# luntergroup/smcsmc

Hardware: AMD Instinct MI355X
Metric: genome segments/sec per EM iteration (Np=10000, 2 diploids, 100 Mb) (higher is better)
Workload: dtype f64

## Files before the change

include/smcsmc_pf.h:

```cpp
#ifndef SMCSMC_PF_H
#define SMCSMC_PF_H
#include <stdint.h>

#ifdef __cplusplus
extern "C" {
#endif

typedef struct pf_model {
    int32_t n_epochs;
    int32_t n_pops;
    int32_t nsam;
    int32_t flags;
    double loci_length;
    double mutation_rate;
    double recombination_rate;
    const double* change_times;
    const double* pop_sizes;
    const double* mig_rates;
    const double* single_mig;
    const int32_t* sample_pops;
    const int32_t* record_flags;
    const double* lags;
    int32_t n_bias_heights;
    int32_t delay_type;
    const double* bias_heights;
    const double* bias_strengths;
    const double* application_delays;
    const double* vb_coal_counts;
    const double* vb_mig_counts;
    int32_t n_rate_segments;
    int32_t reserved2;
    const double* rate_positions;
    const double* rate_values;
    const double* leaf_rel_rates;
    const double* sample_times;
} pf_model;

typedef struct pf_params {
    int64_t np;
    double ess_fraction;
    uint64_t seed;
    int32_t max_trace_events;
    int32_t flags;
    int64_t log_cap;
    int64_t gen_cap;
    int64_t piece_cap;
    int32_t debug;
    int32_t mig_cap;
    int32_t count_wgs;
    int32_t delay_cap;
    int32_t count_workers;
    int32_t reserved4;
} pf_params;
#define PF_MODEL_WIDE_POPS 4
#define PF_MODEL_SAMPLE_TIMES 8
#define PF_FLAG_MP_LDS_ROWS 8
#define PF_DEBUG_FORCE_LDS 1
#define PF_DEBUG_NO_FUSE   2
#define PF_DEBUG_NO_COUNT  4
#define PF_DEBUG_TWO_LAUNCH 8
#define PF_DEBUG_NO_SPEC_STAGE 32
#define PF_DEBUG_K_PIPE   16

#define PF_DEBUG_NO_DRAW_TABLE 128

#define PF_DEBUG_NO_SEARCH_LUT 256

#define PF_DEBUG_ONE_LAUNCH (1 << 23)

#define PF_DEBUG_SIGNAL_ALL_COUNTS 16384
#define PF_DEBUG_NO_PAIR 4096
#define PF_DEBUG_FORCE_WIDE 2048

typedef struct pf_segments {
    int64_t n;
    const double* start;
    const double* length;
    const int8_t* state;
    const int8_t* alleles;
    const int32_t* max_record_epoch;
} pf_segments;

typedef struct pf_lookahead {
    int32_t level;
    int32_t max_doubletons;
    int32_t n_quantiles;
    int32_t flags;
    int64_t n;
    const double* first_singleton_distance;
    const double* relative_mutation_rate;
    const int8_t* is_singleton_unphased;
    const int32_t* n_doubletons;
    const int8_t* doubleton_idx;
    const double* doubleton_dist;
    const double* first_split_distance;
    const int8_t* split_alleles;
    const int32_t* split_count;
    const double* quantiles;
    const double* tbl_lengths;
    double mean_total_branch_length;
} pf_lookahead;
#define PF_LA_ROW_PIPELINE 1
#define PF_LA_ROW_PIPELINE_MP 2
#define PF_LA_ROW_PIPELINE_LDS 4

typedef struct pf_handle pf_handle;

#define PF_COUNTS_LEN(E) (6 * (E) + 4)
#define PF_COUNTS_LEN2(E, P) ((P) == 1 ? PF_COUNTS_LEN(E) : (3 * (E) * (P) + 3 * (E) + (E) * (P) * (P) + 2 * (E) * (P) + 4))

const char* pf_last_error(void);
int pf_device_count(void);
int pf_device_cus(int device);

pf_handle* pf_create(const pf_model* model, const pf_params* params, int device);
void pf_destroy(pf_handle* h);

int pf_init_prior(pf_handle* h, double initial_position);
int64_t pf_sample_tree_events(pf_handle* h, int32_t* kind, double* pos, double* height, uint32_t* desc, int64_t max_events,
                              int64_t* particle_out);
int64_t pf_sample_tree_events_pops(pf_handle* h, int32_t* kind, double* pos, double* height, uint32_t* desc, int32_t* from_pop,
                                   int32_t* to_pop, int64_t max_events, int64_t* particle_out);

int pf_load_lookahead(pf_handle* h, const pf_lookahead* la);
int pf_terminal_branch_quantiles(const pf_model* model, uint64_t seed, int64_t n_trees, const double* quantiles, int32_t nq,
                                 double* lengths_out, double* mean_total_out, int device);
int pf_load_segments(pf_handle* h, const pf_segments* segs);

int pf_update_segment(pf_handle* h, int64_t s);
int pf_count(pf_handle* h, int64_t s, int end_data);
int pf_resample(pf_handle* h, int64_t s);
int pf_run(pf_handle* h, int64_t s_begin, int64_t s_end);
int pf_run_many(pf_handle* const* handles, int32_t n_handles, int64_t s_begin, int64_t s_end);
int pf_can_run_many(pf_handle* const* handles, int32_t n_handles);
#define PF_PATH_GENERAL     0
#define PF_PATH_TWO_LAUNCH  1
#define PF_PATH_K_PIPE      2
#define PF_PATH_SWEEP       3
#define PF_PATH_SWEEP_SPLIT 4
#define PF_PATH_SWEEP_XMP   5
#define PF_PATH_SWEEP_XL    6
#define PF_PATH_SWEEP_XLMP  7
int pf_get_run_path(pf_handle* h, int many);
#define PF_ROW_FORM_NONE    0
#define PF_ROW_FORM_SINGLE  1
#define PF_ROW_FORM_PAIRED  2
int pf_get_row_form(pf_handle* h);
int pf_finish(pf_handle* h);
int pf_sync(pf_handle* h);

int64_t pf_num_segments_done(pf_handle* h);
double pf_logl(pf_handle* h);
int pf_get_counts(pf_handle* h, double* packed, int32_t n);
int pf_get_trace(pf_handle* h, double* T, double* ess, int32_t* resampled, double* logl, int64_t n);
int pf_get_resample_events(pf_handle* h, int32_t* seg_idx, int32_t* parents, int32_t max_events);
int pf_get_local_recomb(pf_handle* h, double* opp_diff, double* counts, int64_t nbins);
int pf_get_migrations(pf_handle* h, int32_t* n_events, double* times, int8_t* branch, int8_t* newpop, int8_t* node_pops,
                      int32_t cap);
int pf_get_particles(pf_handle* h, double* w_post, double* w_pilot, double* heights, int8_t* children,
                     double* next_base);
int pf_get_kernel_time(pf_handle* h, int k, double* ms, int64_t* launches);
int pf_set_timing(pf_handle* h, int enable);
int pf_debug_stamps(pf_handle* h, int64_t rows, uint64_t* out);
int pf_test_search_lut(const double* tab, int32_t n, uint8_t* lut, int32_t* kbase);
int pf_probe_handoff(int32_t mode, int32_t rows, int32_t nw, int64_t spin_ticks, double* us_per_row, double* checksum, int32_t device);
int pf_probe_tree_edit(int32_t ncases, const double* S, const int32_t* C, const double* h, const int32_t* lin, const int32_t* rp,
                        const int32_t* sb, const double* tc, const double* u_attach, int32_t* out_i, double* out_d, int32_t device);
int pf_probe_wave_prims(int32_t nwaves, const double* xd, const int32_t* xi, double* out_d, int32_t* out_i, int32_t device);
int pf_set_wg_trace(pf_handle* h, int64_t first_step, int32_t n_steps);
int64_t pf_get_wg_trace(pf_handle* h, uint64_t* out, int64_t cap_words, int32_t* info);
int pf_get_delay_stats(pf_handle* h, int64_t* n_forced, int32_t* peak_pending);
int pf_get_stats(pf_handle* h, int64_t* n_records, int64_t* state_bytes_per_particle, int64_t* n_resamples);

int pf_median_survival(const pf_model* model, uint64_t seed, int32_t min_events, int64_t max_trees, double* median_out,
                       int64_t* trees_used, int device);
int pf_median_survival_opts(const pf_model* model, uint64_t seed, int32_t min_events, int64_t max_trees, double* median_out,
                            int64_t* trees_used, int32_t debug, int device);

int pf_simulate_sites(const pf_model* model, uint64_t seed, int32_t nchunks, int64_t max_sites, double* pos, uint32_t* masks,
                      int64_t* n_sites, int device);
int pf_simulate_sites_wide(const pf_model* model, uint64_t seed, int32_t nchunks, int64_t max_sites, double* pos, uint64_t* masks,
                        int64_t* n_sites, int device);

int pf_test_math(const double* x, int64_t n, double* out_exp, double* out_log, double* out_fastexp, int device);
int pf_test_div(const double* a, const double* b, int64_t n, double* out, int device);
int pf_test_uniform(uint64_t seed, uint32_t slot, uint32_t stream, uint64_t first_draw, int64_t n, double* out,
                    int device);
int pf_test_reduce(const double* x, int64_t n, double* out_sum, double* out_incl_scan, int device);
int pf_test_systematic(const double* pilot, int64_t n, double u, int32_t* lo, int device);
int64_t pf_test_live_bytes(void);
int pf_test_plan(const pf_model* model, const pf_params* params, int32_t* out, int32_t n_out);

#ifdef __cplusplus
}
#endif
#endif
```

smcsmc_amd/csrc/pf_device.h:

```cpp
#pragma once
#include <hip/hip_runtime.h>
#include <stdint.h>

#ifndef PF_BS
#define PF_BS 256
#endif
#define PF_NMAX 16
#define PF_NMAX_WIDE 64
#define PF_INF (__longlong_as_double(0x7ff0000000000000LL))

namespace pf {

__device__ __forceinline__ double dexp(double x) {
    const double ln2HI = 6.93147180369123816490e-01;
    const double ln2LO = 1.90821492927058770002e-10;
    const double invln2 = 1.44269504088896338700e+00;
    const double P1 = 1.66666666666666019037e-01;
    const double P2 = -2.77777777770155933842e-03;
    const double P3 = 6.61375632143793436117e-05;
    const double P4 = -1.65339022054652515390e-06;
    const double P5 = 4.13813679705723846039e-08;
    if (x > 709.782712893383973096) return PF_INF;
    if (x < -745.13321910194110842) return 0.0;
    double ax = x < 0 ? -x : x;
// ... 134 lines not shown
        c0 = n0; c1 = lo1; c2 = n2; c3 = lo0;
        k0 += 0x9E3779B9u;
        k1 += 0xBB67AE85u;
    }
    unsigned long long b0 = (((unsigned long long)c0 << 32) | c1) >> 11;
    unsigned long long b1 = (((unsigned long long)c2 << 32) | c3) >> 11;
    u0 = ((double)b0 + 0.5) * 1.1102230246251565e-16;
    u1 = ((double)b1 + 0.5) * 1.1102230246251565e-16;
}

__device__ __forceinline__ int pf_bx() { return (int)blockIdx.x; }
__device__ __forceinline__ int pf_chunk() { return (int)blockIdx.y; }

constexpr int DPP_QUAD_XOR1 = 0xB1, DPP_QUAD_XOR2 = 0x4E, DPP_ROW_HALF_MIRROR = 0x141, DPP_ROW_MIRROR = 0x140, DPP_WAVE_SHR1 = 0x138;
constexpr int DPP_ROW_SHR = 0x110, DPP_ROW_ROR = 0x120, DPP_ROW_BCAST15 = 0x142, DPP_ROW_BCAST31 = 0x143;

template <int CTRL, int ROW_MASK = 0xf>
__device__ __forceinline__ int dpp_mov(int old, int src) { return __builtin_amdgcn_update_dpp(old, src, CTRL, ROW_MASK, 0xf, false); }
template <int CTRL, int ROW_MASK = 0xf>
__device__ __forceinline__ double dpp_mov(double old, double src) {
    const int lo = dpp_mov<CTRL, ROW_MASK>(__double2loint(old), __double2loint(src));
    const int hi = dpp_mov<CTRL, ROW_MASK>(__double2hiint(old), __double2hiint(src));
    return __hiloint2double(hi, lo);
}
struct WavePairI { int a, b; };
struct WavePairD { double a, b; };
__device__ __forceinline__ WavePairI wave_swap16(int v) {
    const auto r = __builtin_amdgcn_permlane16_swap((unsigned)v, (unsigned)v, false, false);
    return {(int)r[0], (int)r[1]};
}
__device__ __forceinline__ WavePairI wave_swap32(int v) {
    const auto r = __builtin_amdgcn_permlane32_swap((unsigned)v, (unsigned)v, false, false);
    return {(int)r[0], (int)r[1]};
}
__device__ __forceinline__ WavePairD wave_swap16(double v) {
    const WavePairI lo = wave_swap16(__double2loint(v)), hi = wave_swap16(__double2hiint(v));
    return {__hiloint2double(hi.a, lo.a), __hiloint2double(hi.b, lo.b)};
}
__device__ __forceinline__ WavePairD wave_swap32(double v) {
    const WavePairI lo = wave_swap32(__double2loint(v)), hi = wave_swap32(__double2hiint(v));
    return {__hiloint2double(hi.a, lo.a), __hiloint2double(hi.b, lo.b)};
}
template <class T>
__device__ __forceinline__ T wave_row_up(T v, int lane) {
    const auto r = wave_swap16(v);
    const auto h = wave_swap32(r.b);
    return (lane & 16) ? r.a : h.a;
}

__device__ __forceinline__ double wave_tree_sum_lds(double v) {
#pragma unroll
    for (int m = 1; m < 64; m <<= 1) v = v + __shfl_xor(v, m, 64);
    return v;
}
__device__ __forceinline__ double wave_tree_sum(double v) {
    v = v + dpp_mov<DPP_QUAD_XOR1>(v, v);
    v = v + dpp_mov<DPP_QUAD_XOR2>(v, v);
    v = v + dpp_mov<DPP_ROW_HALF_MIRROR>(v, v);
    v = v + dpp_mov<DPP_ROW_MIRROR>(v, v);
    const WavePairD r = wave_swap16(v);
    v = r.a + r.b;
    const WavePairD h = wave_swap32(v);
    return h.a + h.b;
}
__device__ __forceinline__ void wave_minmax_lds(int& cmin, int& cmax) {
#pragma unroll
    for (int m = 1; m < 64; m <<= 1) {
        int o1 = __shfl_xor(cmin, m, 64), o2 = __shfl_xor(cmax, m, 64);
        cmin = o1 < cmin ? o1 : cmin; cmax = o2 > cmax ? o2 : cmax;
    }
}
__device__ __forceinline__ void wave_minmax(int& cmin, int& cmax) {
    cmin = min(cmin, dpp_mov<DPP_QUAD_XOR1>(cmin, cmin));             cmax = max(cmax, dpp_mov<DPP_QUAD_XOR1>(cmax, cmax));
    cmin = min(cmin, dpp_mov<DPP_QUAD_XOR2>(cmin, cmin));             cmax = max(cmax, dpp_mov<DPP_QUAD_XOR2>(cmax, cmax));
    cmin = min(cmin, dpp_mov<DPP_ROW_HALF_MIRROR>(cmin, cmin));       cmax = max(cmax, dpp_mov<DPP_ROW_HALF_MIRROR>(cmax, cmax));
    cmin = min(cmin, dpp_mov<DPP_ROW_MIRROR>(cmin, cmin));            cmax = max(cmax, dpp_mov<DPP_ROW_MIRROR>(cmax, cmax));
    const WavePairI a = wave_swap16(cmin), b = wave_swap16(cmax);
    cmin = min(a.a, a.b); cmax = max(b.a, b.b);
    const WavePairI c = wave_swap32(cmin), e = wave_swap32(cmax);
    cmin = min(c.a, c.b); cmax = max(e.a, e.b);
}
template <int CTRL, int ROW_MASK>
__device__ __forceinline__ double wave_dpp_add(double v) {
    const int lo = __double2loint(v), hi = __double2hiint(v);
    const int slo = __builtin_amdgcn_update_dpp(0, lo, CTRL, ROW_MASK, 0xf, false);
    const int shi = __builtin_amdgcn_update_dpp(0, hi, CTRL, ROW_MASK, 0xf, false);
    return v + __hiloint2double(shi, slo);
}
__device__ __forceinline__ double wave_total_dpp(double v) {
    v = wave_dpp_add<0x111, 0xf>(v);
    v = wave_dpp_add<0x112, 0xf>(v);
    v = wave_dpp_add<0x114, 0xf>(v);
    v = wave_dpp_add<0x118, 0xf>(v);
    v = wave_dpp_add<0x142, 0xa>(v);
    v = wave_dpp_add<0x143, 0xc>(v);
    const int lo = __builtin_amdgcn_readlane(__double2loint(v), 63), hi = __builtin_amdgcn_readlane(__double2hiint(v), 63);
    return __hiloint2double(hi, lo);
}
template <class T>
__device__ __forceinline__ T wave_prev_lane(T v, T first) { return dpp_mov<DPP_WAVE_SHR1>(first, v); }
__device__ __forceinline__ double wave_hs_scan_lds(double v, int lane) {
#pragma unroll
    for (int d = 1; d < 64; d <<= 1) {
        double o = __shfl_up(v, d, 64);
        if (lane >= d) v = o + v;
    }
    return v;
}
__device__ __forceinline__ double wave_hs_scan(double v, int lane) {
    double o = dpp_mov<DPP_WAVE_SHR1>(v, v);
    v = lane >= 1 ? o + v : v;
    o = dpp_mov<DPP_WAVE_SHR1>(v, v); o = dpp_mov<DPP_WAVE_SHR1>(o, o);
    v = lane >= 2 ? o + v : v;
    o = dpp_mov<DPP_ROW_SHR + 4>(dpp_mov<DPP_ROW_ROR + 4>(v, wave_row_up(v, lane)), v);
    v = lane >= 4 ? o + v : v;
    o = dpp_mov<DPP_ROW_SHR + 8>(dpp_mov<DPP_ROW_ROR + 8>(v, wave_row_up(v, lane)), v);
    v = lane >= 8 ? o + v : v;
    o = wave_row_up(v, lane);
    v = lane >= 16 ? o + v : v;
    o = wave_swap32(v).a;
    v = lane >= 32 ? o + v : v;
    return v;
}
__device__ __forceinline__ double wave_max_scan_d_lds(double v, int lane) {
#pragma unroll
    for (int d = 1; d < 64; d <<= 1) {
        double o = __shfl_up(v, d, 64);
        if (lane >= d) v = o > v ? o : v;
    }
    return v;
}
__device__ __forceinline__ int wave_max_scan_i_lds(int v, int lane) {
#pragma unroll
    for (int d = 1; d < 64; d <<= 1) {
        int o = __shfl_up(v, d, 64);
        if (lane >= d) v = max(v, o);
    }
    return v;
}
template <int CTRL, int ROW_MASK = 0xf>
__device__ __forceinline__ double wave_dpp_max(double v) { const double o = dpp_mov<CTRL, ROW_MASK>(v, v); return o > v ? o : v; }
template <int CTRL, int ROW_MASK = 0xf>
__device__ __forceinline__ int wave_dpp_max(int v) { return max(v, dpp_mov<CTRL, ROW_MASK>(v, v)); }
template <class T>
__device__ __forceinline__ T wave_max_scan(T v) {
    v = wave_dpp_max<DPP_ROW_SHR + 1>(v);
    v = wave_dpp_max<DPP_ROW_SHR + 2>(v);
    v = wave_dpp_max<DPP_ROW_SHR + 4>(v);
    v = wave_dpp_max<DPP_ROW_SHR + 8>(v);
    v = wave_dpp_max<DPP_ROW_BCAST15, 0xa>(v);
    v = wave_dpp_max<DPP_ROW_BCAST31, 0xc>(v);
    return v;
}
__device__ __forceinline__ double wave_max_scan_d(double v, int) { return wave_max_scan(v); }
__device__ __forceinline__ int wave_max_scan_i(int v, int) { return wave_max_scan(v); }

struct Lane {
    double* S;
    int8_t* C;
    const double* T;
    const double* I;
    const double* H;
    double uq0, uq1, uq2, uq3;
    int uqn = 0;
    const int* RF;
    int E, n;
    double L, mu, rho;
    unsigned long long seed;
    unsigned slot;
    unsigned stream;
    unsigned long long ctr;
    double ebuf;
    double Ltree;
    const double* vbc;
    double upd_fac;
    const double* ST = nullptr;
    double STsum = 0.0;
};

#define LS(ln, r) ((ln).S[(r) * PF_BS])
#define LC(ln, r, s) ((ln).C[((r) * 2 + (s)) * PF_BS])

__device__ __forceinline__ void prefetch_update_uniforms(Lane& ln) {
    philox_pair(ln.seed, ln.slot, ln.stream, ln.ctr, ln.uq0, ln.uq1);
    philox_pair(ln.seed, ln.slot, ln.stream, ln.ctr + 1, ln.uq2, ln.uq3);
    ln.ctr += 2;
    ln.uqn = 4;
}
__device__ __forceinline__ double uni(Lane& ln) {
    if (ln.uqn > 0) {
        const double u = ln.uqn == 4 ? ln.uq0 : (ln.uqn == 3 ? ln.uq1 : (ln.uqn == 2 ? ln.uq2 : ln.uq3));
        --ln.uqn;
        return u;
    }
    return philox_uniform(ln.seed, ln.slot, ln.stream, ln.ctr++);
}

__device__ __forceinline__ int epoch_of(const Lane& ln, double t) {
    int e = 0;
    while (e + 1 < ln.E && ln.T[e + 1] <= t) ++e;
    return e;
}
__device__ __forceinline__ double epoch_end(const Lane& ln, int e) { return e + 1 < ln.E ? ln.T[e + 1] : PF_INF; }
__device__ __forceinline__ double node_h(const Lane& ln, int id) { return id < ln.n ? (ln.ST ? ln.ST[id] : 0.0) : LS(ln, id - ln.n); }
__device__ __forceinline__ bool leaf_absent(const Lane& ln, int id, double time) { return ln.ST && id < ln.n && ln.ST[id] > time; }

__device__ __forceinline__ double tree_length(const Lane& ln, int nleaves) {
    double acc = 0.0, prev = 0.0;
    for (int r = 0; r < nleaves - 1; ++r) {
        double s = LS(ln, r);
        acc += (double)(nleaves - r) * (s - prev);
        prev = s;
    }
    if (ln.ST) acc -= ln.STsum;
    return acc;
}

__device__ __forceinline__ int lineages_at(const Lane& ln, int ni, double time, int want, int* pr, int* ps) {
    int R = 0;
    while (R < ni && LS(ln, R) <= time) ++R;
    int cnt = 0;
    for (int r = R; r < ni; ++r)
        for (int s = 0; s < 2; ++s) {
            int id = LC(ln, r, s);
            if ((id < ln.n || id - ln.n < R) && !leaf_absent(ln, id, time)) {
                if (cnt == want) { *pr = r; *ps = s; }
                ++cnt;
            }
        }
    return cnt;
}

__device__ __forceinline__ void remove_rank(Lane& ln, int ni, int rp, int sib, int* a, int* b) {
    const int pid = ln.n + rp;
    for (int r = rp + 1; r < ni; ++r)
        for (int s = 0; s < 2; ++s)
            if (LC(ln, r, s) == pid) LC(ln, r, s) = (int8_t)sib;
    for (int r = rp; r + 1 < ni; ++r) {
        LS(ln, r) = LS(ln, r + 1);
        LC(ln, r, 0) = LC(ln, r + 1, 0);
        LC(ln, r, 1) = LC(ln, r + 1, 1);
    }
    for (int r = 0; r < ni - 1; ++r)
        for (int s = 0; s < 2; ++s)
            if (LC(ln, r, s) > pid) LC(ln, r, s) -= 1;
    if (*a > pid) *a -= 1;
    if (*b > pid) *b -= 1;
}

__device__ __forceinline__ void insert_node(Lane& ln, int ni, double h, int fl, int pr, int ps, int root_id) {
    int rn = 0;
    while (rn < ni && LS(ln, rn) <= h) ++rn;
    const int nid = ln.n + rn;
    for (int r = 0; r < ni; ++r)
        for (int s = 0; s < 2; ++s)
            if (LC(ln, r, s) >= nid) LC(ln, r, s) += 1;
    if (fl >= nid) fl += 1;
    if (root_id >= nid) root_id += 1;
    for (int r = ni; r > rn; --r) {
        LS(ln, r) = LS(ln, r - 1);
        LC(ln, r, 0) = LC(ln, r - 1, 0);
        LC(ln, r, 1) = LC(ln, r - 1, 1);
    }
    int target;
    if (pr >= 0) {
        if (pr >= rn) pr += 1;
        target = LC(ln, pr, ps);
        LC(ln, pr, ps) = (int8_t)nid;
    } else {
        target = root_id;
    }
    LS(ln, rn) = h;
    LC(ln, rn, 0) = (int8_t)fl;
    LC(ln, rn, 1) = (int8_t)target;
}

template <class HeightAt>
__device__ __forceinline__ double coalesce_up(Lane& ln, HeightAt Sh, int ns, int nl, double h) {
    int e = epoch_of(ln, h);
    double Hc = ln.H[e] + (h - ln.T[e]) * ln.I[e];
    int i = 0;
    while (i < ns && Sh(i) <= h) ++i;
    double lower = h, kd;
    for (;;) {
        if (i >= ns) { kd = 1.0; break; }
        kd = (double)(nl - i);
        const double sn = Sh(i);
        const int en = epoch_of(ln, sn);
        const double Hn = ln.H[en] + (sn - ln.T[en]) * ln.I[en];
        const double need = (Hn - Hc) * kd;
        if (!(ln.ebuf > need)) break;
        ln.ebuf -= need;
        Hc = Hn; lower = sn; ++i;
    }
    const double C = Hc + ln.ebuf / kd;
    int es = 0;
    while (es + 1 < ln.E && ln.H[es + 1] <= C) ++es;
    double t1 = ln.T[es] + (C - ln.H[es]) / ln.I[es];
    if (t1 < lower) t1 = lower;
    if (i < ns) { const double sn = Sh(i); if (t1 > sn) t1 = sn; }
    ln.ebuf = -dlog(uni(ln));
    if (ln.vbc) ln.upd_fac *= ln.vbc[es];
    return t1;
}

__device__ __forceinline__ double sample_next_base(Lane& ln, double x) {
// ... 61 lines not shown
```

smcsmc_amd/csrc/pf_get.h:

```cpp
#pragma once

int pf_sync(pf_handle* h) {
    HIPCHK(hipSetDevice(h->device));
    HIPCHK(hipStreamSynchronize(h->cstream));
    if (h->fin_pending) {
        hipLaunchKernelGGL(k_count_fin, dim3(1), dim3(256), 0, h->stream, h->A);
        h->fin_pending = false;
    }
    HIPCHK(hipStreamSynchronize(h->stream));
    if (harvest_spans(h)) return -1;
    Ctrl c;
    if (read_ctrl(h, c)) return -1;
    if (c.err) {
        const char* msg = "unknown device error";
        if (c.err == ERR_LOG_OVERFLOW) msg = "event log ring overflow (raise pf_params.log_cap)";
        if (c.err == ERR_GEN_OVERFLOW) msg = "generation ledger overflow (raise pf_params.gen_cap)";
        if (c.err == ERR_ZERO_PROB) msg = "Zero or negative probabilities";
        if (c.err == ERR_MIG_OVERFLOW) msg = "too many migration events on one local tree";
        if (c.err == ERR_MP_INTERNAL) msg = "structured-model genealogy update: coalescence partners inconsistent";
        if (c.err == ERR_NO_COALESCENCE) msg = "No final coalescence event was sampled!";
        if (c.err == ERR_DELAY_OVERFLOW) msg = "delayed-factor store overflow (raise pf_params.delay_cap)";
        if (c.err == ERR_PAIR_STALL) msg = "row kernel, paired form: a wavefront waited 0.1 s for its partner (PF_DEBUG_NO_PAIR runs the other form)";
        g_err = msg;
        return -2;
// ... 181 lines not shown
                                 double* out) {
    const int g = (int)(blockIdx.x * blockDim.x + threadIdx.x);
    if (g >= ngen) return;
    double* o = out + (size_t)off[g] * A.RS;
    for (unsigned k = k0[g]; k < k1[g]; ++k) {
        const double* rec = rec_ptr(A, slot[g], k);
        for (int j = 0; j < A.RS; ++j) *o++ = rec[j];
    }
}

__global__ void k_gather_pieces(KArgs A, int nrec, const int* slot, const unsigned* pstart, const unsigned* np, const long long* off,
                                double* out) {
    const int i = (int)(blockIdx.x * blockDim.x + threadIdx.x);
    if (i >= nrec) return;
    double* o = out + (size_t)off[i] * 3;
    for (unsigned j = 0; j < np[i]; ++j) {
        const double* q = A.plog + ((size_t)slot[i] * A.pcap + ((pstart[i] + j) % A.pcap)) * 3;
        *o++ = q[0]; *o++ = q[1]; *o++ = q[2];
    }
}

int64_t pf_sample_tree_events(pf_handle* h, int32_t* kind, double* pos, double* height, uint32_t* desc, int64_t max_events,
                              int64_t* particle_out) {
    return pf_sample_tree_events_pops(h, kind, pos, height, desc, nullptr, nullptr, max_events, particle_out);
}

int64_t pf_sample_tree_events_pops(pf_handle* h, int32_t* kind, double* pos, double* height, uint32_t* desc, int32_t* from_pop,
                                   int32_t* to_pop, int64_t max_events, int64_t* particle_out) {
    if (!h->A.rec_trees) { g_err = "pf_sample_tree_events: the handle was not created with tree recording (pf_params.flags bit 1)"; return -1; }
    if (pf_sync(h)) return -1;
    Ctrl c;
    if (read_ctrl(h, c)) return -1;
    const long long Np = h->Np;
    std::vector<double> w;
    if (download(w, state_slot(h->A, c.cur).w_pilot, (size_t)Np)) return -1;
    double total = 0.0;
    for (double v : w) total += v;
    const double u = philox_uniform_host((unsigned long long)h->A.seed, 0xFFFFFFFFu, 1, (unsigned long long)c.n_resample);
    long long j = 0;
    double acc = 0.0;
    for (; j < Np - 1; ++j) { acc += w[j]; if (acc > u * total) break; }
    if (particle_out) *particle_out = j;
    const int G = c.gen;
    std::vector<unsigned> k0, k1, rstart, rnp;
    std::vector<long long> off(G + 1);
    std::vector<long long> poff;
    std::vector<int> rslot;
    DevMem tmp;
    int* dslot; unsigned *dk0, *dk1; const long long* doff;
    if (tmp.reserve(&dslot, (size_t)G + 1) || tmp.reserve(&dk0, (size_t)G + 1) || tmp.reserve(&dk1, (size_t)G + 1)) return -1;
    hipLaunchKernelGGL(k_trace_ancestry, dim3(1), dim3(1), 0, h->stream, h->A, G, (int)j, dslot, dk0, dk1);
    HIPCHK(hipStreamSynchronize(h->stream));
    if (download(k0, dk0, (size_t)G + 1) || download(k1, dk1, (size_t)G + 1)) return -1;
    long long nrec = 0;
    for (int g = 0; g <= G; ++g) { off[g] = nrec; nrec += (long long)(k1[g] - k0[g]); }
    const int RS = h->A.RS;
    double* drec;
    if (tmp.upload(&doff, off.data(), (size_t)G + 1, h->stream) || tmp.reserve(&drec, (size_t)nrec * RS)) return -1;
    hipLaunchKernelGGL(k_gather_records, dim3((unsigned)((G + 1 + 255) / 256)), dim3(256), 0, h->stream, h->A, G + 1, dslot, dk0, dk1, doff, drec);
    HIPCHK(hipStreamSynchronize(h->stream));
    std::vector<double> rec;
    if (download(rec, drec, (size_t)nrec * RS)) return -1;
    std::vector<double> pieces;
    poff.assign((size_t)nrec + 1, 0);
    if (h->P > 1 && nrec) {
        std::vector<int> gslot;
        if (download(gslot, dslot, (size_t)G + 1)) return -1;
        rslot.resize((size_t)nrec); rstart.resize((size_t)nrec); rnp.resize((size_t)nrec);
        for (int g = 0; g <= G; ++g)
            for (long long r = off[g]; r < off[g] + (long long)(k1[g] - k0[g]); ++r) rslot[(size_t)r] = gslot[g];
        for (long long r = 0; r < nrec; ++r) {
            const double* q = &rec[(size_t)r * RS];
            unsigned long long meta, ref;
            memcpy(&meta, &q[4], 8);
            memcpy(&ref, &q[3], 8);
            const int type = (int)(meta & 0xff);
            const bool has = type == 0 || type == 2;
            rstart[(size_t)r] = has ? (unsigned)(ref & 0xffffffffu) : 0u;
            rnp[(size_t)r] = has ? (unsigned)(ref >> 32) : 0u;
            poff[(size_t)r + 1] = poff[(size_t)r] + rnp[(size_t)r];
        }
        const long long npieces = poff[(size_t)nrec];
        const int* d_s; const unsigned *d_p0, *d_np; const long long* d_off; double* d_out;
        if (tmp.upload(&d_s, rslot.data(), (size_t)nrec, h->stream) || tmp.upload(&d_p0, rstart.data(), (size_t)nrec, h->stream) ||
            tmp.upload(&d_np, rnp.data(), (size_t)nrec, h->stream) || tmp.upload(&d_off, poff.data(), (size_t)nrec, h->stream) ||
            tmp.reserve(&d_out, (size_t)npieces * 3)) return -1;
        hipLaunchKernelGGL(k_gather_pieces, dim3((unsigned)((nrec + 255) / 256)), dim3(256), 0, h->stream, h->A, (int)nrec, d_s, d_p0, d_np, d_off, d_out);
        HIPCHK(hipStreamSynchronize(h->stream));
        if (download(pieces, d_out, (size_t)npieces * 3)) return -1;
    }
    tmp.clear();
    int64_t nout = 0;
    auto emit = [&](int kd, double x, double t, unsigned d, int from, int to) {
        if (nout < max_events) {
            if (kind) kind[nout] = kd;
            if (pos) pos[nout] = x;
            if (height) height[nout] = t;
            if (desc) desc[nout] = d;
            if (from_pop) from_pop[nout] = from;
            if (to_pop) to_pop[nout] = to;
        }
        ++nout;
    };
    const unsigned full = (1u << h->n) - 1u;
    for (long long r = nrec - 1; r >= 0; --r) {
        const double* q = &rec[(size_t)r * RS];
        unsigned long long meta;
        memcpy(&meta, &q[4], 8);
        const int type = (int)(meta & 0xff);
        if (type != 0 && type != 2) continue;
        const unsigned cut = (unsigned)((meta >> 32) & 0xffff), below = (unsigned)((meta >> 48) & 0xffff);
        if (type == 0) emit(0, q[1], q[2], cut, -1, -1);
        if (h->P == 1) { emit(1, q[1], q[3], below, 0, -1); continue; }
        const int leaf = (int)((meta >> 24) & 0xff);
        const unsigned fl = type == 0 ? cut : (1u << leaf);
        const unsigned rt = type == 0 ? (full & ~cut) : ((1u << leaf) - 1u);
        for (long long j = poff[(size_t)r + 1] - 1; j >= poff[(size_t)r]; --j) {
            long long tag;
            memcpy(&tag, &pieces[(size_t)j * 3], 8);
            const int pop = (int)(tag & 0xff), kd = (int)((tag >> 8) & 0xff), to = (int)((tag >> 16) & 0xff);
            const double t1 = pieces[(size_t)j * 3 + 2];
            if (kd & 1) emit(1, q[1], t1, below, pop, -1);
            if (kd & 2) emit(2, q[1], t1, (kd & 4) ? rt : fl, pop, to);
        }
    }
    return nout;
}

int pf_set_timing(pf_handle* h, int period) {
    h->timing_period = period;
    if (period > 0 && h->span_overhead_ms == 0) {
        HIPCHK(hipSetDevice(h->device));
        HIPCHK(hipStreamSynchronize(h->stream));
        std::vector<float> empty;
        for (int i = 0; i < 64; ++i) {
            hipEvent_t a = get_event(h), b = get_event(h);
            hipEventRecord(a, h->stream); hipEventRecord(b, h->stream);
            HIPCHK(hipEventSynchronize(b));
            float ms = 0;
            HIPCHK(hipEventElapsedTime(&ms, a, b));
            empty.push_back(ms);
            h->ev_pool.push_back(a); h->ev_pool.push_back(b);
        }
        std::sort(empty.begin(), empty.end());
        h->span_overhead_ms = empty[empty.size() / 2];
    }
    return 0;
}

int pf_debug_stamps(pf_handle* h, int64_t rows, uint64_t* out) {
    HIPCHK(hipSetDevice(h->device));
    if (rows > 0 && !out) {
        unsigned long long* buf = nullptr;
        if (h->alloc(&buf, (size_t)rows * h->A.nc * PF_STAMP_W)) return -1;
        HIPCHK(hipMemset(buf, 0, (size_t)rows * h->A.nc * PF_STAMP_W * 8));
        HIPCHK(hipStreamSynchronize(h->stream));
        h->A.stamps = buf; h->A.stamp_rows = rows;
        return 0;
    }
    if (!h->A.stamps) { g_err = "pf_debug_stamps: not enabled"; return -1; }
    if (pf_sync(h)) return -1;
    HIPCHK(hipMemcpy(out, h->A.stamps, (size_t)std::min<long long>(rows, h->A.stamp_rows) * h->A.nc * PF_STAMP_W * 8, hipMemcpyDeviceToHost));
    return 0;
}

int pf_get_kernel_time(pf_handle* h, int k, double* ms, int64_t* launches) {
    if (k < 0 || k > 3) return -1;
    if (pf_sync(h)) return -1;
    double mean = h->k_timed[k] ? h->k_ms[k] / (double)h->k_timed[k] : 0.0;
    if (ms) *ms = mean * (double)h->k_launches[k];
    if (launches) *launches = h->k_launches[k];
    return 0;
}

int pf_set_wg_trace(pf_handle* h, int64_t first_step, int32_t n_steps) {
    HIPCHK(hipSetDevice(h->device));
    if (pf_sync(h)) return -1;
    h->trace_mem.clear(); h->d_trace = nullptr;
    h->trace_t0 = (int)std::max<int64_t>(0, first_step);
    h->trace_n = std::max(0, n_steps);
    h->trace_stride = 0; h->trace_words = 0;
    return 0;
}

int64_t pf_get_wg_trace(pf_handle* h, uint64_t* out, int64_t cap_words, int32_t* info) {
    if (hipSetDevice(h->device) != hipSuccess || pf_sync(h)) return -1;
    if (info) { info[0] = h->d_trace ? h->trace_n : 0; info[1] = h->trace_stride; }
    if (!h->d_trace) return 0;
    const size_t nw = std::min<size_t>(h->trace_words, (size_t)std::max<int64_t>(0, cap_words));
    if (out && nw && hipMemcpy(out, h->d_trace, nw * 8, hipMemcpyDeviceToHost) != hipSuccess) { g_err = "copy of the workgroup trace failed"; return -1; }
    return (int64_t)h->trace_words;
}

int pf_get_delay_stats(pf_handle* h, int64_t* n_forced, int32_t* peak_pending) {
    if (pf_sync(h)) return -1;
    Ctrl c;
    if (read_ctrl(h, c)) return -1;
    if (n_forced) *n_forced = (int64_t)c.n_delay_evict;
    if (peak_pending) *peak_pending = c.delay_peak;
    return 0;
}

int pf_get_stats(pf_handle* h, int64_t* n_records, int64_t* state_bytes, int64_t* n_resamples) {
    if (pf_sync(h)) return -1;
    if (n_records) {
        std::vector<unsigned> w;
        if (download(w, h->A.widx, (size_t)h->Np)) return -1;
        long long t = 0;
        for (unsigned v : w) t += v;
        *n_records = t;
    }
    if (state_bytes) *state_bytes = (int64_t)(h->n - 1) * 8 + 2 * (h->n - 1) + 5 * 8 + 4 + 8 + 8 + 4;
    if (n_resamples) {
        Ctrl c;
        if (read_ctrl(h, c)) return -1;
        *n_resamples = c.n_resample;
    }
    return 0;
}
```

smcsmc_amd/csrc/pf_hip.hip:

```cpp
#include <hip/hip_runtime.h>
#include <type_traits>
#include <hip/hip_ext.h>

#include <algorithm>
#include <atomic>
#include <cmath>
#include <cstdio>
#include <cstdlib>
#include <cstring>
#include <mutex>
#include <string>
#include <vector>

#include "../../include/smcsmc_pf.h"
#include "pf_device.h"
#include "pf_types.h"
#include "pf_lane.h"
#include "pf_tree_reg.h"
#include "pf_look_reg.h"
#include "pf_lds_body.h"
#include "pf_mp_host.h"
#include "pf_wide_host.h"
#include "pf_pipe.h"
#include "pf_lds_pipe.h"

using namespace pf;

__global__ __launch_bounds__(PF_BS) void k_init(KArgs A, double initial_position) {
    extern __shared__ double smem[];
    init_lds_body(A, initial_position, smem);
}

__global__ __launch_bounds__(PF_BS) void k_extend(KArgs A, long long s) {
    extern __shared__ double smem[];
    extend_lds_body(A, s, smem);
}

__device__ __forceinline__ double in_vgpr(double x) { double y; asm("v_mov_b64 %0, %1" : "=v"(y) : "s"(x)); return y; }
__device__ __forceinline__ unsigned long long in_vgpr(unsigned long long x) { unsigned long long y; asm("v_mov_b64 %0, %1" : "=v"(y) : "s"(x)); return y; }

#ifdef PF_STAMPS
__device__ __forceinline__ void pf_acc_trip(unsigned long long* a) { a[5] += 1; }
#else
#define pf_acc_trip(a) do {} while (0)
#endif
#ifdef PF_STAMPS
#define PF_STAMP(k) do { if (A.stamps && (threadIdx.x & 63) == 0 && s < A.stamp_rows)                                   \
        A.stamps[((size_t)s * A.nc + (size_t)(((long long)pf_bx() * PF_BS + threadIdx.x) >> 6)) * PF_STAMP_W + (k)] = wall_clock64(); } while (0)
#define PF_TICK(var) unsigned long long var = wall_clock64()
#define PF_ACC(slot, t0, t1) pf_acc[slot] += (t1) - (t0)
#define PF_ACC_DECL unsigned long long pf_acc[6] = {0, 0, 0, 0, 0, 0}, pf_acc2[8] = {0, 0, 0, 0, 0, 0, 0, 0}
#define PF_ACC_PARAMS , unsigned long long* pf_acc, unsigned long long* pf_acc2, unsigned long long tk1
#define PF_ACC_ARGS , pf_acc, pf_acc2, tk1
#define PF_ACC2(slot, t0, t1) pf_acc2[slot] += (t1) - (t0)
#define PF_ACC_STORE do { if (A.stamps && (threadIdx.x & 63) == 0 && s < A.stamp_rows) {                                \
        for (int k_ = 0; k_ < 6; ++k_)                                                                                  \
            A.stamps[((size_t)s * A.nc + (size_t)(((long long)pf_bx() * PF_BS + threadIdx.x) >> 6)) * PF_STAMP_W + 9 + k_] = pf_acc[k_]; \
        for (int k_ = 0; k_ < 8; ++k_)                                                                                  \
            A.stamps[((size_t)s * A.nc + (size_t)(((long long)pf_bx() * PF_BS + threadIdx.x) >> 6)) * PF_STAMP_W + 21 + k_] = pf_acc2[k_]; } } while (0)
#else
#define PF_STAMP(k) do {} while (0)
#define PF_TICK(var) do {} while (0)
#define PF_ACC(slot, t0, t1) do {} while (0)
#define PF_ACC2(slot, t0, t1) do {} while (0)
#define PF_ACC_DECL do {} while (0)
#define PF_ACC_PARAMS
#define PF_ACC_ARGS
#define PF_ACC_STORE do {} while (0)
#endif

template <class KA>
__device__ __forceinline__ int gridDim_particles(const KA& A) { return (int)((A.Np + PF_BS - 1) / PF_BS); }

__device__ __forceinline__ int pf_arrive(int v) { asm volatile("" : "+v"(v)); return __builtin_amdgcn_readfirstlane(v); }
__device__ __forceinline__ long long pf_arrive(long long v) {
    asm volatile("" : "+v"(v));
    const unsigned lo = (unsigned)__builtin_amdgcn_readfirstlane((int)(unsigned)((unsigned long long)v & 0xffffffffu));
    const unsigned hi = (unsigned)__builtin_amdgcn_readfirstlane((int)(unsigned)((unsigned long long)v >> 32));
    return (long long)(((unsigned long long)hi << 32) | lo);
}
__device__ __forceinline__ double pf_arrive(double v) { return __longlong_as_double(pf_arrive(__double_as_longlong(v))); }

__device__ __forceinline__ int row_spec_lo(int first, int own, int nc, int flags) {
    int spec_lo = first - (PF_PIPE_STAGE - own) / 2;
    if (spec_lo > nc - PF_PIPE_STAGE) spec_lo = nc - PF_PIPE_STAGE;
    if (spec_lo < 0) spec_lo = 0;
    if (flags & 256) spec_lo = -0x40000000;
    return spec_lo;
}
__device__ __forceinline__ int row_parent_chunk(const PipeLds& q, int nc, double lhs, double dn) {
    int lo_c = 0, hi_c = nc - 1;
    while (lo_c < hi_c) {
        int mid = (lo_c + hi_c) >> 1;
        if (lhs < dn * q.pmx[mid + 1]) hi_c = mid; else lo_c = mid + 1;
    }
    return lo_c;
}
template <class KA, class MARK>
__device__ __forceinline__ void row_parent_in_chunk(const KA& A, const PipeLds& q, const double* sm, int pch, int stage_lo, int nst, double lhs, double dn,
                                                    long long p, const RowDecision& d, long long& a, bool& first_copy, MARK&& found) {
    const double coff_p = pipe_chunk_offset(q, pch);
    const double pm_p = q.pmx[pch];
    const bool staged = pch >= stage_lo && pch - stage_lo < nst;
    auto val_at = [&](int l) -> double {
        long long idx = (long long)pch * 64 + l;
        double smv = staged ? q.stage[(pch - stage_lo) * 64 + l] : (idx < A.Np ? sm[idx] : PF_INF);
        double w = coff_p + smv;
        return pm_p > w ? pm_p : w;
    };
    int lo_l = 0, hi_l = 63;
    while (lo_l < hi_l) {
        int mid = (lo_l + hi_l) >> 1;
        if (lhs < dn * val_at(mid)) hi_l = mid; else lo_l = mid + 1;
    }
    a = (long long)pch * 64 + lo_l;
    found();
    if (a > A.Np - 1) a = A.Np - 1;
    const int la = (int)(a & 63);
    if (p == 0 || a == 0) first_copy = (p == 0);
    else {
        double vprev = la > 0 ? val_at(la - 1) : pm_p;
        if (a != (long long)pch * 64 + lo_l) {
            long long am = a - 1;
            int chm = (int)(am >> 6);
            double w = pipe_chunk_offset(q, chm) + sm[am];
            vprev = q.pmx[chm] > w ? q.pmx[chm] : w;
        }
        first_copy = ((((double)(p - 1)) + d.u) * d.S1 < dn * vprev);
    }
}
__device__ __forceinline__ void row_close_record(double* rec, double x_mark, double pos, int mark_limit, int n) {
    rec[0] = x_mark;
    rec[1] = pos;
    rec[2] = 0.0; rec[3] = 0.0;
    rec[4] = __longlong_as_double((long long)make_meta(1, mark_limit, -1, n));
}
struct RowMasks { unsigned one = 0, zero = 0, present = 0, two = 0; int missing = 0; };
template <int NM, class F>
__device__ __forceinline__ RowMasks row_masks(int n, F&& allele) {
    RowMasks m;
#pragma unroll
    for (int i = 0; i < NM; ++i) if (i < n) {
        int d = allele(i);
        m.missing += d == -1;
        if (d == 1) m.one |= 1u << i;
        if (d == 0) m.zero |= 1u << i;
        if (d == 2) m.two |= 1u << i;
        if (d >= 0) m.present |= 1u << i;
    }
    return m;
}
template <int NM>
__device__ __forceinline__ double row_site_lik(const RTree<NM>& t, int n, double v_mu, unsigned one_mask, unsigned zero_mask, unsigned two_mask, bool dephase, bool anc) {
    unsigned het_pairs = 0;
    int ncfg = 1;
    for (int i = 0; i + 1 < n; i += 2) {
        bool d0_two = (two_mask >> i) & 1u;
        bool one0 = (one_mask >> i) & 1u, one1 = (one_mask >> (i + 1)) & 1u;
        bool zero0 = (zero_mask >> i) & 1u, zero1 = (zero_mask >> (i + 1)) & 1u;
        bool het = d0_two || (dephase && ((one0 && zero1) || (zero0 && one1)));
        if (het) {
            ncfg *= 2;
            het_pairs |= 1u << i;
            one_mask &= ~(3u << i); zero_mask &= ~(3u << i);
            zero_mask |= 1u << i;
            one_mask |= 1u << (i + 1);
        }
    }
    double norm = 1.0 / (double)ncfg;
    RBranchP<NM> bprob;
    r_site_branch_probs(t, n, v_mu, bprob);
    double lik = 0;
    for (;;) {
        lik += r_site_lik_from(t, n, bprob, one_mask, zero_mask, anc);
        if (ncfg == 1) break;
        bool more = false;
        for (int i = 0; i + 1 < n; i += 2) {
            if (!((het_pairs >> i) & 1)) continue;
            if ((zero_mask >> i) & 1) {
                zero_mask &= ~(1u << i); one_mask |= 1u << i;
                one_mask &= ~(1u << (i + 1)); zero_mask |= 1u << (i + 1);
                more = true;
                break;
            }
            one_mask &= ~(1u << i); zero_mask |= 1u << i;
            zero_mask &= ~(1u << (i + 1)); one_mask |= 1u << (i + 1);
        }
        if (!more) break;
    }
    lik *= norm;
    return lik;
}
struct RowScans { double sc, sp, sq, scp, scm; };
__device__ __forceinline__ RowScans row_scans(double w_post, double w_pilot, int lane) {
    RowScans r;
    r.sc = wave_hs_scan(w_pilot, lane);
    r.sp = wave_tree_sum(w_post);
    r.sq = wave_tree_sum(w_pilot * w_pilot);
    r.scp = wave_hs_scan(w_post, lane);
    r.scm = wave_max_scan_d(r.sc, lane);
    return r;
}
template <class KA>
__device__ __forceinline__ void row_scans_store(const KA& A2, int cur, long long p, bool active, int lane, const RowScans& r) {
    const long long chunk = p >> 6;
    const size_t ro = (size_t)cur * A2.Np, co = (size_t)cur * A2.nc;
    if (active) { A2.rg_scan1[ro + p] = r.sc; A2.rg_scanp[ro + p] = r.scp; A2.rg_scan1m[ro + p] = r.scm; }
    if (p == A2.Np - 1) A2.ctrl->last1[cur] = r.sc;
    if (lane == 63 && chunk < A2.nc) {
        A2.rg_cpost[co + chunk] = r.sp;
        A2.rg_csq[co + chunk] = r.sq;
        A2.rg_cpil[co + chunk] = r.sc;
        A2.rg_cpp[co + chunk] = r.scp;
// ... 999 lines not shown
    lmap_add(L, last, -(li * dens));
}
__device__ __forceinline__ void lmap_opportunity(const LMap& L, double x_lo, double x_hi, double weight, double opp) {
    const double iv = 100.0;
    long long first = (long long)(x_lo / iv);
    long long last = (long long)(1 + x_hi / iv);
    double dens = weight * opp / (x_hi - x_lo);
    if (first == last - 1) {
        double top = (double)(first + 1) * iv;
        double first_interval = (top < x_hi ? top : x_hi) - x_lo;
        lmap_add(L, first, first_interval * dens);
        lmap_add(L, first + 1, -(first_interval * dens));
    } else {
        lmap_left(L, x_lo, dens);
        lmap_right(L, x_hi, dens);
    }
}
template <class M>
__device__ __forceinline__ void lmap_event(const LMap& L, int n, double event_base, double h, M desc, double weight) {
    long long idx = (long long)(event_base / 100.0);
    if (idx < 0 || idx >= L.nbins) return;
    const int nd = sizeof(M) == 8 ? __popcll((unsigned long long)desc) : __popc((unsigned)desc);
    const long long k = idx - L.b0;
    if (k >= 0 && k < L.ncnt) {
        typedef __attribute__((address_space(3))) double lds_double;
        lds_double* base = (lds_double*)L.lds + L.nlds + k;
        for (int i = 0; i < n; ++i)
            if ((desc >> i) & (M)1) __hip_atomic_fetch_add(base + (size_t)i * L.ncnt, weight / nd, __ATOMIC_RELAXED, __HIP_MEMORY_SCOPE_WORKGROUP);
        __hip_atomic_fetch_add(base + (size_t)n * L.ncnt, weight * h, __ATOMIC_RELAXED, __HIP_MEMORY_SCOPE_WORKGROUP);
        __hip_atomic_fetch_add(base + (size_t)(n + 1) * L.ncnt, weight * dlog(h + 1.0), __ATOMIC_RELAXED, __HIP_MEMORY_SCOPE_WORKGROUP);
        return;
    }
    for (int i = 0; i < n; ++i)
        if ((desc >> i) & (M)1) atomicAdd(&L.gcnt[(size_t)i * L.nbins + idx], weight / nd);
    atomicAdd(&L.gcnt[(size_t)n * L.nbins + idx], weight * h);
    atomicAdd(&L.gcnt[(size_t)(n + 1) * L.nbins + idx], weight * dlog(h + 1.0));
}

template <int NI, int P, class KA>
__device__ __forceinline__ void stretch_contrib(AccT<P>& acc, const KA& A, const Win& W, const LMap& L, double w, double x0,
                                                double x1, const double (&S)[NI], int lim_start) {
    if (!(W.rf & REC_RECOMB) || W.e > lim_start) return;
    double xs = ovl(x0, x1, W.a_e, W.b_e);
    if (!(xs > 0.0)) return;
    double len = slice_len<NI>(S, A.n - 1, A.n, W.T0, W.T1, 0.0, PF_INF, false) - W.dead;
    if (!(len > 0.0)) return;
    double opp = len * xs;
    acc.v[AccT<P>::RO] += w * opp;
    acc.v[AccT<P>::RW] += w * w * opp;
    if (L.gopp) lmap_opportunity(L, x0 > W.a_e ? x0 : W.a_e, x1 < W.b_e ? x1 : W.b_e, w, opp);
}

template <int NI, int P, class KA>
__device__ __forceinline__ void record_contrib_one(AccT<P>& acc, const KA& A, const Win& W, const LMap& L, double w, long long a,
                                                   double f0, double f1, double f2, double f3, double f4, const double (&S)[NI],
                                                   unsigned long long desc_wide = 0) {
    using AC = AccT<P>;
    const int n = A.n;
    double x0 = f0, x1 = f1;
    if (x1 < W.a_e) return;
    unsigned long long meta = (unsigned long long)__double_as_longlong(f4);
    int type = (int)(meta & 0xff);
    int lim_start = (int)((meta >> 8) & 0xff) - 1;
    int lim_event = (int)((meta >> 16) & 0xff) - 1;
    int n_eff = (int)((meta >> 24) & 0xff);
    if (type <= 1) stretch_contrib<NI, P>(acc, A, W, L, w, x0, x1, S, lim_start);
    if (type == 0 || type == 2) {
        double h = f2;
        bool inwin = (W.a_e <= x1) && (x1 < W.b_e);
        if constexpr (P == 1) {
            double tc = f3;
            if (inwin && (W.rf & REC_COALMIGR) && W.e <= lim_event && tc >= W.T0 && h < W.T1) {
                double opp = slice_len<NI>(S, n_eff - 1, n_eff, W.T0, W.T1, h, tc, true);
                acc.v[AC::CO] += w * opp;
                acc.v[AC::CW] += w * w * opp;
                if (W.T0 <= tc && tc < W.T1) acc.v[AC::CC] += w;
            }
        } else {
            (void)n_eff;
            const unsigned span = (unsigned)((meta >> 48) & 0xffff);
            const bool elsewhere = !A.rec_trees && (span & 0x1000u) && (W.e < (int)(span & 63u) || W.e > (int)((span >> 6) & 63u));
            if (inwin && (W.rf & REC_COALMIGR) && W.e <= lim_event && !elsewhere) {
                unsigned long long ref = (unsigned long long)__double_as_longlong(f3);
                unsigned pstart = (unsigned)(ref & 0xffffffffu), np_ = (unsigned)(ref >> 32);
                if (A.pidx[a] - pstart > A.pcap || np_ > A.pcap) { if (!A.ctrl->err) A.ctrl->err = ERR_LOG_OVERFLOW; np_ = 0; }
                for (unsigned j = 0; j < np_; ++j) {
                    const double* q = A.plog + ((size_t)a * A.pcap + ((pstart + j) % A.pcap)) * 3;
                    long long tag = __double_as_longlong(q[0]);
                    const double t0 = q[1], t1 = q[2];
                    const int pop = (int)(tag & 0xff), kind = (int)((tag >> 8) & 0xff), to = (int)((tag >> 16) & 0xff);
                    const double lo = t0 > W.T0 ? t0 : W.T0, hi = t1 < W.T1 ? t1 : W.T1;
                    const double mo = hi > lo ? hi - lo : 0.0;
                    const bool ev = (kind & 3) != 0 && W.T0 <= t1 && t1 < W.T1;
                    if (!(mo > 0.0) && !ev) continue;
                    const double co = (double)((tag >> 24) & 0xff) * mo;
#pragma unroll
                    for (int pp = 0; pp < P; ++pp)
                        if (pp == pop) {
                            acc.v[AC::CO + pp] += w * co;
                            acc.v[AC::CW + pp] += w * w * co;
                            acc.v[AC::MO + pp] += w * mo;
                            acc.v[AC::MW + pp] += w * w * mo;
                            if (ev && (kind & 1)) acc.v[AC::CC + pp] += w;
                            if (ev && (kind & 2)) {
                                if constexpr (AC::MIG_LDS) {
                                    if (to < P) __hip_atomic_fetch_add((pf_lds_double*)count_mig() + pp * P + to, w, __ATOMIC_RELAXED, __HIP_MEMORY_SCOPE_WORKGROUP);
                                } else {
#pragma unroll
                                for (int qq = 0; qq < P; ++qq)
                                    if (qq == to) acc.v[AC::MC + pp * P + qq] += w;
                                }
                            }
                        }
                }
            }
        }
        if (type == 0) {
            bool inwin_r = (W.a_e <= x1) && ((x1 < W.b_e) || W.end_seq);
            if (inwin_r && (W.rf & REC_RECOMB) && W.e <= lim_event && W.T0 <= h && h < W.T1) {
                acc.v[AC::RC] += w;
                if constexpr (NI >= PF_NMAX) { if (L.gopp) lmap_event(L, n, x1, h, desc_wide, w); }
                else { if (L.gopp) lmap_event(L, n, x1, h, (unsigned)((meta >> 32) & 0xffff), w); }
            }
        }
    }
}

template <int NI, int P, class KA>
__device__ __forceinline__ void records_contrib(AccT<P>& acc, const KA& A, const Win& W, const LMap& L, double w, long long a,
                                                unsigned k0, unsigned k1) {
    const int n = A.n;
    unsigned lo = k0, len = k1 - k0;
    while (len > 4) {
        const unsigned q = len >> 2;
        const double xa = rec_ptr(A, a, lo + q)[1], xb = rec_ptr(A, a, lo + 2 * q)[1], xc = rec_ptr(A, a, lo + 3 * q)[1];
        if (xc < W.a_e) { lo += 3 * q + 1; len -= 3 * q + 1; }
        else if (xb < W.a_e) { lo += 2 * q + 1; len = q; }
        else if (xa < W.a_e) { lo += q + 1; len = q; }
        else len = q;
    }
    for (unsigned k = lo; k != k1; ++k) {
        const double* rec = rec_ptr(A, a, k);
        double f0 = rec[0], f1 = rec[1], f2 = rec[2], f3 = rec[3], f4 = rec[4];
        double S[NI];
#pragma unroll
        for (int r = 0; r < NI; ++r) S[r] = r < n - 1 ? rec[5 + r] : 0.0;
        if (f0 >= W.b_e && !W.end_seq) break;
        unsigned long long dw = 0;
        if constexpr (NI >= PF_NMAX) if (L.gopp) dw = (unsigned long long)__double_as_longlong(rec[4 + n]);
        record_contrib_one<NI, P>(acc, A, W, L, w, a, f0, f1, f2, f3, f4, S, dw);
    }
}

struct RunLists { int* st; int* anc; int* nruns; };
struct CountSrc {
    const double* w; const double* S; const double* xm; const int* ml; const unsigned* widx;
    const unsigned* widx_live;
    const double* scanp; const double* offp;
    RunLists lists;
    double inv; int G, g_lo, g_hi;
};
template <class KA>
__device__ __forceinline__ RunLists run_lists(const KA& A, int ver) {
    RunLists r;
    r.st = ver ? A.run_st2 : A.run_st; r.anc = ver ? A.run_anc2 : A.run_anc; r.nruns = ver ? A.nruns2 : A.nruns;
    return r;
}
template <class KA>
__device__ __forceinline__ CountSrc count_src_parity(const KA& A, int sp, int e) {
    const Ctrl* c = A.ctrl;
    CountSrc q;
    q.w = A.snap_w[sp]; q.S = A.snap_S[sp]; q.xm = A.snap_xm[sp]; q.ml = A.snap_ml[sp]; q.widx = A.snap_widx[sp];
    q.widx_live = A.widx;
    q.scanp = A.scanp2[sp]; q.offp = A.chunk_offp2[sp];
    q.lists = run_lists(A, c->lver);
    q.inv = c->step[sp].inv_T; q.G = c->step[sp].G;
    q.g_lo = e < A.E ? c->g_lo[e] : 0; q.g_hi = e < A.E ? c->g_hi[e] : 0;
    return q;
}

__device__ __forceinline__ double* count_bins() {
    __shared__ double bins[PF_LBINS];
    return bins;
}

#define PF_COUNT_LDS_BYTES 14336
template <int BYTES>
__device__ __forceinline__ char* count_lds() {
    __shared__ __attribute__((aligned(16))) char buf[BYTES];
    return buf;
}

#define PF_CNT_TILE 2048
#define PF_CNT_WIDE 128
#define PF_CNT_BATCH 2

template <int NI, int P, class KA>
__device__ __forceinline__ void count_run(AccT<P>& acc, const KA& A, const CountSrc& Q, const Win& W, const LMap& L, int g, long long i,
                                          int nr, const int* rst, const int* ran, double inv) {
    const long long Np = A.Np;
    int q0 = rst[i];
    int q1 = i + 1 < nr ? rst[i + 1] : (int)Np;
    long long a = ran[i];
    if (q1 <= q0 || q1 > (int)Np || q0 < 0 || a < 0 || a >= Np) return;
    const double* offp = Q.offp;
    const double* scp_ = Q.scanp;
    double hi = offp[(q1 - 1) >> 6] + scp_[q1 - 1];
    double lo = q0 > 0 ? offp[(q0 - 1) >> 6] + scp_[q0 - 1] : 0.0;
    double w = (hi - lo) * inv;
    if (!(w > 0.0)) return;
    unsigned k0 = A.gstart[(size_t)(g % A.Gcap) * Np + a];
    unsigned k1 = A.gstart[(size_t)((g + 1) % A.Gcap) * Np + a];
    if (Q.widx_live[a] - k0 > A.cap || k1 - k0 > A.cap) { if (!A.ctrl->err) A.ctrl->err = ERR_LOG_OVERFLOW; return; }
    records_contrib<NI, P>(acc, A, W, L, w, a, k0, k1);
}

struct FlatTask { double w; int a; unsigned k0; };
__device__ __forceinline__ FlatTask* count_flat_tasks() {
    __shared__ FlatTask ft[PF_BS];
    return ft;
}
__device__ __forceinline__ int* count_flat_prefix() {
    __shared__ int pre[PF_BS + 1];
    return pre;
}

template <int NM, int P, bool EXACT = false, bool ACC_AT_ENTRY = false, bool ANC = false, class KA>
__device__ __forceinline__ void count_body(const KA& A, const CountSrc& Q, int e, double win_a, double win_b, int bx, int nbxg) {
    constexpr int NI = NM - 1;
    using AC = AccT<P>;
    double acc_before = 0.0;
    if constexpr (ACC_AT_ENTRY) { if (threadIdx.x < AC::NC) acc_before = A.partial[((size_t)e * A.nbx + bx) * AC::NC + threadIdx.x]; }
    constexpr int LDS_BYTES = (int)(((sizeof(AC) * (PF_BS / 64) + 15) & ~(size_t)15) + sizeof(int) * (PF_CNT_TILE + 1 + PF_BS / 64) + 16);
    char* const cl = count_lds<LDS_BYTES>();
    AC* const red = (AC*)cl;
    int* const s_off = (int*)(cl + ((sizeof(AC) * (PF_BS / 64) + 15) & ~(size_t)15));
    int* const s_wsum = s_off + PF_CNT_TILE + 1;
    const long long Np = A.Np;
    const int n = EXACT ? NM : A.n;
    const int G = Q.G;
    const double inv = Q.inv;
    Win W;
    W.e = e; W.rf = A.recflags[e];
    W.T0 = A.T[e]; W.T1 = e + 1 < A.E ? A.T[e + 1] : PF_INF;
    W.a_e = win_a; W.b_e = win_b;
    W.end_seq = (A.L == W.b_e);
    if constexpr (ANC) W.dead = A.anc[A.n + e]; else W.dead = 0.0;
    double* const s_lbins = count_bins();
    LMap L;
    L.lds = s_lbins; L.b0 = (long long)(W.a_e / 100.0); L.gopp = A.lmap_opp; L.gcnt = A.lmap_cnt; L.nbins = A.lmap_bins;
    {
        const long long span = (long long)(W.b_e / 100.0) - L.b0 + 4;
        L.nlds = span < 1 ? 1 : (span > PF_LBINS ? PF_LBINS : (int)span);
        L.ncnt = (A.n + 3) * L.nlds <= PF_LBINS ? L.nlds : 0;
    }
    bool bins_ready = false;
    const int g_lo = Q.g_lo, g_hi = Q.g_hi;
    if (g_hi < g_lo) return;
    const int lane = threadIdx.x & 63;
    const long long gtid = (long long)bx * PF_BS + threadIdx.x;
    const long long nthreads = (long long)nbxg * PF_BS;
    AC acc;
#pragma unroll
    for (int k = 0; k < AC::NR; ++k) acc.v[k] = 0.0;
    if constexpr (AC::MIG_LDS) { if (threadIdx.x < P * P) count_mig()[threadIdx.x] = 0.0; }
    for (int tile_hi = g_hi; tile_hi >= g_lo; tile_hi -= PF_CNT_TILE) {
        const int tile_lo = tile_hi - PF_CNT_TILE + 1 > g_lo ? tile_hi - PF_CNT_TILE + 1 : g_lo;
        const int ntile = tile_hi - tile_lo + 1;
        __syncthreads();
        constexpr int PER = PF_CNT_TILE / PF_BS;
        int loc[PER];
        int lsum = 0;
#pragma unroll
        for (int k = 0; k < PER; ++k) {
            int idx = threadIdx.x * PER + k;
            int v = 0;
            if (idx < ntile) {
                int g = tile_hi - idx;
                v = g == G ? (int)Np : Q.lists.nruns[g % A.Gcap];
            }
            loc[k] = v;
            lsum += v;
        }
        int incl = lsum;
#pragma unroll
        for (int d = 1; d < 64; d <<= 1) {
            int o = __shfl_up(incl, d, 64);
            if (lane >= d) incl += o;
        }
        if (lane == 63) s_wsum[threadIdx.x >> 6] = incl;
        __syncthreads();
        int base = 0;
        for (int w = 0; w < (int)(threadIdx.x >> 6); ++w) base += s_wsum[w];
        int run = base + incl - lsum;
#pragma unroll
        for (int k = 0; k < PER; ++k) {
            int idx = threadIdx.x * PER + k;
            if (idx <= ntile) s_off[idx] = run;
            run += loc[k];
        }
        if (threadIdx.x == PF_BS - 1) s_off[ntile] = run;
        __syncthreads();
        const long long T = s_off[ntile];
        if (tile_hi == g_hi && tile_lo == g_lo && (long long)bx * PF_BS >= T) return;
        if (A.flags & (1 << 20)) return;
        if (L.gopp && !bins_ready) {
            for (int k = threadIdx.x; k < L.nlds + (A.n + 2) * L.ncnt; k += PF_BS) s_lbins[k] = 0.0;
            __syncthreads();
            bins_ready = true;
        }
        FlatTask* const s_ft = count_flat_tasks();
        int* const s_fpre = count_flat_prefix();
        for (long long base = (long long)bx * PF_BS; base < T; base += nthreads) {
            const long long t = base + threadIdx.x;
            const bool tval = t < T;
            int lo_i = 0, hi_i = ntile;
            while (tval && hi_i - lo_i > 1) {
                int mid = (lo_i + hi_i) >> 1;
                if ((long long)s_off[mid] <= t) lo_i = mid; else hi_i = mid;
            }
            const int tg = tile_hi - lo_i;
            const long long ti = t - s_off[lo_i];
            const int tnr = s_off[lo_i + 1] - s_off[lo_i];
            const bool tlive = tval && tg == G;
            int q0 = 0, q1 = 0;
            long long aa = -1;
            if (tval && !tlive) {
                const int* rst = Q.lists.st + (size_t)(tg % A.Gcap) * Np;
                const int* ran = Q.lists.anc + (size_t)(tg % A.Gcap) * Np;
                q0 = rst[ti];
                q1 = ti + 1 < tnr ? rst[ti + 1] : (int)Np;
                aa = ran[ti];
            }
            double w = 0.0;
            long long a_t = 0;
            unsigned k0 = 0, nrec = 0;
            if (tlive) {
                const long long a = ti;
                w = Q.w[a] * inv;
                double S[NI];
#pragma unroll
                for (int r = 0; r < NI; ++r) S[r] = r < n - 1 ? Q.S[(size_t)r * Np + a] : 0.0;
                const double xm = Q.xm[a];
                const int ml = Q.ml[a];
                const unsigned g0 = A.gstart[(size_t)(tg % A.Gcap) * Np + a];
                const unsigned g1 = Q.widx[a];
                if (!(A.flags & (1 << 21)) && w != 0.0) {
                    stretch_contrib<NI, P>(acc, A, W, L, w, xm, PF_INF, S, ml);
                    if (g1 - g0 > A.cap) { if (!A.ctrl->err) A.ctrl->err = ERR_LOG_OVERFLOW; }
                    else { a_t = a; k0 = g0; nrec = g1 - g0; }
                }
            } else if (tval && !(q1 <= q0 || q1 > (int)Np || q0 < 0 || aa < 0 || aa >= Np)) {
                const double mhi = Q.offp[(q1 - 1) >> 6] + Q.scanp[q1 - 1];
                const double mlo = q0 > 0 ? Q.offp[(q0 - 1) >> 6] + Q.scanp[q0 - 1] : 0.0;
                const unsigned rk0 = A.gstart[(size_t)(tg % A.Gcap) * Np + aa];
                const unsigned rk1 = A.gstart[(size_t)((tg + 1) % A.Gcap) * Np + aa];
                const unsigned rwl = Q.widx_live[aa];
                w = (mhi - mlo) * inv;
                if (!(A.flags & (1 << 21)) && w > 0.0) {
                    if (rwl - rk0 > A.cap || rk1 - rk0 > A.cap) { if (!A.ctrl->err) A.ctrl->err = ERR_LOG_OVERFLOW; }
                    else { a_t = aa; k0 = rk0; nrec = rk1 - rk0; }
                }
            }
            int incl_r = (int)nrec;
#pragma unroll
            for (int d = 1; d < 64; d <<= 1) {
                const int o = __shfl_up(incl_r, d, 64);
                if (lane >= d) incl_r += o;
            }
            if (lane == 63) s_wsum[threadIdx.x >> 6] = incl_r;
            __syncthreads();
            int base_r = 0;
            for (int wv = 0; wv < (int)(threadIdx.x >> 6); ++wv) base_r += s_wsum[wv];
            s_fpre[threadIdx.x] = base_r + incl_r - (int)nrec;
            if (threadIdx.x == PF_BS - 1) s_fpre[PF_BS] = base_r + incl_r;
            s_ft[threadIdx.x].w = w; s_ft[threadIdx.x].a = (int)a_t; s_ft[threadIdx.x].k0 = k0;
            __syncthreads();
            const int nrec_all = s_fpre[PF_BS];
            for (int r = (int)threadIdx.x; r < nrec_all; r += PF_BS) {
                int lo_j = 0, hi_j = PF_BS;
                while (hi_j - lo_j > 1) { const int mid = (lo_j + hi_j) >> 1; if (s_fpre[mid] <= r) lo_j = mid; else hi_j = mid; }
                const double w_r = s_ft[lo_j].w;
                const long long a_r = s_ft[lo_j].a;
                const double* rec = rec_ptr(A, a_r, s_ft[lo_j].k0 + (unsigned)(r - s_fpre[lo_j]));
                double f0 = rec[0], f1 = rec[1], f2 = rec[2], f3 = rec[3], f4 = rec[4];
                double S[NI];
#pragma unroll
                for (int q = 0; q < NI; ++q) S[q] = q < n - 1 ? rec[5 + q] : 0.0;
                unsigned long long dw = 0;
                if constexpr (NI >= PF_NMAX) if (L.gopp) dw = (unsigned long long)__double_as_longlong(rec[4 + n]);
                record_contrib_one<NI, P>(acc, A, W, L, w_r, a_r, f0, f1, f2, f3, f4, S, dw);
            }
            __syncthreads();
        }
    }
    if (L.gopp && bins_ready) {
        __syncthreads();
        for (int k = threadIdx.x; k < L.nlds; k += PF_BS) {
            double v = s_lbins[k];
            long long idx = L.b0 + k;
            if (v != 0.0 && idx < L.nbins) atomicAdd(&L.gopp[idx], v);
        }
        for (int k = threadIdx.x; k < (A.n + 2) * L.ncnt; k += PF_BS) {
            const double v = s_lbins[L.nlds + k];
            const long long idx = L.b0 + k % L.ncnt;
            if (v != 0.0 && idx < L.nbins) atomicAdd(&L.gcnt[(size_t)(k / L.ncnt) * L.nbins + idx], v);
        }
    }
#pragma unroll
    for (int k = 0; k < AC::NR; ++k) acc.v[k] = wave_tree_sum(acc.v[k]);
    if ((threadIdx.x & 63) == 0) red[threadIdx.x >> 6] = acc;
    __syncthreads();
    if (threadIdx.x < AC::NC) {
        const int k = threadIdx.x;
        double t;
        if constexpr (AC::MIG_LDS) {
            if (k >= AC::MC && k < AC::MC + P * P) t = count_mig()[k - AC::MC];
            else {
                const int kr = k < AC::MC ? k : k - P * P;
                t = red[0].v[kr];
                for (int w = 1; w < PF_BS / 64; ++w) t += red[w].v[kr];
            }
        } else {
        t = red[0].v[k];
        for (int w = 1; w < PF_BS / 64; ++w) t += red[w].v[k];
        }
        if constexpr (ACC_AT_ENTRY) A.partial[((size_t)e * A.nbx + bx) * AC::NC + k] = acc_before + t;
        else A.partial[((size_t)e * A.nbx + bx) * AC::NC + k] += t;
    }
}


template <int NM, int P>
__global__ __launch_bounds__(PF_BS) void k_count(KArgs A, int e0, Windows Wn) {
    const int e = e0 + (int)blockIdx.y;
    if (e < Wn.first || e >= A.E) return;
    count_body<NM, P>(A, count_src_parity(A, A.sp, e), e, Wn.a[e], Wn.b[e], (int)blockIdx.x, (int)gridDim.x);
}

template <int NM, int P>
__global__ __launch_bounds__(PF_BS) void k_count_anc(KArgs A, int e0, Windows Wn) {
    const int e = e0 + (int)blockIdx.y;
    if (e < Wn.first || e >= A.E) return;
    count_body<NM, P, false, false, true>(A, count_src_parity(A, A.sp, e), e, Wn.a[e], Wn.b[e], (int)blockIdx.x, (int)gridDim.x);
}

template <int NM, int P>
__global__ __launch_bounds__(PF_BS) void k_count_cw(KArgs A, int e0, Windows Wn) {
    const int e = e0 + (int)blockIdx.y;
    if (e < Wn.first || e >= A.E) return;
    const int j = A.E - 1 - e;
    const int cnb = A.cw_off[j + 1] - A.cw_off[j];
    if ((int)blockIdx.x >= cnb) return;
    count_body<NM, P>(A, count_src_parity(A, A.sp, e), e, Wn.a[e], Wn.b[e], (int)blockIdx.x, cnb);
}

template <int NM, bool BIASED, bool EXACT, bool TREES = false>
__global__ __launch_bounds__(PF_BS) void k_row(KArgs A, long long s, int fuse, int nb, int count_first, Windows Wprev) {
    if ((int)blockIdx.x < nb) {
        extend_reg_body<NM, BIASED, EXACT, TREES>(A, s, fuse);
    } else {
        const int idx = (int)blockIdx.x - nb;
        const int e = count_first + idx / nb;
        if (e < Wprev.first || e >= A.E) return;
        count_body<NM, 1, EXACT>(A, count_src_parity(A, A.sp ^ 1, e), e, Wprev.a[e], Wprev.b[e], idx % nb, nb);
    }
}

__global__ void k_count_fin(KArgs A) {
    __shared__ double stage[PF_FIN_PAIRS * PF_FIN_TILE_B];
    Ctrl* c = A.ctrl;
    if (c->pending_fin) finalize_counts(A, c, threadIdx.x, blockDim.x, stage);
}

#define PF_LEDGER_PER 8
#define PF_LEDGER_MAXT 1024
#define PF_LEDGER_NEW 64

template <class KA>
__device__ __forceinline__ void ledger_update(const KA& A, int lb, int nlb, int G, int g_ret, RunLists src, RunLists dst) {
    __shared__ int scnt[PF_LEDGER_PER * (PF_LEDGER_MAXT / 64)], sexc[PF_LEDGER_PER * (PF_LEDGER_MAXT / 64)];
    __shared__ int stot;
    const long long Np = A.Np;
    const int* lo = A.lo + (size_t)(G % A.Gcap) * (Np + 1);
    const int tid = threadIdx.x, lane = tid & 63, wave = tid >> 6;
    const int NT = (int)blockDim.x, NW = NT >> 6;
    const int NCNT = PF_LEDGER_PER * NW;
    for (int k = 1 + lb; k < PF_LEDGER_NEW; k += nlb) {
        const int g = G - k;
        if (g < g_ret) break;
        const int* rst = src.st + (size_t)(g % A.Gcap) * Np;
        const int* ran = src.anc + (size_t)(g % A.Gcap) * Np;
        int* wst = dst.st + (size_t)(g % A.Gcap) * Np;
        int* wan = dst.anc + (size_t)(g % A.Gcap) * Np;
        const int nr = src.nruns[g % A.Gcap];
        int out_base = 0;
        for (int tile0 = 0; tile0 < nr; tile0 += PF_LEDGER_PER * NT) {
            int ns[PF_LEDGER_PER], an[PF_LEDGER_PER], nx[PF_LEDGER_PER];
#pragma unroll
            for (int j = 0; j < PF_LEDGER_PER; ++j) {
                const int i = tile0 + j * NT + tid;
                ns[j] = i < nr ? rst[i] : 0;
                an[j] = i < nr ? ran[i] : 0;
                nx[j] = (lane == 63 && i < nr) ? (i + 1 < nr ? rst[i + 1] : (int)Np) : 0;
            }
#pragma unroll
            for (int j = 0; j < PF_LEDGER_PER; ++j) {
                const int i = tile0 + j * NT + tid;
                ns[j] = i < nr ? lo[ns[j]] : 0;
                nx[j] = (lane == 63 && i < nr) ? lo[nx[j]] : 0;
            }
            unsigned keep = 0;
#pragma unroll
            for (int j = 0; j < PF_LEDGER_PER; ++j) {
                const int i = tile0 + j * NT + tid;
                int ne = __shfl_down(ns[j], 1, 64);
                if (lane == 63) ne = nx[j];
                else if (i + 1 >= nr) ne = (int)Np;
                const bool kp = i < nr && ne > ns[j];
                const unsigned long long bal = __ballot(kp);
                if (kp) keep |= 1u << j;
                if (lane == 0) scnt[j * NW + wave] = __popcll(bal);
            }
            asm volatile("s_waitcnt vmcnt(0)" ::: "memory");
            __syncthreads();
            if (tid < 64) {
                const int c0 = 2 * lane < NCNT ? scnt[2 * lane] : 0;
                const int c1 = 2 * lane + 1 < NCNT ? scnt[2 * lane + 1] : 0;
                int incl = c0 + c1;
#pragma unroll
                for (int d = 1; d < 64; d <<= 1) {
                    int o = __shfl_up(incl, d, 64);
                    if (lane >= d) incl += o;
                }
                const int excl = incl - (c0 + c1);
                if (2 * lane < NCNT) sexc[2 * lane] = excl;
                if (2 * lane + 1 < NCNT) sexc[2 * lane + 1] = excl + c0;
                if (lane == 63) stot = incl;
            }
            __syncthreads();
#pragma unroll
            for (int j = 0; j < PF_LEDGER_PER; ++j) {
                const bool kp = (keep >> j) & 1u;
                const unsigned long long bal = __ballot(kp);
                if (kp) {
                    const int pos = out_base + sexc[j * NW + wave] + __popcll(bal & ((1ULL << lane) - 1ULL));
                    wst[pos] = ns[j];
                    wan[pos] = an[j];
                }
            }
            out_base += stot;
            __syncthreads();
        }
        if (tid == 0) dst.nruns[g % A.Gcap] = out_base;
    }
    const int wl = lb * NW + wave;
    const int nwl = nlb * NW;
    for (int g = G - PF_LEDGER_NEW - wl; g >= g_ret; g -= nwl) {
        const int* rst = src.st + (size_t)(g % A.Gcap) * Np;
        const int* ran = src.anc + (size_t)(g % A.Gcap) * Np;
        int* wst = dst.st + (size_t)(g % A.Gcap) * Np;
        int* wan = dst.anc + (size_t)(g % A.Gcap) * Np;
        const int nr = src.nruns[g % A.Gcap];
        int base = 0;
        for (int off = 0; off < nr; off += 64) {
            int i = off + lane;
            bool valid = i < nr;
            int stv = 0, nxt = 0, anc = 0;
            if (valid) {
                stv = rst[i];
                nxt = (i + 1 < nr) ? rst[i + 1] : (int)Np;
                anc = ran[i];
            }
            int ns = valid ? lo[stv] : 0;
            int ne = valid ? lo[nxt] : 0;
            bool keep = valid && ne > ns;
            unsigned long long bal = __ballot(keep);
            int pos = __popcll(bal & ((1ULL << lane) - 1ULL));
            if (keep) { wst[base + pos] = ns; wan[base + pos] = anc; }
            base += __popcll(bal);
        }
        if (lane == 0) dst.nruns[g % A.Gcap] = base;
    }
}

template <class KA>
__device__ __forceinline__ void ledger_new_list(const KA& A, RunLists dst, const int* blkcnt, int nblocks, int bx, int Gx, int gran = 1) {
    const long long Np = A.Np;
    const long long i = (long long)bx * PF_BS + threadIdx.x;
    __shared__ int wsum[PF_BS / 64];
    const int* lox = A.lo + (size_t)(Gx % A.Gcap) * (Np + 1);
    const int lane = threadIdx.x & 63, wave = threadIdx.x >> 6;
    int l0 = 0, l1 = 0;
    if (i < Np) { l0 = lox[i]; l1 = lox[i + 1]; }
    const bool surv = l1 > l0;
    unsigned long long bal = __ballot(surv);
    if (lane == 0) wsum[wave] = __popcll(bal);
    __shared__ int sblk[1024];
    for (int b = threadIdx.x; b < nblocks; b += PF_BS) {
        int v = 0;
        for (int j = 0; j < gran; ++j) v += blkcnt[b * gran + j];
        sblk[b] = v;
    }
    __syncthreads();
    int base = 0;
    for (int b = 0; b < bx; ++b) base += sblk[b];
    for (int w = 0; w < wave; ++w) base += wsum[w];
    if (surv) {
        int pos = base + __popcll(bal & ((1ULL << lane) - 1ULL));
        dst.st[(size_t)(Gx % A.Gcap) * Np + pos] = l0;
        dst.anc[(size_t)(Gx % A.Gcap) * Np + pos] = (int)i;
    }
    if (bx == nblocks - 1 && threadIdx.x == PF_BS - 1) {
        int tot = base + __popcll(bal);
        dst.nruns[Gx % A.Gcap] = tot;
    }
}

template <class KA>
__device__ __forceinline__ void ledger_body(const KA& A, int sp, int nblocks, int bx, int nbt) {
    const Ctrl* c = A.ctrl;
    if (!c->step[sp].flag) return;
    const int Gx = c->step[sp].G;
    const RunLists lists = run_lists(A, c->lver);
    if (bx >= nblocks) {
        ledger_update(A, bx - nblocks, nbt - nblocks, Gx, c->g_retain, lists, lists);
        return;
    }
    ledger_new_list(A, lists, A.blkcnt2[sp], nblocks, bx, Gx);
}

__global__ void k_pipe_seed(KArgs A, int slot) {
    Ctrl* c = A.ctrl;
    Ctrl::RowInfo& r = c->ri[slot];
    r.n_res = c->n_resample; r.gen = c->gen; r.flag = 0; r.lver = c->lver; r.g_retain = c->g_retain; r.first = A.E;
    r.inv_T = 1.0; r.T = 1.0; r.S1 = 0.0; r.u = 0.0; r.pos = c->cur_pos;
    c->xr[slot].n_res = c->n_resample; c->xr[slot].gen = c->gen; c->xr[slot].flag = 0;
}

template <bool BIASED, class KA>
__device__ __forceinline__ void pipe_bookkeeping(const KA& A, const PipeLds& q, const PipeLaunch& PL, const Windows& W) {
    Ctrl* c = A.ctrl;
    const int tid = threadIdx.x, lane = tid & 63, wave = tid >> 6, nwaves = PF_BS / 64;
    const int E = A.E, nc = A.nc, ng = (nc + 63) / 64;
    const int slot = PL.b_slot;
    const long long n_res = c->n_resample;
    const int G = c->gen;
    RowDecision d = decide_row<false>(A, q, slot, n_res);
    __syncthreads();
    const double* cpp = A.rg_cpp + (size_t)slot * nc;
    for (int g = wave; g < ng; g += nwaves) {
        int ch = g * 64 + lane;
        double vq = ch < nc ? cpp[ch] : 0.0;
        double scq = wave_hs_scan(vq, lane);
        if (ch < nc) q.pmx[ch] = scq;
        if (lane == 63) q.l2_post[g] = scq;
    }
    __syncthreads();
    for (int ch = tid; ch < nc; ch += PF_BS) {
        double runp = 0.0;
        for (int g = 0; g < ch / 64; ++g) runp = runp + q.l2_post[g];
        double offp = (ch % 64 == 0) ? 0.0 : q.pmx[ch - 1];
        A.rg_coffp[(size_t)slot * nc + ch] = runp + offp;
    }
    Ctrl::RowInfo& r = c->ri[slot];
    constexpr bool W_IN_LDS = !std::is_same<KA, KArgs>::value;
    for (int e = W_IN_LDS ? (tid < E ? tid : E) : 0; e < E; e = W_IN_LDS ? E : e + 1) {
        const double wa = W.a[e], wb = W.b[e];
        if (tid != e) continue;
        int g = c->g_lo[e];
        while (g < G && A.gen_x0[(g + 1) % A.Gcap] <= wa) ++g;
        c->g_lo[e] = g;
        int h = c->g_hi[e];
        if (e >= W.first) {
            if (h < g) h = g;
            while (h < G && A.gen_x0[(h + 1) % A.Gcap] < wb) ++h;
            c->g_hi[e] = h;
        }
        r.g_lo[e] = g; r.g_hi[e] = h; r.wa[e] = wa; r.wb[e] = wb;
    }
    __syncthreads();
    if (tid == 0) {
        int gr = c->g_lo[0];
        for (int e = 1; e < E; ++e) gr = c->g_lo[e] < gr ? c->g_lo[e] : gr;
        c->g_retain = gr;
        c->g_safe = c->ri[(slot + PF_RING - (PL.nL == -3 ? PF_RING - 1 : 2)) & (PF_RING - 1)].g_retain;
        c->delayed_opp += W.b[E - 1] - W.a[E - 1];
        if (BIASED) {
            long long npend = 0;
            for (int k = 0; k < nc; ++k) npend += A.rg_dpend[(size_t)slot * nc + k];
            c->delayed_count += (double)npend * (W.b[E - 1] - W.a[E - 1]);
        }
        c->first_epoch = W.first;
        c->count_active = W.first < E;
        if (W.first < E) c->pending_fin = 1;
        c->nbx_used = A.nbx;
        c->wq[PL.b_slot] = 0;
        if (!(d.T > 0.0) && !c->err) c->err = ERR_ZERO_PROB;
        double logl = c->logl + dlog(d.T);
        c->logl = logl;
        const long long row = PL.b_row;
        A.tr_T[row] = d.T; A.tr_ess[row] = d.ess; A.tr_flag[row] = d.flag; A.tr_logl[row] = logl;
        c->cur_pos = PL.b_pos;
        c->T = d.T; c->inv_T = d.inv; c->S1 = d.S1; c->S2 = d.S2; c->ess = d.ess; c->u = d.u; c->flag = 0;
        r.T = d.T; r.inv_T = d.inv; r.S1 = d.S1; r.u = d.u; r.pos = PL.b_pos;
        r.n_res = n_res; r.gen = G; r.flag = d.flag; r.g_retain = gr; r.first = W.first; r.lver = c->lver;
        if (d.flag) {
            int ev = (int)n_res;
            if (ev < A.max_trace_events) A.ev_seg[ev] = (int)row;
            c->gen = G + 1;
            A.gen_x0[(G + 1) % A.Gcap] = PL.b_pos;
            c->n_resample = n_res + 1;
            c->lver ^= 1;
            if (G + 1 - gr >= A.Gcap - 1 - (PL.ahead ? PF_RING : 0)) c->err = ERR_GEN_OVERFLOW;
            if (A.rec_trees && G + 2 >= A.Gcap) c->err = ERR_GEN_OVERFLOW;
        }
        c->gen_prev = c->gen; c->nres_prev = c->n_resample;
        if (PL.b_set_cur >= 0) c->cur = PL.b_set_cur;
    }
}

template <class KA>
__device__ __forceinline__ void draw_role(const KA& A, int tb, int nT, int par) {
    const long long Np = A.Np;
    const unsigned long long* c_in = A.dt_ctr + (size_t)(par ^ 1) * Np;
    const unsigned long long* f_in = A.dt_filled + (size_t)(par ^ 1) * Np;
    unsigned long long* f_out = A.dt_filled + (size_t)par * Np;
    const unsigned long long seed = A.seed;
    for (long long p = (long long)tb * PF_BS + threadIdx.x; p < Np; p += (long long)nT * PF_BS) {
        const unsigned long long c0 = c_in[p], f_old = f_in[p];
        const unsigned long long to = c0 + PF_DRAW_RING;
        double2* tab = (double2*)A.dt_tab + (size_t)p * PF_DRAW_RING;
        for (unsigned long long cc = f_old > c0 ? f_old : c0; cc < to; ++cc) {
            double u0, u1;
            philox_pair(seed, (unsigned)p, 0u, cc, u0, u1);
            tab[(unsigned)cc & (PF_DRAW_RING - 1)] = make_double2(u0, -dlog(u1));
        }
        f_out[p] = to;
    }
}

template <class KA>
__device__ __forceinline__ void pipe_ledger_item(const KA& A, const PipeLaunch& PL, const Ctrl::RowInfo& r, int lb) {
    const RunLists src = run_lists(A, r.lver), dst = run_lists(A, r.lver ^ 1);
    const int nblk = PL.nblk;
    if (lb < nblk) ledger_new_list(A, dst, A.rg_blkcnt + (size_t)PL.lc_slot * nblk * A.blk_gran, nblk, lb, r.gen, A.blk_gran);
    else ledger_update(A, lb - nblk, PL.nL - nblk, r.gen, r.g_retain, src, dst);
}

template <int NM, bool EXACT, int P, bool ACC_AT_ENTRY = false, class KA>
__device__ __forceinline__ void pipe_count_item(const KA& A, const PipeLaunch& PL, const Ctrl::RowInfo& r, int idx) {
    int e, cbx, cnb;
    if (A.cw_off && !(A.flags & 512)) {
        int j = 0, hi = A.E;
        while (hi - j > 1) { const int mid = (j + hi) >> 1; if (A.cw_off[mid] <= idx) j = mid; else hi = mid; }
        e = A.E - 1 - j; cbx = idx - A.cw_off[j]; cnb = A.cw_off[j + 1] - A.cw_off[j];
    } else {
        e = (A.flags & 512) ? r.first + idx / PL.ncw : A.E - 1 - idx / PL.ncw;
        cbx = idx % PL.ncw; cnb = PL.ncw;
    }
    if (e >= A.E || e < r.first) return;
    if (A.flags & (1 << 22)) return;
    const DState st = state_slot(A, PL.lc_slot);
    CountSrc Q;
    Q.w = st.w_post; Q.S = st.S; Q.xm = st.x_mark; Q.ml = st.mark_limit;
    Q.widx = A.rg_widx + (size_t)PL.lc_slot * A.Np;
    Q.widx_live = A.rg_widx + (size_t)PL.live_slot * A.Np;
    Q.scanp = A.rg_scanp + (size_t)PL.lc_slot * A.Np;
    Q.offp = A.rg_coffp + (size_t)PL.lc_slot * A.nc;
    Q.lists = run_lists(A, r.lver);
    Q.inv = r.inv_T; Q.G = r.gen; Q.g_lo = r.g_lo[e]; Q.g_hi = r.g_hi[e];
    count_body<NM, P, EXACT, ACC_AT_ENTRY>(A, Q, e, r.wa[e], r.wb[e], cbx, cnb);
}

template <int NM, bool BIASED, bool EXACT, bool TREES, int P = 1, bool BLC = false, bool QUEUE = false, bool LEAN = false, bool NO_EXTEND = false, bool LOOK = false,
          bool ACC_AT_ENTRY = false, class KA>
__device__ __forceinline__ void pipe_roles(const KA& A, long long s, const PipeLaunch& PL, const Windows& Wb) {
    const int bx = pf_bx();
    const int nb = PL.nb;
    if constexpr (!LEAN) {
        if (bx < nb) {
            if constexpr (P == 1 && !BLC && !NO_EXTEND) { if (PL.row.extend || PL.row.complete) extend_reg_body<NM, BIASED, EXACT, TREES, true, false, LOOK>(A, s, 0, PL.row); }
            return;
        }
        if (bx == nb) {
            if (PL.b_slot < 0) return;
            extern __shared__ double smem[];
            PipeLds q = pipe_carve(smem + (2 * PF_EPAD + A.E + 2 * PF_BIAS_MAX + 3), A.nc);
            pipe_bookkeeping<BIASED>(A, q, PL, Wb);
            return;
        }
        if (bx - (nb + 1) < PL.nT) {
            if constexpr (P == 1 && !BLC) draw_role(A, bx - (nb + 1), PL.nT, PL.row.draws - 1);
            return;
        }
    } else {
        if (bx <= nb) return;
    }
    if (PL.lc_slot < 0 || PL.nL < -1) return;
    const Ctrl* c = A.ctrl;
    const Ctrl::RowInfo& r = c->ri[PL.lc_slot];
    const int lb = bx - (nb + 1) - PL.nT;
    if constexpr (!QUEUE) {
        if (lb < PL.nL) { if (r.flag) pipe_ledger_item(A, PL, r, lb); }
        else pipe_count_item<NM, EXACT, P, ACC_AT_ENTRY>(A, PL, r, lb - PL.nL);
    } else {
        __shared__ int s_wk[8];
        if (lb >= PL.workers) return;
        if (threadIdx.x == 0) { s_wk[0] = PL.lc_slot; s_wk[1] = PL.live_slot; s_wk[2] = PL.nL; s_wk[3] = PL.nblk; s_wk[4] = PL.ncw; }
        const KA* Ap = &A;
        for (;;) {
            asm volatile("" : "+s"(Ap));
            const KA& A2 = *Ap;
            __syncthreads();
            if (threadIdx.x == 0) s_wk[6] = (int)__hip_atomic_fetch_add(&A2.ctrl->wq[s_wk[0]], 1u, __ATOMIC_RELAXED, __HIP_MEMORY_SCOPE_AGENT);
            __syncthreads();
            PipeLaunch Q2;
            Q2.lc_slot = s_wk[0]; Q2.live_slot = s_wk[1]; Q2.nL = s_wk[2]; Q2.nblk = s_wk[3]; Q2.ncw = s_wk[4];
            const int it = s_wk[6];
            const Ctrl::RowInfo& r2 = A2.ctrl->ri[Q2.lc_slot];
            const int ncnt = r2.first < A2.E ? (A2.cw_off ? A2.cw_off[A2.E - r2.first] : (A2.E - r2.first) * Q2.ncw) : 0;
            if (it >= ncnt + (r2.flag ? Q2.nL : 0)) return;
            if (it < ncnt) pipe_count_item<NM, EXACT, P>(A2, Q2, r2, it);
            else pipe_ledger_item(A2, Q2, r2, it - ncnt);
        }
    }
}

template <int NM, bool BIASED, bool EXACT, bool TREES>
__global__ __launch_bounds__(PF_BS) void k_pipe(KArgs A, long long s, PipeLaunch PL, Windows Wb) {
    pipe_roles<NM, BIASED, EXACT, TREES>(A, s, PL, Wb);
}

template <class KA>
__device__ __forceinline__ void sweep_windows(const KA& A, Ctrl* c, double pos, Windows& W) {
    const int e = threadIdx.x, E = A.E;
    if (e < 64) {
        const bool in = e < E;
        const double lagging = in ? A.lags[e] : 0.0;
        const double x_end = pos - lagging;
        const double ct = in ? c->counted_to[e] : 0.0;
        const bool small = (x_end - ct) < lagging * 0.1;
        const unsigned long long moved = __ballot(in && !small);
        const int first = moved ? (int)__builtin_ctzll(moved) : E;
        if (in) {
            const double b = (small && first > e) ? ct : x_end;
            W.a[e] = ct; W.b[e] = b;
            c->counted_to[e] = b;
        }
        if (e == 0) { W.first = first; W.end_data = 0; }
    }
    __syncthreads();
}

__device__ __forceinline__ unsigned long long* wg_trace_slot(SweepChunkC& ch, long long t) {
    if (!ch.trace || t < ch.trace_t0 || t >= ch.trace_t0 + ch.trace_n) return nullptr;
    const size_t lin = blockIdx.x + (size_t)gridDim.x * (blockIdx.y + (size_t)gridDim.y * blockIdx.z);
    return ch.trace + ((size_t)(t - ch.trace_t0) * (size_t)ch.trace_stride + lin) * 4;
}

template <int NM, bool BIASED, bool EXACT, bool TREES, bool TRACE = false, bool QUEUE = false, bool HEAD = false, bool LOOK = false, bool PAIR = false>
__device__ __forceinline__ void sweep_kernel_body(const SweepChunk* tab_g, long long t, int nb) {
    SweepChunkC* tab = (SweepChunkC*)tab_g;
    SweepChunkC& ch = tab[pf_chunk()];
    KArgsC& A = ch.A;
    __shared__ Windows W;
    if constexpr (TRACE) {
        if (threadIdx.x == 0) {
            if (unsigned long long* w = wg_trace_slot(ch, t)) {
                w[0] = wall_clock64();
                w[2] = (unsigned long long)__builtin_amdgcn_s_getreg((31 << 11) | 4) | ((unsigned long long)__builtin_amdgcn_s_getreg((3 << 11) | 20) << 32);
                w[3] = (unsigned long long)(unsigned)pf_bx() | ((unsigned long long)(unsigned)pf_chunk() << 32);
            }
        }
    }
    if (HEAD && pf_bx() < nb) {
        if constexpr (HEAD) {
            __builtin_amdgcn_s_waitcnt(0x0F70);
            const SweepHeadR H(sweep_head_of((SweepHeadC*)tab_g, pf_chunk(), t));
            const long long s_begin = PF_HL(H, s_begin), s_last = PF_HL(H, s_last), sx = s_begin + t;
            if (s_last >= s_begin && sx <= s_last + 1) {
                PipeRow PR;
                PR.extend = sx <= s_last ? 1 : 0;
                PR.complete = sx > s_begin ? 1 : 0;
                PR.slot_prev = PR.complete ? (int)((sx - 1) & (PF_RING - 1)) : -1;
                PR.slot_out = (int)(sx & (PF_RING - 1));
                PR.pos_prev = 0.0;
                PR.draws = PF_HI(H, nT) > 0 ? 1 + (int)(sx & 1) : 0;
                PR.ahead = (PF_HI(H, split) || PF_HI(H, P) > 1) ? 1 : 0;
                if constexpr (PAIR) extend_pair_body<EXACT>(A, sx, nb, PR, H);
                else extend_reg_body<NM, BIASED, EXACT, TREES, true, true>(A, sx, 0, PR, H);
            }
        }
    } else {
        const long long s = ch.s_begin + t;
        PipeLaunch PL;
        if (sweep_plan(ch, s, nb, PL)) {
            if (ch.split == 2) PL.nL = -3;
            if (pf_bx() == nb && PL.b_slot >= 0) sweep_windows(A, A.ctrl, PL.b_pos, W);
            pipe_roles<NM, BIASED, EXACT, TREES, 1, false, QUEUE, false, HEAD, LOOK>(A, s, PL, W);
        }
    }
    if constexpr (TRACE) {
        __syncthreads();
        if (threadIdx.x == 0) if (unsigned long long* w = wg_trace_slot(ch, t)) w[1] = wall_clock64();
    }
}
template <int NM, bool BIASED, bool EXACT, bool TREES, bool LOOK = false>
__global__ __launch_bounds__(PF_BS) void k_sweep(const SweepChunk* tab_g, long long t, int nb) {
    sweep_kernel_body<NM, BIASED, EXACT, TREES, false, false, false, LOOK>(tab_g, t, nb);
}
template <bool EXACT, bool TREES>
__global__ __launch_bounds__(PF_BS) __attribute__((amdgpu_waves_per_eu(3, 3))) void k_sweep4(const SweepChunk* tab_g, long long t, int nb) {
    sweep_kernel_body<4, false, EXACT, TREES, false, false, true>(tab_g, t, nb);
}
template <bool EXACT>
__global__ __launch_bounds__(PF_BS) void k_sweep4p(const SweepChunk* tab_g, long long t, int nb) {
    sweep_kernel_body<4, false, EXACT, false, false, false, true, false, true>(tab_g, t, nb);
}
template <bool EXACT, bool TRACE>
__global__ __launch_bounds__(PF_BS) __attribute__((amdgpu_waves_per_eu(3, 3))) void k_sweep4q(const SweepChunk* tab_g, long long t, int nb) {
    sweep_kernel_body<4, false, EXACT, false, TRACE, true, true>(tab_g, t, nb);
}
template <bool EXACT>
__global__ __launch_bounds__(PF_BS) __attribute__((amdgpu_waves_per_eu(3, 3))) void k_sweep4t(const SweepChunk* tab_g, long long t, int nb) {
    sweep_kernel_body<4, false, EXACT, false, true, false, true>(tab_g, t, nb);
}

template <int NM, int P, bool BIASED, bool EXACT = false, bool LEAN = false, bool QUEUE = false, bool COUNTS_ONLY = false>
__device__ __forceinline__ void sweep_blc_body(const SweepChunk* tab_g, long long t) {
    SweepChunkC* tab = (SweepChunkC*)tab_g;
    SweepChunkC& ch = tab[pf_chunk()];
    KArgsC& A = ch.A;
    const long long s = ch.s_begin + t;
    __shared__ Windows W;
    Ctrl* c = A.ctrl;
    PipeLaunch PL;
    if constexpr (COUNTS_ONLY) {
        static_assert(LEAN && !QUEUE, "the second launch of a split step in its static form");
        if (sweep_plan<false>(ch, s, 0, PL)) {
            PL.nT = 0; PL.b_slot = -1;
            pipe_roles<NM, BIASED, EXACT, false, P, true, false, true, false, false, true>(A, s, PL, W);
        }
    } else if (sweep_plan(ch, s, 0, PL)) {
        PL.nT = 0;
        if (ch.split == 2) PL.b_slot = -1;
        if (pf_bx() == 0 && PL.b_slot >= 0) sweep_windows(A, c, PL.b_pos, W);
        pipe_roles<NM, BIASED, EXACT, false, P, true, QUEUE, LEAN>(A, s, PL, W);
    }
}

template <int NM, int P, bool BIASED>
__global__ __launch_bounds__(PF_BS) void k_sweep_blc(const SweepChunk* tab_g, long long t) {
    sweep_blc_body<NM, P, BIASED>(tab_g, t);
}
template <bool EXACT>
__global__ __launch_bounds__(PF_BS) __attribute__((amdgpu_waves_per_eu(4, 4))) void k_sweep_blc4(const SweepChunk* tab_g, long long t) {
    sweep_blc_body<4, 1, false, EXACT, true, false, true>(tab_g, t);
}
template <bool EXACT>
__global__ __launch_bounds__(PF_BS) __attribute__((amdgpu_waves_per_eu(4, 4))) void k_sweep_blc4q(const SweepChunk* tab_g, long long t) {
    sweep_blc_body<4, 1, false, EXACT, true, true>(tab_g, t);
}

template <bool BIASED, bool LOOK = false>
__global__ __launch_bounds__(PF_BS) void k_sweep_xl(const SweepChunk* tab_g, long long t) {
    SweepChunkC* tab = (SweepChunkC*)tab_g;
    SweepChunkC& ch = tab[pf_chunk()];
    KArgsC& A = ch.A;
    const long long s = ch.s_begin + t;
    PipeLaunch PL;
    if (!sweep_plan(ch, s, 0, PL)) return;
    if (!(PL.row.extend || PL.row.complete)) return;
    extern __shared__ double smem[];
    extend_lds_pipe_body<BIASED, LOOK>(A, s, PL.row, smem);
}

__global__ void k_sweep_seed(const SweepChunk* tab_g) {
    SweepChunkC* tab = (SweepChunkC*)tab_g;
    SweepChunkC& ch = tab[blockIdx.x];
    KArgsC& A = ch.A;
    if (ch.s_last < ch.s_begin) return;
    Ctrl* c = A.ctrl;
    const int slot = (int)((ch.s_begin + PF_RING - 1) & (PF_RING - 1));
    if (threadIdx.x == 0) {
        Ctrl::RowInfo& r = c->ri[slot];
        r.n_res = c->n_resample; r.gen = c->gen; r.flag = 0; r.lver = c->lver; r.g_retain = c->g_retain; r.first = A.E;
        r.inv_T = 1.0; r.T = 1.0; r.S1 = 0.0; r.u = 0.0; r.pos = c->cur_pos;
        c->xr[slot].n_res = c->n_resample; c->xr[slot].gen = c->gen; c->xr[slot].flag = 0;
    }
    if ((int)threadIdx.x < A.E) c->counted_to[threadIdx.x] = ch.counted_to[threadIdx.x];
    if ((int)threadIdx.x < PF_RING) c->wq[threadIdx.x] = 0;
    if (ch.nT > 0) {
        const size_t par = (size_t)((ch.s_begin + 1) & 1);
        for (long long p = threadIdx.x; p < A.Np; p += blockDim.x) {
            A.dt_ctr[par * A.Np + p] = A.rng_ctr[p];
            A.dt_filled[par * A.Np + p] = 0;
        }
    }
}

__global__ __launch_bounds__(PF_BS) void k_ledger(KArgs A, int nblocks) {
    ledger_body(A, A.sp, nblocks, (int)blockIdx.x, (int)gridDim.x);
}

__global__ __launch_bounds__(PF_BS) void k_decide(KArgs A, long long s, int mode, Windows W, int nblocks) {
    decide_body(A, s, mode, W, nblocks);
}

__global__ __launch_bounds__(PF_LEDGER_MAXT) void k_decide_ledger(KArgs A, long long s, int mode, Windows W, int nblocks, int ledger_nbt) {
    if ((int)blockIdx.x <= nblocks) {
        if (threadIdx.x < PF_BS) decide_body(A, s, mode, W, nblocks);
    } else {
        const int bx = (int)blockIdx.x - (nblocks + 1);
        if (bx >= nblocks || threadIdx.x < PF_BS) ledger_body(A, A.sp ^ 1, nblocks, bx, ledger_nbt);
    }
}

__global__ __launch_bounds__(PF_BS) void k_resample(KArgs A, long long s, int nblocks) {
    Ctrl* c = A.ctrl;
    if (blockIdx.x == 0 && threadIdx.x == 0) { c->gen_prev = c->gen; c->nres_prev = c->n_resample; }
    const long long Np = A.Np;
    const long long i = (long long)blockIdx.x * PF_BS + threadIdx.x;
    const double inv = c->inv_T;
    if (!c->flag) {
        if (i >= Np) return;
        const DState st = state_slot(A, __builtin_amdgcn_readfirstlane(c->cur));
        st.w_post[i] *= inv;
        st.w_pilot[i] *= inv;
        return;
    }
    if (i >= Np) return;
    const int n = A.n;
    const int G = c->gen - 1;
    const DState src = state_slot(A, __builtin_amdgcn_readfirstlane(c->cur ^ 1));
    const DState dst = state_slot(A, __builtin_amdgcn_readfirstlane(c->cur));
    const int* lo = A.lo + (size_t)(G % A.Gcap) * (Np + 1);
    const double pos = c->cur_pos;
    unsigned widx = A.widx[i];
    if (lo[i + 1] > lo[i]) {
        double* rec = rec_ptr(A, i, widx);
        rec[0] = src.x_mark[i];
        rec[1] = pos;
        rec[2] = 0.0; rec[3] = 0.0;
        rec[4] = __longlong_as_double((long long)make_meta(1, src.mark_limit[i], -1, n));
        for (int r = 0; r < n - 1; ++r) rec[5 + r] = src.S[(size_t)r * Np + i];
        ++widx;
        A.widx[i] = widx;
    }
    A.gstart[(size_t)((G + 1) % A.Gcap) * Np + i] = widx;
    const int q = (int)i;
    const long long a = A.parent[q];
    int ev = (int)c->n_resample - 1;
    if (ev < A.max_trace_events) A.ev_parents[(size_t)ev * Np + q] = (int)a;
    for (int r = 0; r < n - 1; ++r) {
        dst.S[(size_t)r * Np + q] = src.S[(size_t)r * Np + a];
        dst.C[(size_t)(2 * r) * Np + q] = src.C[(size_t)(2 * r) * Np + a];
        dst.C[(size_t)(2 * r + 1) * Np + q] = src.C[(size_t)(2 * r + 1) * Np + a];
    }
    if (A.P > 1) {
        for (int r = 0; r < n - 1; ++r) dst.Pn[(size_t)r * Np + q] = src.Pn[(size_t)r * Np + a];
        const int nmv = src.nm[a];
        dst.nm[q] = nmv;
        for (int k = 0; k < nmv; ++k) {
            dst.Mt[(size_t)k * Np + q] = src.Mt[(size_t)k * Np + a];
            dst.Mb[(size_t)k * Np + q] = src.Mb[(size_t)k * Np + a];
            dst.Mq[(size_t)k * Np + q] = src.Mq[(size_t)k * Np + a];
        }
    }
    double wp = src.w_post[a] * inv;
    double wq = src.w_pilot[a] * inv;
    double sumn = c->S1 * inv;
    double adj = sumn / ((double)Np * wq);
    dst.w_post[q] = wp * adj;
    dst.w_pilot[q] = wq * adj;
    double Lt = src.Ltree[a];
    dst.Ltree[q] = Lt;
    dst.x_mark[q] = pos;
    dst.mark_limit[q] = src.mark_limit[a];
    if (A.apf > 0) dst.lookahead[q] = src.lookahead[a];
    if (A.g_K > 0) dst.ridx[q] = src.ridx[a];
    if (A.n_bias > 0 || A.g_K > 0) {
        int dc = src.dcount[a];
        dst.dcount[q] = dc;
        dst.total_delayed[q] = src.total_delayed[a];
        for (int k = 0; k < dc; ++k) {
            dst.dpos[(size_t)k * Np + q] = src.dpos[(size_t)k * Np + a];
            dst.dfac[(size_t)k * Np + q] = src.dfac[(size_t)k * Np + a];
            dst.ddelta[(size_t)k * Np + q] = src.ddelta[(size_t)k * Np + a];
            dst.dk[(size_t)k * Np + q] = src.dk[(size_t)k * Np + a];
        }
    }
    double nb = src.next_base[a];
    if (q != lo[a] && pos < A.L) {
        Lane ln;
// ... 330 lines not shown
```

smcsmc_amd/csrc/pf_probe.hip:

```cpp
#include <hip/hip_runtime.h>

#include <cstdint>
#include <vector>

#include "pf_tree_reg.h"

namespace {

constexpr int NPART = 5;

__device__ __forceinline__ void spin_100mhz(long long ticks) {
    if (ticks <= 0) return;
    const long long t0 = wall_clock64();
    while (wall_clock64() - t0 < ticks) __builtin_amdgcn_s_sleep(1);
}

__device__ __forceinline__ double reduce_partials(const double* part, int nw, bool coherent) {
    const int lane = threadIdx.x & 63;
    double acc = 0.0;
    for (int k = lane; k < nw * NPART; k += 64) {
        const double v = coherent ? __hip_atomic_load(&part[k], __ATOMIC_RELAXED, __HIP_MEMORY_SCOPE_AGENT) : part[k];
        acc += v;
    }
#pragma unroll
    for (int m = 1; m < 64; m <<= 1) acc += __shfl_xor(acc, m, 64);
    return acc;
}

__global__ __launch_bounds__(256) void k_handoff_launch(const double* prev, double* next, int nw, long long spin, double* out, int row) {
    const int gw = blockIdx.x * 4 + (threadIdx.x >> 6), lane = threadIdx.x & 63;
    double acc = reduce_partials(prev, nw, false);
    spin_100mhz(spin);
    if (gw < nw && lane < NPART) next[gw * NPART + lane] = acc * 1e-3 + (double)(gw + lane + row);
    if (gw < nw && lane == 0) out[gw] = acc;
}

__global__ __launch_bounds__(256) void k_handoff_resident(double* part , unsigned* arrive , int nw, int rows,
                                                          long long spin, double* out, int* err) {
    const int gw = blockIdx.x * 4 + (threadIdx.x >> 6), lane = threadIdx.x & 63;
    double acc = 0.0;
    for (int r = 0; r < rows; ++r) {
        double* mine = part + (size_t)(r & 1) * nw * NPART;
        spin_100mhz(spin);
        if (gw < nw && lane < NPART) __hip_atomic_store(&mine[gw * NPART + lane], acc * 1e-3 + (double)(gw + lane + r), __ATOMIC_RELAXED, __HIP_MEMORY_SCOPE_AGENT);
        if (gw < nw) {
            if (lane == 0) {
                __hip_atomic_fetch_add(&arrive[r], 1u, __ATOMIC_RELEASE, __HIP_MEMORY_SCOPE_AGENT);
                int guard = 0;
                while (__hip_atomic_load(&arrive[r], __ATOMIC_ACQUIRE, __HIP_MEMORY_SCOPE_AGENT) < (unsigned)nw) {
                    if (++guard > 4000000) { *err = 1; break; }
                    __builtin_amdgcn_s_sleep(1);
                }
            }
            __builtin_amdgcn_wave_barrier();
        }
        if (__hip_atomic_load(err, __ATOMIC_RELAXED, __HIP_MEMORY_SCOPE_AGENT)) break;
        acc = reduce_partials(mine, nw, true);
    }
    if (gw < nw && lane == 0) out[gw] = acc;
}

__global__ __launch_bounds__(256) void k_handoff_resident_wg(double* part, unsigned* arrive, int nw, int rows, long long spin, double* out, int* err) {
    __shared__ double s_part[4096];
    __shared__ int s_bad;
    const int gw = blockIdx.x * 4 + (threadIdx.x >> 6), lane = threadIdx.x & 63;
    const int nwg = (int)gridDim.x, np = nw * NPART;
    double acc = 0.0;
    if (threadIdx.x == 0) s_bad = 0;
    for (int r = 0; r < rows; ++r) {
        double* mine = part + (size_t)(r & 1) * np;
        spin_100mhz(spin);
        if (gw < nw && lane < NPART) __hip_atomic_store(&mine[gw * NPART + lane], acc * 1e-3 + (double)(gw + lane + r), __ATOMIC_RELAXED, __HIP_MEMORY_SCOPE_AGENT);
        __syncthreads();
        if (threadIdx.x == 0) {
            __hip_atomic_fetch_add(&arrive[r], 1u, __ATOMIC_RELEASE, __HIP_MEMORY_SCOPE_AGENT);
            int guard = 0;
            while (__hip_atomic_load(&arrive[r], __ATOMIC_ACQUIRE, __HIP_MEMORY_SCOPE_AGENT) < (unsigned)nwg) {
                if (++guard > 4000000) { *err = 1; break; }
                __builtin_amdgcn_s_sleep(1);
            }
            if (__hip_atomic_load(err, __ATOMIC_RELAXED, __HIP_MEMORY_SCOPE_AGENT)) s_bad = 1;
        }
        __syncthreads();
        if (s_bad) break;
        for (int k = threadIdx.x; k < np && k < 4096; k += 256) s_part[k] = __hip_atomic_load(&mine[k], __ATOMIC_RELAXED, __HIP_MEMORY_SCOPE_AGENT);
        __syncthreads();
        double a2 = 0.0;
        for (int k = lane; k < np && k < 4096; k += 64) a2 += s_part[k];
#pragma unroll
        for (int m = 1; m < 64; m <<= 1) a2 += __shfl_xor(a2, m, 64);
        acc = a2;
        __syncthreads();
    }
    if (gw < nw && lane == 0) out[gw] = acc;
}

__global__ __launch_bounds__(256) void k_tree_edit4(int ncases, const double* S, const int32_t* Cin, const double* h, const int32_t* lin,
                                                    const int32_t* rp, const int32_t* sb, const double* tc, const double* u_attach,
                                                    int32_t* oi, double* od) {
    const int i = blockIdx.x * 256 + threadIdx.x;
    if (i >= ncases) return;
#pragma unroll
    for (int form = 0; form < 2; ++form) {
        pf::RTree<4> t;
#pragma unroll
        for (int r = 0; r < 3; ++r) { t.S[r] = S[(size_t)3 * i + r]; t.C0[r] = Cin[(size_t)6 * i + 2 * r]; t.C1[r] = Cin[(size_t)6 * i + 2 * r + 1]; }
        int s_rp = 0, s_sb = 0;
        unsigned desc = 0;
        double Sp = 0.0;
        bool changed = false;
        if (form == 0) {
            pf::RCtx cx = {};
            cx.n = 4; cx.want_desc = true;
            unsigned tmask[7];
            pf::r_update_select<4>(cx, t, 4, h[i], lin[i], false, true, &s_rp, &s_sb, tmask);
            desc = cx.last_desc;
            pf::r_update_edit<4>(cx, t, 4, rp[i], sb[i], tc[i], u_attach[i], tmask, &Sp, &changed);
        } else {
            pf::r4_select(t, h[i], lin[i], &s_rp, &s_sb, &desc);
            pf::r4_edit(t, rp[i], sb[i], tc[i], u_attach[i], &Sp, &changed);
        }
        int32_t* o = oi + ((size_t)form * ncases + i) * 10;
        o[0] = s_rp; o[1] = s_sb; o[2] = (int32_t)desc;
#pragma unroll
        for (int r = 0; r < 3; ++r) { o[3 + 2 * r] = t.C0[r]; o[4 + 2 * r] = t.C1[r]; }
        o[9] = changed ? 1 : 0;
        double* d = od + ((size_t)form * ncases + i) * 4;
#pragma unroll
        for (int r = 0; r < 3; ++r) d[r] = t.S[r];
        d[3] = Sp;
    }
}

__global__ __launch_bounds__(256) void k_wave_prims(int nwaves, const double* xd, const int32_t* xi, double* od, int32_t* oi) {
    const size_t i = (size_t)blockIdx.x * 256 + threadIdx.x, n = (size_t)nwaves * 64;
    const int lane = threadIdx.x & 63;
    if (i >= n) return;
    const double v = xd[i];
    const int k = xi[i];
    od[(0 * 4 + 0) * n + i] = pf::wave_tree_sum_lds(v);
    od[(0 * 4 + 1) * n + i] = pf::wave_hs_scan_lds(v, lane);
    od[(0 * 4 + 2) * n + i] = pf::wave_max_scan_d_lds(v, lane);
    od[(0 * 4 + 3) * n + i] = __shfl_up(v, 1, 64);
    od[(1 * 4 + 0) * n + i] = pf::wave_tree_sum(v);
    od[(1 * 4 + 1) * n + i] = pf::wave_hs_scan(v, lane);
    od[(1 * 4 + 2) * n + i] = pf::wave_max_scan_d(v, lane);
    od[(1 * 4 + 3) * n + i] = pf::wave_prev_lane(v, v);
    int mn = k, mx = k;
    pf::wave_minmax_lds(mn, mx);
    oi[(0 * 4 + 0) * n + i] = pf::wave_max_scan_i_lds(k, lane);
    oi[(0 * 4 + 1) * n + i] = mn;
    oi[(0 * 4 + 2) * n + i] = mx;
    oi[(0 * 4 + 3) * n + i] = __shfl_up(k, 1, 64);
    mn = k; mx = k;
    pf::wave_minmax(mn, mx);
    oi[(1 * 4 + 0) * n + i] = pf::wave_max_scan_i(k, lane);
    oi[(1 * 4 + 1) * n + i] = mn;
    oi[(1 * 4 + 2) * n + i] = mx;
    oi[(1 * 4 + 3) * n + i] = pf::wave_prev_lane(k, k);
}

}

extern "C" int pf_probe_handoff(int32_t mode, int32_t rows, int32_t nw, int64_t spin_ticks, double* us_per_row, double* checksum, int32_t device) {
    if (rows < 1 || nw < 1 || nw > 4096 || (mode == 2 && nw * NPART > 4096)) return -1;
    if (hipSetDevice(device) != hipSuccess) return -1;
    const int nwg = (nw + 3) / 4;
    double *part = nullptr, *out = nullptr;
    unsigned* arrive = nullptr;
    int* err = nullptr;
    hipStream_t st;
    hipEvent_t e0, e1;
    if (hipMalloc(&part, (size_t)2 * nw * NPART * 8) != hipSuccess || hipMalloc(&out, (size_t)nw * 8) != hipSuccess ||
        hipMalloc(&arrive, (size_t)rows * 4) != hipSuccess || hipMalloc(&err, 4) != hipSuccess) return -1;
    hipMemset(part, 0, (size_t)2 * nw * NPART * 8); hipMemset(arrive, 0, (size_t)rows * 4); hipMemset(err, 0, 4); hipMemset(out, 0, (size_t)nw * 8);
    hipStreamCreateWithFlags(&st, hipStreamNonBlocking);
    hipEventCreate(&e0); hipEventCreate(&e1);
    hipDeviceSynchronize();
    if (mode == 0) hipLaunchKernelGGL(k_handoff_launch, dim3(nwg), dim3(256), 0, st, part, part + (size_t)nw * NPART, nw, 0LL, out, -1);
    hipStreamSynchronize(st);
    hipMemset(part, 0, (size_t)2 * nw * NPART * 8);
    hipEventRecord(e0, st);
    if (mode == 0) {
        for (int r = 0; r < rows; ++r) {
            double* prev = part + (size_t)((r + 1) & 1) * nw * NPART;
            double* next = part + (size_t)(r & 1) * nw * NPART;
            hipLaunchKernelGGL(k_handoff_launch, dim3(nwg), dim3(256), 0, st, prev, next, nw, (long long)spin_ticks, out, r);
        }
    } else if (mode == 1) {
        hipLaunchKernelGGL(k_handoff_resident, dim3(nwg), dim3(256), 0, st, part, arrive, nw, rows, (long long)spin_ticks, out, err);
    } else {
        hipLaunchKernelGGL(k_handoff_resident_wg, dim3(nwg), dim3(256), 0, st, part, arrive, nw, rows, (long long)spin_ticks, out, err);
    }
    hipEventRecord(e1, st);
    if (mode == 0)
        hipLaunchKernelGGL(k_handoff_launch, dim3(nwg), dim3(256), 0, st, part + (size_t)((rows + 1) & 1) * nw * NPART, part + (size_t)(rows & 1) * nw * NPART, nw, 0LL, out, rows);
    const hipError_t rc = hipStreamSynchronize(st);
    float ms = 0.f;
    hipEventElapsedTime(&ms, e0, e1);
    std::vector<double> h(nw);
    int herr = 0;
    hipMemcpy(h.data(), out, (size_t)nw * 8, hipMemcpyDeviceToHost);
    hipMemcpy(&herr, err, 4, hipMemcpyDeviceToHost);
    double cs = 0.0;
    for (double v : h) cs += v;
    if (us_per_row) *us_per_row = 1e3 * (double)ms / rows;
    if (checksum) *checksum = cs;
    hipFree(part); hipFree(out); hipFree(arrive); hipFree(err);
    hipEventDestroy(e0); hipEventDestroy(e1); hipStreamDestroy(st);
    return (rc == hipSuccess && herr == 0) ? 0 : -2;
}

extern "C" int pf_probe_tree_edit(int32_t ncases, const double* S, const int32_t* C, const double* h, const int32_t* lin, const int32_t* rp,
                                   const int32_t* sb, const double* tc, const double* u_attach, int32_t* out_i, double* out_d, int32_t device) {
    if (ncases < 1 || ncases > (1 << 24)) return -1;
    if (hipSetDevice(device) != hipSuccess) return -1;
    const size_t nc = (size_t)ncases;
    const void* src[8] = {S, C, h, lin, rp, sb, tc, u_attach};
    const size_t bytes[8] = {nc * 3 * 8, nc * 6 * 4, nc * 8, nc * 4, nc * 4, nc * 4, nc * 8, nc * 8};
    void* d[8] = {};
    int32_t* d_oi = nullptr;
    double* d_od = nullptr;
    bool ok = true;
    for (int k = 0; k < 8 && ok; ++k)
        ok = hipMalloc(&d[k], bytes[k]) == hipSuccess && hipMemcpy(d[k], src[k], bytes[k], hipMemcpyHostToDevice) == hipSuccess;
    ok = ok && hipMalloc(&d_oi, nc * 2 * 10 * 4) == hipSuccess && hipMalloc(&d_od, nc * 2 * 4 * 8) == hipSuccess;
    if (ok) {
        hipLaunchKernelGGL(k_tree_edit4, dim3((unsigned)((nc + 255) / 256)), dim3(256), 0, 0, ncases, (const double*)d[0], (const int32_t*)d[1],
                           (const double*)d[2], (const int32_t*)d[3], (const int32_t*)d[4], (const int32_t*)d[5], (const double*)d[6],
                           (const double*)d[7], d_oi, d_od);
        ok = hipGetLastError() == hipSuccess && hipDeviceSynchronize() == hipSuccess &&
             hipMemcpy(out_i, d_oi, nc * 2 * 10 * 4, hipMemcpyDeviceToHost) == hipSuccess &&
             hipMemcpy(out_d, d_od, nc * 2 * 4 * 8, hipMemcpyDeviceToHost) == hipSuccess;
    }
    for (int k = 0; k < 8; ++k) if (d[k]) hipFree(d[k]);
    if (d_oi) hipFree(d_oi);
    if (d_od) hipFree(d_od);
    return ok ? 0 : -2;
}

extern "C" int pf_probe_wave_prims(int32_t nwaves, const double* xd, const int32_t* xi, double* out_d, int32_t* out_i, int32_t device) {
    if (nwaves < 1 || nwaves > (1 << 18)) return -1;
    if (hipSetDevice(device) != hipSuccess) return -1;
    const size_t n = (size_t)nwaves * 64;
    double *d_xd = nullptr, *d_od = nullptr;
    int32_t *d_xi = nullptr, *d_oi = nullptr;
    bool ok = hipMalloc(&d_xd, n * 8) == hipSuccess && hipMalloc(&d_xi, n * 4) == hipSuccess && hipMalloc(&d_od, n * 8 * 8) == hipSuccess &&
              hipMalloc(&d_oi, n * 8 * 4) == hipSuccess && hipMemcpy(d_xd, xd, n * 8, hipMemcpyHostToDevice) == hipSuccess &&
              hipMemcpy(d_xi, xi, n * 4, hipMemcpyHostToDevice) == hipSuccess;
    if (ok) {
        hipLaunchKernelGGL(k_wave_prims, dim3((unsigned)((n + 255) / 256)), dim3(256), 0, 0, nwaves, (const double*)d_xd, (const int32_t*)d_xi, d_od, d_oi);
        ok = hipGetLastError() == hipSuccess && hipDeviceSynchronize() == hipSuccess &&
             hipMemcpy(out_d, d_od, n * 8 * 8, hipMemcpyDeviceToHost) == hipSuccess &&
             hipMemcpy(out_i, d_oi, n * 8 * 4, hipMemcpyDeviceToHost) == hipSuccess;
    }
    if (d_xd) hipFree(d_xd);
    if (d_xi) hipFree(d_xi);
    if (d_od) hipFree(d_od);
    if (d_oi) hipFree(d_oi);
    return ok ? 0 : -2;
}
```

smcsmc_amd/pf.py:

```python
import ctypes as C
import os

import numpy as np

_HERE = os.path.dirname(os.path.abspath(__file__))
LIB_PATH = os.path.join(_HERE, "csrc", "libsmcsmc_pf.so")
_LIB = None


class PfError(RuntimeError):
    pass


class _Model(C.Structure):
    _fields_ = [
        ("n_epochs", C.c_int32), ("n_pops", C.c_int32), ("nsam", C.c_int32), ("flags", C.c_int32),
        ("loci_length", C.c_double), ("mutation_rate", C.c_double), ("recombination_rate", C.c_double),
        ("change_times", C.POINTER(C.c_double)), ("pop_sizes", C.POINTER(C.c_double)),
        ("mig_rates", C.POINTER(C.c_double)), ("single_mig", C.POINTER(C.c_double)),
        ("sample_pops", C.POINTER(C.c_int32)), ("record_flags", C.POINTER(C.c_int32)),
        ("lags", C.POINTER(C.c_double)),
        ("n_bias_heights", C.c_int32), ("delay_type", C.c_int32),
        ("bias_heights", C.POINTER(C.c_double)), ("bias_strengths", C.POINTER(C.c_double)),
        ("application_delays", C.POINTER(C.c_double)),
        ("vb_coal_counts", C.POINTER(C.c_double)), ("vb_mig_counts", C.POINTER(C.c_double)),
        ("n_rate_segments", C.c_int32), ("reserved2", C.c_int32),
        ("rate_positions", C.POINTER(C.c_double)), ("rate_values", C.POINTER(C.c_double)),
        ("leaf_rel_rates", C.POINTER(C.c_double)),
        ("sample_times", C.POINTER(C.c_double)),
    ]


class _Params(C.Structure):
    _fields_ = [("np", C.c_int64), ("ess_fraction", C.c_double), ("seed", C.c_uint64),
                ("max_trace_events", C.c_int32), ("flags", C.c_int32),
                ("log_cap", C.c_int64), ("gen_cap", C.c_int64), ("piece_cap", C.c_int64),
                ("debug", C.c_int32), ("mig_cap", C.c_int32), ("count_wgs", C.c_int32), ("delay_cap", C.c_int32),
                ("count_workers", C.c_int32), ("reserved4", C.c_int32)]


DEBUG_FORCE_LDS, DEBUG_NO_FUSE, DEBUG_NO_COUNT, DEBUG_TWO_LAUNCH = 1, 2, 4, 8
DEBUG_FORCE_WIDE = 2048
NSAM_MAX, NSAM_MAX_WIDE = 16, 64


class _Segments(C.Structure):
    _fields_ = [("n", C.c_int64), ("start", C.POINTER(C.c_double)), ("length", C.POINTER(C.c_double)),
                ("state", C.POINTER(C.c_int8)), ("alleles", C.POINTER(C.c_int8)),
                ("max_record_epoch", C.POINTER(C.c_int32))]


class _Lookahead(C.Structure):
    _fields_ = [("level", C.c_int32), ("max_doubletons", C.c_int32), ("n_quantiles", C.c_int32), ("flags", C.c_int32),
                ("n", C.c_int64),
                ("first_singleton_distance", C.POINTER(C.c_double)), ("relative_mutation_rate", C.POINTER(C.c_double)),
                ("is_singleton_unphased", C.POINTER(C.c_int8)), ("n_doubletons", C.POINTER(C.c_int32)),
                ("doubleton_idx", C.POINTER(C.c_int8)), ("doubleton_dist", C.POINTER(C.c_double)),
                ("first_split_distance", C.POINTER(C.c_double)), ("split_alleles", C.POINTER(C.c_int8)),
                ("split_count", C.POINTER(C.c_int32)), ("quantiles", C.POINTER(C.c_double)),
                ("tbl_lengths", C.POINTER(C.c_double)), ("mean_total_branch_length", C.c_double)]


LA_ROW_PIPELINE = 1
LA_ROW_PIPELINE_MP = 2
LA_ROW_PIPELINE_LDS = 4


class PackedLookahead:

    def __init__(self, la, level, tbl, quantiles, struct_cls=_Lookahead, pipeline=False, structured=False, lds=False):
        f = lambda a, t: np.ascontiguousarray(a, dtype=t)
        self.a = [f(la["first_singleton_distance"], np.float64), f(la["relative_mutation_rate"], np.float64),
                  f(la["is_singleton_unphased"], np.int8), f(la["n_doubletons"], np.int32), f(la["doubleton_idx"], np.int8),
                  f(la["doubleton_dist"], np.float64), f(la["first_split_distance"], np.float64),
                  f(la["split_alleles"], np.int8), f(la["split_count"], np.int32), f(quantiles, np.float64),
                  f(tbl[0], np.float64)]
        ptr = lambda a: a.ctypes.data_as(C.POINTER({np.dtype(np.float64): C.c_double, np.dtype(np.int8): C.c_int8,
                                                    np.dtype(np.int32): C.c_int32}[a.dtype]))
        self.struct = struct_cls(int(level), int(la["max_doubletons"]), len(quantiles),
                                 (LA_ROW_PIPELINE if pipeline else 0) | (LA_ROW_PIPELINE_MP if structured else 0) |
                                 (LA_ROW_PIPELINE_LDS if lds else 0),
                                 len(la["n_doubletons"]),
                                 *[ptr(a) for a in self.a], float(tbl[1]))


EXPORTS = [
    "pf_last_error", "pf_device_count", "pf_device_cus", "pf_create", "pf_destroy", "pf_init_prior", "pf_load_segments", "pf_load_lookahead",
    "pf_terminal_branch_quantiles",
    "pf_update_segment", "pf_count", "pf_resample", "pf_run", "pf_run_many", "pf_can_run_many", "pf_get_run_path", "pf_get_row_form", "pf_finish", "pf_sync",
    "pf_num_segments_done", "pf_logl", "pf_get_counts", "pf_get_trace", "pf_get_resample_events",
    "pf_get_particles", "pf_get_migrations", "pf_get_local_recomb", "pf_sample_tree_events", "pf_sample_tree_events_pops", "pf_get_kernel_time", "pf_set_timing", "pf_get_stats", "pf_get_delay_stats", "pf_probe_handoff", "pf_probe_tree_edit", "pf_probe_wave_prims", "pf_set_wg_trace", "pf_get_wg_trace", "pf_debug_stamps", "pf_test_search_lut", "pf_simulate_sites",
    "pf_simulate_sites_wide", "pf_median_survival", "pf_median_survival_opts", "pf_test_math", "pf_test_div", "pf_test_uniform", "pf_test_reduce", "pf_test_systematic",
    "pf_test_live_bytes", "pf_test_plan",
]


def load_library(path=None):
    global _LIB
    if _LIB is not None and path is None:
        return _LIB
    path = path or LIB_PATH
    if not os.path.exists(path):
        raise PfError("HIP extension %s is missing: run `python -c 'import __graft_entry__ as g; g.build()'` "
                      "(there is no CPU fallback)" % path)
    L = C.CDLL(path)
    vp = C.c_void_p
    L.pf_last_error.restype = C.c_char_p
    L.pf_device_count.restype = C.c_int
    L.pf_device_cus.argtypes = [C.c_int]
    L.pf_create.restype = vp
    L.pf_create.argtypes = [C.POINTER(_Model), C.POINTER(_Params), C.c_int]
    L.pf_destroy.argtypes = [vp]
    L.pf_init_prior.argtypes = [vp, C.c_double]
    L.pf_load_segments.argtypes = [vp, C.POINTER(_Segments)]
    L.pf_load_lookahead.argtypes = [vp, C.POINTER(_Lookahead)]
    L.pf_terminal_branch_quantiles.argtypes = [C.POINTER(_Model), C.c_uint64, C.c_int64, vp, C.c_int32, vp, vp, C.c_int]
    L.pf_update_segment.argtypes = [vp, C.c_int64]
    L.pf_count.argtypes = [vp, C.c_int64, C.c_int]
    L.pf_resample.argtypes = [vp, C.c_int64]
    L.pf_run.argtypes = [vp, C.c_int64, C.c_int64]
    L.pf_run_many.argtypes = [vp, C.c_int32, C.c_int64, C.c_int64]
    L.pf_can_run_many.argtypes = [vp, C.c_int32]
    L.pf_get_run_path.argtypes = [vp, C.c_int]
    L.pf_get_row_form.argtypes = [vp]
    L.pf_finish.argtypes = [vp]
    L.pf_sync.argtypes = [vp]
    L.pf_sample_tree_events.restype = C.c_int64
    L.pf_sample_tree_events.argtypes = [vp, vp, vp, vp, vp, C.c_int64, C.POINTER(C.c_int64)]
    L.pf_sample_tree_events_pops.restype = C.c_int64
    L.pf_sample_tree_events_pops.argtypes = [vp, vp, vp, vp, vp, vp, vp, C.c_int64, C.POINTER(C.c_int64)]
    L.pf_num_segments_done.restype = C.c_int64
    L.pf_num_segments_done.argtypes = [vp]
    L.pf_logl.restype = C.c_double
    L.pf_logl.argtypes = [vp]
    L.pf_get_counts.argtypes = [vp, vp, C.c_int32]
    L.pf_get_trace.argtypes = [vp, vp, vp, vp, vp, C.c_int64]
    L.pf_get_resample_events.argtypes = [vp, vp, vp, C.c_int32]
    L.pf_get_particles.argtypes = [vp, vp, vp, vp, vp, vp]
    L.pf_get_migrations.argtypes = [vp, vp, vp, vp, vp, vp, C.c_int32]
    L.pf_get_local_recomb.argtypes = [vp, vp, vp, C.c_int64]
    L.pf_get_kernel_time.argtypes = [vp, C.c_int, vp, vp]
    L.pf_set_timing.argtypes = [vp, C.c_int]
    L.pf_get_stats.argtypes = [vp, vp, vp, vp]
    L.pf_get_delay_stats.argtypes = [vp, vp, vp]
    L.pf_probe_handoff.argtypes = [C.c_int32, C.c_int32, C.c_int32, C.c_int64, vp, vp, C.c_int32]
    L.pf_probe_tree_edit.argtypes = [C.c_int32] + [vp] * 10 + [C.c_int32]
    L.pf_probe_wave_prims.argtypes = [C.c_int32] + [vp] * 4 + [C.c_int32]
    L.pf_set_wg_trace.argtypes = [vp, C.c_int64, C.c_int32]
    L.pf_get_wg_trace.argtypes = [vp, vp, C.c_int64, vp]
    L.pf_get_wg_trace.restype = C.c_int64
    L.pf_median_survival.argtypes = [C.POINTER(_Model), C.c_uint64, C.c_int32, C.c_int64, vp, vp, C.c_int]
    L.pf_median_survival_opts.argtypes = [C.POINTER(_Model), C.c_uint64, C.c_int32, C.c_int64, vp, vp, C.c_int32, C.c_int]
    L.pf_simulate_sites_wide.argtypes = [C.c_void_p, C.c_uint64, C.c_int32, C.c_int64, C.c_void_p, C.c_void_p, C.c_void_p, C.c_int]
    L.pf_simulate_sites_wide.restype = C.c_int
    L.pf_test_math.argtypes = [vp, C.c_int64, vp, vp, vp, C.c_int]
    L.pf_test_div.argtypes = [vp, vp, C.c_int64, vp, C.c_int]
    L.pf_test_uniform.argtypes = [C.c_uint64, C.c_uint32, C.c_uint32, C.c_uint64, C.c_int64, vp, C.c_int]
    L.pf_test_reduce.argtypes = [vp, C.c_int64, vp, vp, C.c_int]
    L.pf_test_systematic.argtypes = [vp, C.c_int64, C.c_double, vp, C.c_int]
    L.pf_test_live_bytes.restype = C.c_int64
    L.pf_test_live_bytes.argtypes = []
    L.pf_test_plan.argtypes = [C.POINTER(_Model), C.POINTER(_Params), vp, C.c_int32]
    if path == LIB_PATH:
        _LIB = L
    return L


def _dp(a):
    return a.ctypes.data_as(C.POINTER(C.c_double))


def _err(L):
    return (L.pf_last_error() or b"").decode()


def _attach_bias(owner, cmodel, m):
    bh = m.get("bias_heights")
    if bh is None or len(bh) == 0:
        cmodel.n_bias_heights = 0
        return
    owner._bh = np.ascontiguousarray(bh, dtype=np.float64)
    owner._bs = np.ascontiguousarray(m["bias_strengths"], dtype=np.float64)
    owner._ad = np.ascontiguousarray(m["application_delays"], dtype=np.float64)
    if len(owner._bs) != len(owner._bh) + 1 or len(owner._ad) != cmodel.n_epochs:
        raise PfError("bias_strengths needs one more entry than bias_heights; application_delays one per epoch")
    cmodel.n_bias_heights = len(owner._bh)
    cmodel.delay_type = int(m.get("delay_type", 0))
    cmodel.bias_heights = _dp(owner._bh)
    cmodel.bias_strengths = _dp(owner._bs)
    cmodel.application_delays = _dp(owner._ad)


def _attach_structure(owner, cmodel, m, E, P):
    if P > 4:
        cmodel.flags |= MODEL_WIDE_POPS
    if m.get("sample_times") is not None:
        owner._stimes = np.ascontiguousarray(m["sample_times"], dtype=np.float64)
        if len(owner._stimes) != cmodel.nsam:
            raise PfError("sample_times needs one entry per sample")
        cmodel.sample_times = _dp(owner._stimes)
        cmodel.flags |= MODEL_SAMPLE_TIMES
    if m.get("mig_rates") is not None:
        owner._mig = np.ascontiguousarray(m["mig_rates"], dtype=np.float64).reshape(E * P * P)
        cmodel.mig_rates = _dp(owner._mig)
    if m.get("single_mig") is not None:
        owner._smig = np.ascontiguousarray(m["single_mig"], dtype=np.float64).reshape(E * P * P)
        cmodel.single_mig = _dp(owner._smig)
    if m.get("guide") is not None:
        gd = m["guide"]
        owner._gpos = np.ascontiguousarray(gd["positions"], dtype=np.float64)
        owner._grate = np.ascontiguousarray(gd["rates"], dtype=np.float64)
        owner._gleaf = np.ascontiguousarray(gd["leaf_rates"], dtype=np.float64).reshape(len(owner._gpos) * cmodel.nsam)
        cmodel.n_rate_segments = len(owner._gpos)
        cmodel.rate_positions = _dp(owner._gpos)
        cmodel.rate_values = _dp(owner._grate)
        cmodel.leaf_rel_rates = _dp(owner._gleaf)
        if not cmodel.application_delays:
            owner._gad = np.ascontiguousarray(m["application_delays"], dtype=np.float64)
            cmodel.application_delays = _dp(owner._gad)
            cmodel.delay_type = int(m.get("delay_type", 0))
    if m.get("vb_coal_counts") is not None:
        owner._vbc = np.ascontiguousarray(m["vb_coal_counts"], dtype=np.float64).reshape(E * P)
        cmodel.vb_coal_counts = _dp(owner._vbc)
        if m.get("vb_mig_counts") is not None:
            owner._vbm = np.ascontiguousarray(m["vb_mig_counts"], dtype=np.float64).reshape(E * P * P)
            cmodel.vb_mig_counts = _dp(owner._vbm)
    if m.get("sample_pops") is not None:
        owner._spop = np.ascontiguousarray(m["sample_pops"], dtype=np.int32)
        if len(owner._spop) != cmodel.nsam:
            raise PfError("sample_pops needs one entry per sample")
        cmodel.sample_pops = owner._spop.ctypes.data_as(C.POINTER(C.c_int32))


def counts_len(E, P=1):
    return 6 * E + 4 if P == 1 else 3 * E * P + 3 * E + E * P * P + 2 * E * P + 4


def unpack_counts(out, E, P=1):
    if P == 1:
        return {
            "coal_count": out[0:E].copy(), "coal_opp": out[E:2 * E].copy(), "coal_weight": out[2 * E:3 * E].copy(),
            "rec_count": out[3 * E:4 * E].copy(), "rec_opp": out[4 * E:5 * E].copy(),
            "rec_weight": out[5 * E:6 * E].copy(), "delayed_opp": out[6 * E], "delayed_count": out[6 * E + 1],
            "resample_count": out[6 * E + 2], "logl": out[6 * E + 3],
        }
    o = 0
    d = {}
    for k in ("coal_count", "coal_opp", "coal_weight"):
        d[k] = out[o:o + E * P].reshape(E, P).copy(); o += E * P
    for k in ("rec_count", "rec_opp", "rec_weight"):
        d[k] = out[o:o + E].copy(); o += E
    d["mig_count"] = out[o:o + E * P * P].reshape(E, P, P).copy(); o += E * P * P
    for k in ("mig_opp", "mig_weight"):
        d[k] = out[o:o + E * P].reshape(E, P).copy(); o += E * P
    d["delayed_opp"], d["delayed_count"], d["resample_count"], d["logl"] = (float(v) for v in out[o:o + 4])
    return d


KERNEL_CLASSES = ("extend", "decide", "count", "resample")


def probe_handoff(mode, rows=2000, nw=157, spin_us=0.0, device=0):
    L = load_library()
    us = C.c_double(); cs = C.c_double()
    rc = L.pf_probe_handoff(int(mode), int(rows), int(nw), int(round(spin_us * 100.0)), C.byref(us), C.byref(cs), int(device))
    if rc != 0:
        raise PfError("pf_probe_handoff failed (%d)" % rc)
    return us.value, cs.value


def probe_tree_edit(S, Cc, h, lin, rp, sb, tc, u_attach, device=0):
    L = load_library()
    f8 = lambda a, shape: np.ascontiguousarray(a, dtype=np.float64).reshape(shape)
    i4 = lambda a, shape: np.ascontiguousarray(a, dtype=np.int32).reshape(shape)
    n = len(h)
    a = [f8(S, (n, 3)), i4(Cc, (n, 6)), f8(h, n), i4(lin, n), i4(rp, n), i4(sb, n), f8(tc, n), f8(u_attach, n)]
    oi = np.zeros((2, n, 10), np.int32); od = np.zeros((2, n, 4), np.float64)
    rc = L.pf_probe_tree_edit(n, *[x.ctypes.data for x in a], oi.ctypes.data, od.ctypes.data, int(device))
    if rc != 0:
        raise PfError("pf_probe_tree_edit failed (%d)" % rc)
    return oi, od


WAVE_PRIMS_D = ("wave_tree_sum", "wave_hs_scan", "wave_max_scan_d", "wave_prev_lane")
WAVE_PRIMS_I = ("wave_max_scan_i", "wave_minmax.min", "wave_minmax.max", "wave_prev_lane")


def probe_wave_prims(xd, xi, device=0):
    L = load_library()
    xd = np.ascontiguousarray(xd, dtype=np.float64); xi = np.ascontiguousarray(xi, dtype=np.int32)
    if xd.ndim != 2 or xd.shape[1] != 64 or xi.shape != xd.shape:
        raise PfError("probe_wave_prims: xd and xi must both be [K][64]")
    k = xd.shape[0]
    od = np.zeros((2, 4, k, 64), np.float64); oi = np.zeros((2, 4, k, 64), np.int32)
    rc = L.pf_probe_wave_prims(k, xd.ctypes.data, xi.ctypes.data, od.ctypes.data, oi.ctypes.data, int(device))
    if rc != 0:
        raise PfError("pf_probe_wave_prims failed (%d)" % rc)
    return od, oi


RUN_PATHS = ("General", "TwoLaunch", "KPipe", "Sweep", "SweepSplit", "SweepXmp", "SweepXl", "SweepXlmp")
ROW_FORMS = (None, "single", "paired")
DEBUG_NO_PAIR = 4096
MODEL_SAMPLE_TIMES = 8
MODEL_WIDE_POPS = 4
FLAG_MP_LDS_ROWS = 8
DEBUG_SIGNAL_ALL_COUNTS = 16384


class ParticleFilter:
    def __init__(self, model, np_particles, ess_fraction=0.5, seed=1, max_trace_events=64, device=0, local_recomb=False,
                 record_trees=False, log_cap=0, gen_cap=0, piece_cap=0, debug=0, mig_cap=0, count_wgs=0, delay_cap=0,
                 delay_evict=False, count_workers=0, mp_rows=False):
        self.L = load_library()
        self._pack(model, np_particles, ess_fraction, seed, max_trace_events, local_recomb, record_trees, log_cap, gen_cap, piece_cap, debug,
                   mig_cap, count_wgs, delay_cap, delay_evict, count_workers, mp_rows)
        self.h = self.L.pf_create(C.byref(self._model), C.byref(self._params), int(device))
        if not self.h:
            raise PfError(_err(self.L))
        self.n_segs = 0

    def _pack(self, model, np_particles, ess_fraction=0.5, seed=1, max_trace_events=64, local_recomb=False, record_trees=False, log_cap=0,
              gen_cap=0, piece_cap=0, debug=0, mig_cap=0, count_wgs=0, delay_cap=0, delay_evict=False, count_workers=0, mp_rows=False):
        m = model
        self._ct = np.ascontiguousarray(m["change_times"], dtype=np.float64)
        E = len(self._ct)
        P = int(m.get("n_pops", 1))
        self._ps = np.ascontiguousarray(m["pop_sizes"], dtype=np.float64).reshape(E * P)
        self._rf = np.ascontiguousarray(m.get("record_flags", [3] * E), dtype=np.int32)
        self._lags = np.ascontiguousarray(m["lags"], dtype=np.float64)
        flags = (1 if m.get("ancestral_aware") else 0) | (2 if m.get("dephase") else 0)
        self.E, self.P, self.nsam, self.Np = E, P, int(m["nsam"]), int(np_particles)
        self.max_trace_events = int(max_trace_events)
        self._model = _Model(E, P, self.nsam, flags, float(m["loci_length"]), float(m["mutation_rate"]),
                             float(m["recombination_rate"]), _dp(self._ct), _dp(self._ps), None, None, None,
                             self._rf.ctypes.data_as(C.POINTER(C.c_int32)), _dp(self._lags))
        _attach_bias(self, self._model, m)
        _attach_structure(self, self._model, m, E, P)
        self.loci_length = float(m["loci_length"])
        self._params = _Params(self.Np, float(ess_fraction), int(seed), self.max_trace_events,
                               (1 if local_recomb else 0) | (2 if record_trees else 0) | (4 if delay_evict else 0) | (FLAG_MP_LDS_ROWS if mp_rows else 0),
                               int(log_cap), int(gen_cap), int(piece_cap), int(debug), int(mig_cap), int(count_wgs), int(delay_cap), int(count_workers), 0)
        self.mig_cap = int(mig_cap) if mig_cap else 96

    def _chk(self, rc):
        if rc < 0:
            raise PfError(_err(self.L))
        return rc

    def close(self):
        if getattr(self, "h", None):
            self.L.pf_destroy(self.h)
            self.h = None

    def __del__(self):
        try:
            self.close()
        except Exception:
            pass

    def init_prior(self, initial_position=0.0):
        self._chk(self.L.pf_init_prior(self.h, float(initial_position)))

    def load_segments(self, segs):
        self._s0 = np.ascontiguousarray(segs["start"], dtype=np.float64)
        self._s1 = np.ascontiguousarray(segs["length"], dtype=np.float64)
        self._s2 = np.ascontiguousarray(segs["state"], dtype=np.int8)
        self._s3 = np.ascontiguousarray(segs["alleles"], dtype=np.int8).reshape(-1)
        self._s4 = np.ascontiguousarray(segs["max_record_epoch"], dtype=np.int32)
        n = len(self._s0)
        assert len(self._s3) == n * self.nsam
        sg = _Segments(n, _dp(self._s0), _dp(self._s1), self._s2.ctypes.data_as(C.POINTER(C.c_int8)),
                       self._s3.ctypes.data_as(C.POINTER(C.c_int8)), self._s4.ctypes.data_as(C.POINTER(C.c_int32)))
        self._chk(self.L.pf_load_segments(self.h, C.byref(sg)))
        self.n_segs = n

    def load_lookahead(self, la, level, tbl, quantiles=None, pipeline=False, structured=False, lds=False):
        from . import segments as segmod
        self._la = PackedLookahead(la, level, tbl, segmod.TBL_QUANTILES if quantiles is None else quantiles, pipeline=pipeline,
                                   structured=structured, lds=lds)
        self._chk(self.L.pf_load_lookahead(self.h, C.byref(self._la.struct)))

    def run(self, s_begin=0, s_end=None):
        self._chk(self.L.pf_run(self.h, int(s_begin), int(self.n_segs if s_end is None else s_end)))

    @staticmethod
    def run_many(filters, s_begin=0, s_end=None):
        if s_end is None:
            s_end = max(f.n_segs for f in filters)
        hs = (C.c_void_p * len(filters))(*[f.h for f in filters])
        filters[0]._chk(filters[0].L.pf_run_many(hs, len(filters), int(s_begin), int(s_end)))

    @staticmethod
    def can_run_many(filters):
        if not filters:
            return False
        hs = (C.c_void_p * len(filters))(*[f.h for f in filters])
        return bool(filters[0].L.pf_can_run_many(hs, len(filters)))

    def run_path(self, many=False):
        k = int(self.L.pf_get_run_path(self.h, int(bool(many))))
        return None if k < 0 else RUN_PATHS[k]

    def row_form(self):
        return ROW_FORMS[int(self.L.pf_get_row_form(self.h))]

    def update_segment(self, s):
        self._chk(self.L.pf_update_segment(self.h, int(s)))

    def count(self, s, end_data=False):
        self._chk(self.L.pf_count(self.h, int(s), int(end_data)))

    def resample(self, s):
        self._chk(self.L.pf_resample(self.h, int(s)))

    def finish(self):
        self._chk(self.L.pf_finish(self.h))

    def sync(self):
        self._chk(self.L.pf_sync(self.h))

    def segments_done(self):
        return int(self.L.pf_num_segments_done(self.h))

    def logl(self):
        return float(self.L.pf_logl(self.h))

    def trace(self):
        self.sync()
        n = self.segments_done()
        T = np.zeros(n); ess = np.zeros(n); flag = np.zeros(n, np.int32); logl = np.zeros(n)
        self._chk(self.L.pf_get_trace(self.h, T.ctypes.data, ess.ctypes.data, flag.ctypes.data, logl.ctypes.data, n))
        return {"T": T, "ess": ess, "resampled": flag, "logl": logl}

    def resample_events(self):
        seg = np.zeros(max(1, self.max_trace_events), np.int32)
        par = np.zeros((max(1, self.max_trace_events), self.Np), np.int32)
        n = self._chk(self.L.pf_get_resample_events(self.h, seg.ctypes.data, par.ctypes.data, self.max_trace_events))
        return seg[:n], par[:n]

    def particles(self):
        n = self.nsam
        wp = np.zeros(self.Np); wq = np.zeros(self.Np); H = np.zeros((self.Np, n - 1))
        Ch = np.zeros((self.Np, n - 1, 2), np.int8); nb = np.zeros(self.Np)
        self._chk(self.L.pf_get_particles(self.h, wp.ctypes.data, wq.ctypes.data, H.ctypes.data, Ch.ctypes.data,
                                          nb.ctypes.data))
        return {"w_post": wp, "w_pilot": wq, "heights": H, "children": Ch, "next_base": nb}

    def counts(self):
        out = np.zeros(counts_len(self.E, self.P))
        self._chk(self.L.pf_get_counts(self.h, out.ctypes.data, len(out)))
        return unpack_counts(out, self.E, self.P)

# ... 207 lines not shown
```

Baseline: 48290.

## Add short-window count path with register offsets and DPP integer scans

Adds a SHORT_WIN variant of the count body. When a workgroup's generation window spans fewer than four generations, it reads the run counts directly into registers and picks each task's generation with comparisons. This skips the LDS prefix-sum tile, its barriers and the binary search. The shuffle-based integer scans are replaced with DPP row-shift scans, and the ledger update moves into its own header. New probes and per-workgroup stamps are added for validation and profiling, at the cost of another template instantiation and extra code paths to keep correct.

```diff
diff --git a/include/smcsmc_pf.h b/include/smcsmc_pf.h
--- a/include/smcsmc_pf.h
+++ b/include/smcsmc_pf.h
@@ -162,11 +162,15 @@
 int pf_get_kernel_time(pf_handle* h, int k, double* ms, int64_t* launches);
 int pf_set_timing(pf_handle* h, int enable);
 int pf_debug_stamps(pf_handle* h, int64_t rows, uint64_t* out);
+int pf_debug_stamps_blc(pf_handle* h, int64_t rows, uint64_t* out);
 int pf_test_search_lut(const double* tab, int32_t n, uint8_t* lut, int32_t* kbase);
 int pf_probe_handoff(int32_t mode, int32_t rows, int32_t nw, int64_t spin_ticks, double* us_per_row, double* checksum, int32_t device);
 int pf_probe_tree_edit(int32_t ncases, const double* S, const int32_t* C, const double* h, const int32_t* lin, const int32_t* rp,
                         const int32_t* sb, const double* tc, const double* u_attach, int32_t* out_i, double* out_d, int32_t device);
 int pf_probe_wave_prims(int32_t nwaves, const double* xd, const int32_t* xi, double* out_d, int32_t* out_i, int32_t device);
+int pf_probe_wave_iscan(int32_t nwaves, const int32_t* xi, int32_t* out_i, int32_t device);
+int pf_probe_ledger(int32_t Np, int32_t ngen, int32_t nlb, const int32_t* st, const int32_t* anc, const int32_t* nruns, const int32_t* lo,
+                    int32_t* out_st, int32_t* out_anc, int32_t* out_nruns, int32_t device);
 int pf_set_wg_trace(pf_handle* h, int64_t first_step, int32_t n_steps);
 int64_t pf_get_wg_trace(pf_handle* h, uint64_t* out, int64_t cap_words, int32_t* info);
 int pf_get_delay_stats(pf_handle* h, int64_t* n_forced, int32_t* peak_pending);
diff --git a/profiles/stamps_blc.py b/profiles/stamps_blc.py
--- /dev/null
+++ b/profiles/stamps_blc.py
@@ -0,0 +1,94 @@
+import argparse
+import ctypes as C
+import os
+import sys
+
+import numpy as np
+
+ROOT = os.path.dirname(os.path.dirname(os.path.abspath(__file__)))
+sys.path.insert(0, ROOT)
+from smcsmc_amd import pf, build as _build
+
+ap = argparse.ArgumentParser()
+ap.add_argument("--rows", type=int, default=6000)
+ap.add_argument("--debug", type=int, default=0)
+ap.add_argument("--lib", default=None, help="a -DPF_STAMPS library built beforehand (default: build it, smcsmc_amd/build.py)")
+a = ap.parse_args()
+pf.LIB_PATH = a.lib or _build.build_stamps_lib()
+import bench
+
+WG, W = 1600, 8
+args = argparse.Namespace(nsam=4, length=1e7, epochs=32, pops=1)
+model, segs = bench.build_workload(args, seed=1)
+f = pf.ParticleFilter(model, 10000, seed=1, max_trace_events=0, local_recomb=True, debug=a.debug)
+f.load_segments(segs)
+L = f.L
+L.pf_debug_stamps.argtypes = [C.c_void_p, C.c_int64, C.c_void_p]; L.pf_debug_stamps.restype = C.c_int
+L.pf_debug_stamps_blc.argtypes = [C.c_void_p, C.c_int64, C.c_void_p]; L.pf_debug_stamps_blc.restype = C.c_int
+f.init_prior(0.0); f.run(0, 200); f.sync()
+rows = a.rows
+assert L.pf_debug_stamps(f.h, rows, None) == 0
+f.init_prior(0.0); f.run(0, rows); f.sync()
+out = np.zeros((rows, WG, W), np.uint64)
+assert L.pf_debug_stamps_blc(f.h, rows, out.ctypes.data) == 0, "not a -DPF_STAMPS library?"
+flag = f.trace()["resampled"][:rows]
+
+us = lambda x: x.astype(np.int64) * 10.0 / 1000.0
+steps = np.arange(8, rows - 1)
+st = out[steps]
+used = st[:, :, 0] > 0
+role = st[:, :, 7].astype(np.int64)
+t0 = np.where(used, us(st[:, :, 0]), np.inf).min(axis=1)
+rel = lambda k: us(st[:, :, k]) - t0[:, None]
+resampled = flag[steps - 2] == 1
+print("steps %d, of which the row resampled: %d (%.1f %%)" % (len(steps), resampled.sum(), 100.0 * resampled.mean()))
+print("workgroups of a launch: mean %.0f; start of the last one after the first: mean %.2f us" % (used.sum(axis=1).mean(), np.where(used, rel(0), 0).max(axis=1).mean()))
+print("plan made (start -> word 1), mean over workgroups: %.2f us" % (us(st[:, :, 1]) - us(st[:, :, 0]))[used & (st[:, :, 1] > 0)].mean())
+
+led = (role == 1) | (role == 2)
+cnt = role == 3
+led_end = np.where(led & (st[:, :, 2] > 0), rel(2), -1.0)
+cnt_done = np.where(cnt, np.maximum.reduce([np.where(st[:, :, k] > 0, rel(k), -1.0) for k in (2, 3, 4, 5)]), -1.0)
+for sel, nm in ((resampled, "rows that resample"), (~resampled, "rows that do not")):
+    if not sel.any():
+        continue
+    le, ce = led_end[sel].max(axis=1), cnt_done[sel].max(axis=1)
+    print("%s (%d): last ledger workgroup ends at %.2f us (median %.2f), last count workgroup at %.2f us (median %.2f); the launch ends with the ledger on %.1f %% of them"
+          % (nm, sel.sum(), le[le >= 0].mean() if (le >= 0).any() else float("nan"), np.median(le[le >= 0]) if (le >= 0).any() else float("nan"),
+             ce[ce >= 0].mean() if (ce >= 0).any() else float("nan"), np.median(ce[ce >= 0]) if (ce >= 0).any() else float("nan"), 100.0 * (le > ce).mean()))
+    ss = st[sel]
+    if (le >= 0).any():
+        i = led_end[sel].argmax(axis=1)
+        w = ss[np.arange(len(i)), i]
+        ok = le >= 0
+        print("   last ledger workgroup: start %.2f, plan made +%.2f, done +%.2f us; it is the re-basing of the newest list on %.1f %% of the rows"
+              % ((us(w[:, 0]) - t0[sel])[ok].mean(), (us(w[:, 1]) - us(w[:, 0]))[ok].mean(), (us(w[:, 2]) - us(w[:, 1]))[ok].mean(),
+                 100.0 * (i[ok] == np.where(role[sel] == 2, np.arange(WG)[None, :], WG).min(axis=1)[ok]).mean()))
+    j = cnt_done[sel].argmax(axis=1)
+    w = ss[np.arange(len(j)), j]
+    ok = (ce >= 0) & (w[:, 5] > 0)
+    if ok.any():
+        print("   last count workgroup: start %.2f, plan made +%.2f, prologue +%.2f, rounds 1 and 2 +%.2f, records +%.2f, reduction stored +%.2f us; window of %.2f generations"
+              % ((us(w[:, 0]) - t0[sel])[ok].mean(), (us(w[:, 1]) - us(w[:, 0]))[ok].mean(), (us(w[:, 2]) - us(w[:, 1]))[ok].mean(),
+                 (us(w[:, 3]) - us(w[:, 2]))[ok].mean(), (us(w[:, 4]) - us(w[:, 3]))[ok].mean(), (us(w[:, 5]) - us(w[:, 4]))[ok].mean(),
+                 (w[:, 6].astype(np.int64) & 0xffff)[ok].mean()))
+
+pct = (1, 10, 25, 50, 75, 90, 99)
+r2 = (role == 2) & resampled[:, None]
+if r2.any():
+    first = np.where(r2, np.arange(WG)[None, :], WG).min(axis=1)
+    rows_r = np.nonzero(first < WG)[0]
+    ret = st[rows_r, first[rows_r], 4].astype(np.int64)
+    nl = st[rows_r, first[rows_r], 5].astype(np.int64)
+    print("retained generations G - g_retain on resampling rows, percentiles %s: %s; above 64 (second pass has work) on %.1f %%, above 832 (two to a wavefront) on %.1f %%"
+          % (pct, np.percentile(ret, pct).astype(int).tolist(), 100.0 * (ret > 64).mean(), 100.0 * (ret > 832).mean()))
+    print("runs of the newest list, percentiles %s: %s; more than 2 048 (two tiles) on %.1f %%, more than 4 096 on %.1f %%, more than 6 144 on %.1f %%"
+          % (pct, np.percentile(nl, pct).astype(int).tolist(), 100.0 * (nl > 2048).mean(), 100.0 * (nl > 4096).mean(), 100.0 * (nl > 6144).mean()))
+depth = (st[:, :, 6].astype(np.int64) & 0xffff)[cnt]
+worked = (st[:, :, 5] > 0)[cnt]
+print("count workgroups past their window check: %d a step; generations of their windows, percentiles %s: %s; at most 1: %.1f %%, 2: %.1f %%, 4: %.1f %%"
+      % (cnt.sum() / len(steps), pct, np.percentile(depth, pct).astype(int).tolist(), 100.0 * (depth <= 1).mean(), 100.0 * (depth <= 2).mean(), 100.0 * (depth <= 4).mean()))
+if worked.any():
+    dw = depth[worked]
+    print("   of those with tasks (%d a step): at most 1: %.1f %%, 2: %.1f %%, 4: %.1f %%, 8: %.1f %%; largest %d"
+          % (worked.sum() / len(steps), 100.0 * (dw <= 1).mean(), 100.0 * (dw <= 2).mean(), 100.0 * (dw <= 4).mean(), 100.0 * (dw <= 8).mean(), dw.max()))
diff --git a/smcsmc_amd/csrc/pf_device.h b/smcsmc_amd/csrc/pf_device.h
--- a/smcsmc_amd/csrc/pf_device.h
+++ b/smcsmc_amd/csrc/pf_device.h
@@ -310,6 +310,17 @@
     v = wave_dpp_max<DPP_ROW_BCAST31, 0xc>(v);
     return v;
 }
+template <int CTRL, int ROW_MASK = 0xf>
+__device__ __forceinline__ int wave_dpp_iadd(int v) { return v + dpp_mov<CTRL, ROW_MASK>(0, v); }
+__device__ __forceinline__ int wave_iscan(int v) {
+    v = wave_dpp_iadd<DPP_ROW_SHR + 1>(v);
+    v = wave_dpp_iadd<DPP_ROW_SHR + 2>(v);
+    v = wave_dpp_iadd<DPP_ROW_SHR + 4>(v);
+    v = wave_dpp_iadd<DPP_ROW_SHR + 8>(v);
+    v = wave_dpp_iadd<DPP_ROW_BCAST15, 0xa>(v);
+    v = wave_dpp_iadd<DPP_ROW_BCAST31, 0xc>(v);
+    return v;
+}
 __device__ __forceinline__ double wave_max_scan_d(double v, int) { return wave_max_scan(v); }
 __device__ __forceinline__ int wave_max_scan_i(int v, int) { return wave_max_scan(v); }
 
diff --git a/smcsmc_amd/csrc/pf_get.h b/smcsmc_amd/csrc/pf_get.h
--- a/smcsmc_amd/csrc/pf_get.h
+++ b/smcsmc_amd/csrc/pf_get.h
@@ -357,8 +357,9 @@
     HIPCHK(hipSetDevice(h->device));
     if (rows > 0 && !out) {
         unsigned long long* buf = nullptr;
-        if (h->alloc(&buf, (size_t)rows * h->A.nc * PF_STAMP_W)) return -1;
-        HIPCHK(hipMemset(buf, 0, (size_t)rows * h->A.nc * PF_STAMP_W * 8));
+        const size_t words = (size_t)rows * h->A.nc * PF_STAMP_W + (size_t)rows * 1600 * 8;
+        if (h->alloc(&buf, words)) return -1;
+        HIPCHK(hipMemset(buf, 0, words * 8));
         HIPCHK(hipStreamSynchronize(h->stream));
         h->A.stamps = buf; h->A.stamp_rows = rows;
         return 0;
@@ -366,6 +367,15 @@
     if (!h->A.stamps) { g_err = "pf_debug_stamps: not enabled"; return -1; }
     if (pf_sync(h)) return -1;
     HIPCHK(hipMemcpy(out, h->A.stamps, (size_t)std::min<long long>(rows, h->A.stamp_rows) * h->A.nc * PF_STAMP_W * 8, hipMemcpyDeviceToHost));
+    return 0;
+}
+
+int pf_debug_stamps_blc(pf_handle* h, int64_t rows, uint64_t* out) {
+    HIPCHK(hipSetDevice(h->device));
+    if (!h->A.stamps || !out) { g_err = "pf_debug_stamps_blc: not enabled"; return -1; }
+    if (pf_sync(h)) return -1;
+    HIPCHK(hipMemcpy(out, h->A.stamps + (size_t)h->A.stamp_rows * h->A.nc * PF_STAMP_W,
+                     (size_t)std::min<long long>(rows, h->A.stamp_rows) * 1600 * 8 * 8, hipMemcpyDeviceToHost));
     return 0;
 }
 
diff --git a/smcsmc_amd/csrc/pf_hip.hip b/smcsmc_amd/csrc/pf_hip.hip
--- a/smcsmc_amd/csrc/pf_hip.hip
+++ b/smcsmc_amd/csrc/pf_hip.hip
@@ -58,7 +58,14 @@
             A.stamps[((size_t)s * A.nc + (size_t)(((long long)pf_bx() * PF_BS + threadIdx.x) >> 6)) * PF_STAMP_W + 9 + k_] = pf_acc[k_]; \
         for (int k_ = 0; k_ < 8; ++k_)                                                                                  \
             A.stamps[((size_t)s * A.nc + (size_t)(((long long)pf_bx() * PF_BS + threadIdx.x) >> 6)) * PF_STAMP_W + 21 + k_] = pf_acc2[k_]; } } while (0)
+#define PF_BSTAMP_WG 1600
+#define PF_BSTAMP_W 8
+__device__ __forceinline__ long long* pf_bstamp_step() { __shared__ long long step_; return &step_; }
+#define PF_BSTAMP(k, v) do { if (threadIdx.x == 0 && A.stamps) { const long long s_ = *pf_bstamp_step();                  \
+        if (s_ >= 0 && s_ < A.stamp_rows && pf_bx() < PF_BSTAMP_WG)                                                     \
+            (A.stamps + (size_t)A.stamp_rows * A.nc * PF_STAMP_W)[((size_t)s_ * PF_BSTAMP_WG + pf_bx()) * PF_BSTAMP_W + (k)] = (unsigned long long)(v); } } while (0)
 #else
+#define PF_BSTAMP(k, v) do {} while (0)
 #define PF_STAMP(k) do {} while (0)
 #define PF_TICK(var) do {} while (0)
 #define PF_ACC(slot, t0, t1) do {} while (0)
@@ -1364,7 +1371,7 @@
     }
 }
 
-struct RunLists { int* st; int* anc; int* nruns; };
+#include "pf_ledger.h"
 struct CountSrc {
     const double* w; const double* S; const double* xm; const int* ml; const unsigned* widx;
     const unsigned* widx_live;
@@ -1404,6 +1411,7 @@
 }
 
 #define PF_CNT_TILE 2048
+#define PF_CNT_SHORT 4
 #define PF_CNT_WIDE 128
 #define PF_CNT_BATCH 2
 
@@ -1437,7 +1445,7 @@
     return pre;
 }
 
-template <int NM, int P, bool EXACT = false, bool ACC_AT_ENTRY = false, bool ANC = false, class KA>
+template <int NM, int P, bool EXACT = false, bool ACC_AT_ENTRY = false, bool ANC = false, bool SHORT_WIN = false, class KA>
 __device__ __forceinline__ void count_body(const KA& A, const CountSrc& Q, int e, double win_a, double win_b, int bx, int nbxg) {
     constexpr int NI = NM - 1;
     using AC = AccT<P>;
@@ -1472,6 +1480,12 @@
     const int lane = threadIdx.x & 63;
     const long long gtid = (long long)bx * PF_BS + threadIdx.x;
     const long long nthreads = (long long)nbxg * PF_BS;
+    bool short_win = false;
+    int sw_o1 = 0, sw_o2 = 0, sw_o3 = 0;
+    if constexpr (SHORT_WIN) {
+        static_assert(!AC::MIG_LDS && PF_CNT_SHORT == 4 && PF_CNT_SHORT <= PF_CNT_TILE, "one tile, four counts in registers, no table to clear behind a barrier");
+        short_win = g_hi - g_lo < PF_CNT_SHORT;
+    }
     AC acc;
 #pragma unroll
     for (int k = 0; k < AC::NR; ++k) acc.v[k] = 0.0;
@@ -1479,6 +1493,17 @@
     for (int tile_hi = g_hi; tile_hi >= g_lo; tile_hi -= PF_CNT_TILE) {
         const int tile_lo = tile_hi - PF_CNT_TILE + 1 > g_lo ? tile_hi - PF_CNT_TILE + 1 : g_lo;
         const int ntile = tile_hi - tile_lo + 1;
+        long long T;
+        if (SHORT_WIN && short_win) {
+            const int* const nru = Q.lists.nruns;
+            int c1 = 0, c2 = 0, c3 = 0;
+            const int c0 = g_hi == G ? (int)Np : nru[g_hi % A.Gcap];
+            if (ntile > 1) c1 = g_hi - 1 == G ? (int)Np : nru[(g_hi - 1) % A.Gcap];
+            if (ntile > 2) c2 = g_hi - 2 == G ? (int)Np : nru[(g_hi - 2) % A.Gcap];
+            if (ntile > 3) c3 = g_hi - 3 == G ? (int)Np : nru[(g_hi - 3) % A.Gcap];
+            sw_o1 = c0; sw_o2 = sw_o1 + c1; sw_o3 = sw_o2 + c2;
+            T = sw_o3 + c3;
+        } else {
         __syncthreads();
         constexpr int PER = PF_CNT_TILE / PF_BS;
         int loc[PER];
@@ -1495,10 +1520,13 @@
             lsum += v;
         }
         int incl = lsum;
+        if constexpr (SHORT_WIN) incl = wave_iscan(incl);
+        else {
 #pragma unroll
         for (int d = 1; d < 64; d <<= 1) {
             int o = __shfl_up(incl, d, 64);
             if (lane >= d) incl += o;
+        }
         }
         if (lane == 63) s_wsum[threadIdx.x >> 6] = incl;
         __syncthreads();
@@ -1513,7 +1541,9 @@
         }
         if (threadIdx.x == PF_BS - 1) s_off[ntile] = run;
         __syncthreads();
-        const long long T = s_off[ntile];
+        T = s_off[ntile];
+        }
+        if constexpr (SHORT_WIN) { PF_BSTAMP(2, wall_clock64()); PF_BSTAMP(6, (unsigned)ntile | ((unsigned)e << 16)); PF_BSTAMP(7, 3); }
         if (tile_hi == g_hi && tile_lo == g_lo && (long long)bx * PF_BS >= T) return;
         if (A.flags & (1 << 20)) return;
         if (L.gopp && !bins_ready) {
@@ -1527,13 +1557,20 @@
             const long long t = base + threadIdx.x;
             const bool tval = t < T;
             int lo_i = 0, hi_i = ntile;
+            int sw_off = 0, sw_nr = 0;
+            if (SHORT_WIN && short_win) {
+                const bool ge1 = tval && t >= sw_o1, ge2 = tval && t >= sw_o2, ge3 = tval && t >= sw_o3;
+                lo_i = (int)ge1 + (int)ge2 + (int)ge3;
+                sw_off = ge3 ? sw_o3 : ge2 ? sw_o2 : ge1 ? sw_o1 : 0;
+                sw_nr = (ge3 ? (int)T : ge2 ? sw_o3 : ge1 ? sw_o2 : sw_o1) - sw_off;
+            } else
             while (tval && hi_i - lo_i > 1) {
                 int mid = (lo_i + hi_i) >> 1;
                 if ((long long)s_off[mid] <= t) lo_i = mid; else hi_i = mid;
             }
             const int tg = tile_hi - lo_i;
-            const long long ti = t - s_off[lo_i];
-            const int tnr = s_off[lo_i + 1] - s_off[lo_i];
+            const long long ti = t - ((SHORT_WIN && short_win) ? sw_off : s_off[lo_i]);
+            const int tnr = (SHORT_WIN && short_win) ? sw_nr : s_off[lo_i + 1] - s_off[lo_i];
             const bool tlive = tval && tg == G;
             int q0 = 0, q1 = 0;
             long long aa = -1;
@@ -1575,10 +1612,14 @@
                 }
             }
             int incl_r = (int)nrec;
+            if constexpr (SHORT_WIN) PF_BSTAMP(3, wall_clock64());
+            if constexpr (SHORT_WIN) incl_r = wave_iscan(incl_r);
+            else {
 #pragma unroll
             for (int d = 1; d < 64; d <<= 1) {
                 const int o = __shfl_up(incl_r, d, 64);
                 if (lane >= d) incl_r += o;
+            }
             }
             if (lane == 63) s_wsum[threadIdx.x >> 6] = incl_r;
             __syncthreads();
@@ -1606,6 +1647,7 @@
             __syncthreads();
         }
     }
+    if constexpr (SHORT_WIN) PF_BSTAMP(4, wall_clock64());
     if (L.gopp && bins_ready) {
         __syncthreads();
         for (int k = threadIdx.x; k < L.nlds; k += PF_BS) {
@@ -1640,6 +1682,7 @@
         if constexpr (ACC_AT_ENTRY) A.partial[((size_t)e * A.nbx + bx) * AC::NC + k] = acc_before + t;
         else A.partial[((size_t)e * A.nbx + bx) * AC::NC + k] += t;
     }
+    if constexpr (SHORT_WIN) PF_BSTAMP(5, wall_clock64());
 }
 
 
@@ -1683,150 +1726,6 @@
     __shared__ double stage[PF_FIN_PAIRS * PF_FIN_TILE_B];
     Ctrl* c = A.ctrl;
     if (c->pending_fin) finalize_counts(A, c, threadIdx.x, blockDim.x, stage);
-}
-
-#define PF_LEDGER_PER 8
-#define PF_LEDGER_MAXT 1024
-#define PF_LEDGER_NEW 64
-
-template <class KA>
-__device__ __forceinline__ void ledger_update(const KA& A, int lb, int nlb, int G, int g_ret, RunLists src, RunLists dst) {
-    __shared__ int scnt[PF_LEDGER_PER * (PF_LEDGER_MAXT / 64)], sexc[PF_LEDGER_PER * (PF_LEDGER_MAXT / 64)];
-    __shared__ int stot;
-    const long long Np = A.Np;
-    const int* lo = A.lo + (size_t)(G % A.Gcap) * (Np + 1);
-    const int tid = threadIdx.x, lane = tid & 63, wave = tid >> 6;
-    const int NT = (int)blockDim.x, NW = NT >> 6;
-    const int NCNT = PF_LEDGER_PER * NW;
-    for (int k = 1 + lb; k < PF_LEDGER_NEW; k += nlb) {
-        const int g = G - k;
-        if (g < g_ret) break;
-        const int* rst = src.st + (size_t)(g % A.Gcap) * Np;
-        const int* ran = src.anc + (size_t)(g % A.Gcap) * Np;
-        int* wst = dst.st + (size_t)(g % A.Gcap) * Np;
-        int* wan = dst.anc + (size_t)(g % A.Gcap) * Np;
-        const int nr = src.nruns[g % A.Gcap];
-        int out_base = 0;
-        for (int tile0 = 0; tile0 < nr; tile0 += PF_LEDGER_PER * NT) {
-            int ns[PF_LEDGER_PER], an[PF_LEDGER_PER], nx[PF_LEDGER_PER];
-#pragma unroll
-            for (int j = 0; j < PF_LEDGER_PER; ++j) {
-                const int i = tile0 + j * NT + tid;
-                ns[j] = i < nr ? rst[i] : 0;
-                an[j] = i < nr ? ran[i] : 0;
-                nx[j] = (lane == 63 && i < nr) ? (i + 1 < nr ? rst[i + 1] : (int)Np) : 0;
-            }
-#pragma unroll
-            for (int j = 0; j < PF_LEDGER_PER; ++j) {
-                const int i = tile0 + j * NT + tid;
-                ns[j] = i < nr ? lo[ns[j]] : 0;
-                nx[j] = (lane == 63 && i < nr) ? lo[nx[j]] : 0;
-            }
-            unsigned keep = 0;
-#pragma unroll
-            for (int j = 0; j < PF_LEDGER_PER; ++j) {
-                const int i = tile0 + j * NT + tid;
-                int ne = __shfl_down(ns[j], 1, 64);
-                if (lane == 63) ne = nx[j];
-                else if (i + 1 >= nr) ne = (int)Np;
-                const bool kp = i < nr && ne > ns[j];
-                const unsigned long long bal = __ballot(kp);
-                if (kp) keep |= 1u << j;
-                if (lane == 0) scnt[j * NW + wave] = __popcll(bal);
-            }
-            asm volatile("s_waitcnt vmcnt(0)" ::: "memory");
-            __syncthreads();
-            if (tid < 64) {
-                const int c0 = 2 * lane < NCNT ? scnt[2 * lane] : 0;
-                const int c1 = 2 * lane + 1 < NCNT ? scnt[2 * lane + 1] : 0;
-                int incl = c0 + c1;
-#pragma unroll
-                for (int d = 1; d < 64; d <<= 1) {
-                    int o = __shfl_up(incl, d, 64);
-                    if (lane >= d) incl += o;
-                }
-                const int excl = incl - (c0 + c1);
-                if (2 * lane < NCNT) sexc[2 * lane] = excl;
-                if (2 * lane + 1 < NCNT) sexc[2 * lane + 1] = excl + c0;
-                if (lane == 63) stot = incl;
-            }
-            __syncthreads();
-#pragma unroll
-            for (int j = 0; j < PF_LEDGER_PER; ++j) {
-                const bool kp = (keep >> j) & 1u;
-                const unsigned long long bal = __ballot(kp);
-                if (kp) {
-                    const int pos = out_base + sexc[j * NW + wave] + __popcll(bal & ((1ULL << lane) - 1ULL));
-                    wst[pos] = ns[j];
-                    wan[pos] = an[j];
-                }
-            }
-            out_base += stot;
-            __syncthreads();
-        }
-        if (tid == 0) dst.nruns[g % A.Gcap] = out_base;
-    }
-    const int wl = lb * NW + wave;
-    const int nwl = nlb * NW;
-    for (int g = G - PF_LEDGER_NEW - wl; g >= g_ret; g -= nwl) {
-        const int* rst = src.st + (size_t)(g % A.Gcap) * Np;
-        const int* ran = src.anc + (size_t)(g % A.Gcap) * Np;
-        int* wst = dst.st + (size_t)(g % A.Gcap) * Np;
-        int* wan = dst.anc + (size_t)(g % A.Gcap) * Np;
-        const int nr = src.nruns[g % A.Gcap];
-        int base = 0;
-        for (int off = 0; off < nr; off += 64) {
-            int i = off + lane;
-            bool valid = i < nr;
-            int stv = 0, nxt = 0, anc = 0;
-            if (valid) {
-                stv = rst[i];
-                nxt = (i + 1 < nr) ? rst[i + 1] : (int)Np;
-                anc = ran[i];
-            }
-            int ns = valid ? lo[stv] : 0;
-            int ne = valid ? lo[nxt] : 0;
-            bool keep = valid && ne > ns;
-            unsigned long long bal = __ballot(keep);
-            int pos = __popcll(bal & ((1ULL << lane) - 1ULL));
-            if (keep) { wst[base + pos] = ns; wan[base + pos] = anc; }
-            base += __popcll(bal);
-        }
-        if (lane == 0) dst.nruns[g % A.Gcap] = base;
-    }
-}
-
-template <class KA>
-__device__ __forceinline__ void ledger_new_list(const KA& A, RunLists dst, const int* blkcnt, int nblocks, int bx, int Gx, int gran = 1) {
-    const long long Np = A.Np;
-    const long long i = (long long)bx * PF_BS + threadIdx.x;
-    __shared__ int wsum[PF_BS / 64];
-    const int* lox = A.lo + (size_t)(Gx % A.Gcap) * (Np + 1);
-    const int lane = threadIdx.x & 63, wave = threadIdx.x >> 6;
-    int l0 = 0, l1 = 0;
-    if (i < Np) { l0 = lox[i]; l1 = lox[i + 1]; }
-    const bool surv = l1 > l0;
-    unsigned long long bal = __ballot(surv);
-    if (lane == 0) wsum[wave] = __popcll(bal);
-    __shared__ int sblk[1024];
-    for (int b = threadIdx.x; b < nblocks; b += PF_BS) {
-        int v = 0;
-        for (int j = 0; j < gran; ++j) v += blkcnt[b * gran + j];
-        sblk[b] = v;
-    }
-    __syncthreads();
-    int base = 0;
-    for (int b = 0; b < bx; ++b) base += sblk[b];
-    for (int w = 0; w < wave; ++w) base += wsum[w];
-    if (surv) {
-        int pos = base + __popcll(bal & ((1ULL << lane) - 1ULL));
-        dst.st[(size_t)(Gx % A.Gcap) * Np + pos] = l0;
-        dst.anc[(size_t)(Gx % A.Gcap) * Np + pos] = (int)i;
-    }
-    if (bx == nblocks - 1 && threadIdx.x == PF_BS - 1) {
-        int tot = base + __popcll(bal);
-        dst.nruns[Gx % A.Gcap] = tot;
-    }
 }
 
 template <class KA>
@@ -1952,15 +1851,17 @@
     }
 }
 
-template <class KA>
+template <bool BATCH2 = false, class KA>
 __device__ __forceinline__ void pipe_ledger_item(const KA& A, const PipeLaunch& PL, const Ctrl::RowInfo& r, int lb) {
     const RunLists src = run_lists(A, r.lver), dst = run_lists(A, r.lver ^ 1);
     const int nblk = PL.nblk;
+    if constexpr (BATCH2) { PF_BSTAMP(7, lb < nblk ? 1 : 2); PF_BSTAMP(4, r.gen - r.g_retain); PF_BSTAMP(5, r.gen > 0 ? src.nruns[(r.gen - 1) % A.Gcap] : 0); }
     if (lb < nblk) ledger_new_list(A, dst, A.rg_blkcnt + (size_t)PL.lc_slot * nblk * A.blk_gran, nblk, lb, r.gen, A.blk_gran);
-    else ledger_update(A, lb - nblk, PL.nL - nblk, r.gen, r.g_retain, src, dst);
-}
-
-template <int NM, bool EXACT, int P, bool ACC_AT_ENTRY = false, class KA>
+    else ledger_update<BATCH2>(A, lb - nblk, PL.nL - nblk, r.gen, r.g_retain, src, dst);
+    if constexpr (BATCH2) PF_BSTAMP(2, wall_clock64());
+}
+
+template <int NM, bool EXACT, int P, bool ACC_AT_ENTRY = false, bool SHORT_WIN = false, class KA>
 __device__ __forceinline__ void pipe_count_item(const KA& A, const PipeLaunch& PL, const Ctrl::RowInfo& r, int idx) {
     int e, cbx, cnb;
     if (A.cw_off && !(A.flags & 512)) {
@@ -1982,11 +1883,11 @@
     Q.offp = A.rg_coffp + (size_t)PL.lc_slot * A.nc;
     Q.lists = run_lists(A, r.lver);
     Q.inv = r.inv_T; Q.G = r.gen; Q.g_lo = r.g_lo[e]; Q.g_hi = r.g_hi[e];
-    count_body<NM, P, EXACT, ACC_AT_ENTRY>(A, Q, e, r.wa[e], r.wb[e], cbx, cnb);
+    count_body<NM, P, EXACT, ACC_AT_ENTRY, false, SHORT_WIN>(A, Q, e, r.wa[e], r.wb[e], cbx, cnb);
 }
 
 template <int NM, bool BIASED, bool EXACT, bool TREES, int P = 1, bool BLC = false, bool QUEUE = false, bool LEAN = false, bool NO_EXTEND = false, bool LOOK = false,
-          bool ACC_AT_ENTRY = false, class KA>
+          bool ACC_AT_ENTRY = false, bool SHORT_WIN = false, bool LEDGER_BATCH2 = false, class KA>
 __device__ __forceinline__ void pipe_roles(const KA& A, long long s, const PipeLaunch& PL, const Windows& Wb) {
     const int bx = pf_bx();
     const int nb = PL.nb;
@@ -2014,8 +1915,8 @@
     const Ctrl::RowInfo& r = c->ri[PL.lc_slot];
     const int lb = bx - (nb + 1) - PL.nT;
     if constexpr (!QUEUE) {
-        if (lb < PL.nL) { if (r.flag) pipe_ledger_item(A, PL, r, lb); }
-        else pipe_count_item<NM, EXACT, P, ACC_AT_ENTRY>(A, PL, r, lb - PL.nL);
+        if (lb < PL.nL) { if (r.flag) pipe_ledger_item<LEDGER_BATCH2>(A, PL, r, lb); }
+        else pipe_count_item<NM, EXACT, P, ACC_AT_ENTRY, SHORT_WIN>(A, PL, r, lb - PL.nL);
     } else {
         __shared__ int s_wk[8];
         if (lb >= PL.workers) return;
@@ -2150,9 +2051,14 @@
     PipeLaunch PL;
     if constexpr (COUNTS_ONLY) {
         static_assert(LEAN && !QUEUE, "the second launch of a split step in its static form");
+#ifdef PF_STAMPS
+        if (threadIdx.x == 0) *pf_bstamp_step() = s;
+#endif
+        PF_BSTAMP(0, wall_clock64());
         if (sweep_plan<false>(ch, s, 0, PL)) {
             PL.nT = 0; PL.b_slot = -1;
-            pipe_roles<NM, BIASED, EXACT, false, P, true, false, true, false, false, true>(A, s, PL, W);
+            PF_BSTAMP(1, wall_clock64());
+            pipe_roles<NM, BIASED, EXACT, false, P, true, false, true, false, false, true, true, true>(A, s, PL, W);
         }
     } else if (sweep_plan(ch, s, 0, PL)) {
         PL.nT = 0;
diff --git a/smcsmc_amd/csrc/pf_ledger.h b/smcsmc_amd/csrc/pf_ledger.h
--- /dev/null
+++ b/smcsmc_amd/csrc/pf_ledger.h
@@ -0,0 +1,208 @@
+#pragma once
+#include "pf_device.h"
+
+struct RunLists { int* st; int* anc; int* nruns; };
+
+#define PF_LEDGER_PER 8
+#define PF_LEDGER_MAXT 1024
+#define PF_LEDGER_NEW 64
+
+#define PF_LEDGER_BATCH 4
+
+template <bool BATCH2 = false, class KA>
+__device__ __forceinline__ void ledger_update(const KA& A, int lb, int nlb, int G, int g_ret, RunLists src, RunLists dst) {
+    __shared__ int scnt[PF_LEDGER_PER * (PF_LEDGER_MAXT / 64)], sexc[PF_LEDGER_PER * (PF_LEDGER_MAXT / 64)];
+    __shared__ int stot;
+    const long long Np = A.Np;
+    const int* lo = A.lo + (size_t)(G % A.Gcap) * (Np + 1);
+    const int tid = threadIdx.x, lane = tid & 63, wave = tid >> 6;
+    const int NT = (int)blockDim.x, NW = NT >> 6;
+    const int NCNT = PF_LEDGER_PER * NW;
+    for (int k = 1 + lb; k < PF_LEDGER_NEW; k += nlb) {
+        const int g = G - k;
+        if (g < g_ret) break;
+        const int* rst = src.st + (size_t)(g % A.Gcap) * Np;
+        const int* ran = src.anc + (size_t)(g % A.Gcap) * Np;
+        int* wst = dst.st + (size_t)(g % A.Gcap) * Np;
+        int* wan = dst.anc + (size_t)(g % A.Gcap) * Np;
+        const int nr = src.nruns[g % A.Gcap];
+        int out_base = 0;
+        for (int tile0 = 0; tile0 < nr; tile0 += PF_LEDGER_PER * NT) {
+            int ns[PF_LEDGER_PER], an[PF_LEDGER_PER], nx[PF_LEDGER_PER];
+#pragma unroll
+            for (int j = 0; j < PF_LEDGER_PER; ++j) {
+                const int i = tile0 + j * NT + tid;
+                ns[j] = i < nr ? rst[i] : 0;
+                an[j] = i < nr ? ran[i] : 0;
+                nx[j] = (lane == 63 && i < nr) ? (i + 1 < nr ? rst[i + 1] : (int)Np) : 0;
+            }
+#pragma unroll
+            for (int j = 0; j < PF_LEDGER_PER; ++j) {
+                const int i = tile0 + j * NT + tid;
+                ns[j] = i < nr ? lo[ns[j]] : 0;
+                nx[j] = (lane == 63 && i < nr) ? lo[nx[j]] : 0;
+            }
+            unsigned keep = 0;
+#pragma unroll
+            for (int j = 0; j < PF_LEDGER_PER; ++j) {
+                const int i = tile0 + j * NT + tid;
+                int ne = __shfl_down(ns[j], 1, 64);
+                if (lane == 63) ne = nx[j];
+                else if (i + 1 >= nr) ne = (int)Np;
+                const bool kp = i < nr && ne > ns[j];
+                const unsigned long long bal = __ballot(kp);
+                if (kp) keep |= 1u << j;
+                if (lane == 0) scnt[j * NW + wave] = __popcll(bal);
+            }
+            asm volatile("s_waitcnt vmcnt(0)" ::: "memory");
+            __syncthreads();
+            if (tid < 64) {
+                const int c0 = 2 * lane < NCNT ? scnt[2 * lane] : 0;
+                const int c1 = 2 * lane + 1 < NCNT ? scnt[2 * lane + 1] : 0;
+                int incl = c0 + c1;
+#pragma unroll
+                for (int d = 1; d < 64; d <<= 1) {
+                    int o = __shfl_up(incl, d, 64);
+                    if (lane >= d) incl += o;
+                }
+                const int excl = incl - (c0 + c1);
+                if (2 * lane < NCNT) sexc[2 * lane] = excl;
+                if (2 * lane + 1 < NCNT) sexc[2 * lane + 1] = excl + c0;
+                if (lane == 63) stot = incl;
+            }
+            __syncthreads();
+#pragma unroll
+            for (int j = 0; j < PF_LEDGER_PER; ++j) {
+                const bool kp = (keep >> j) & 1u;
+                const unsigned long long bal = __ballot(kp);
+                if (kp) {
+                    const int pos = out_base + sexc[j * NW + wave] + __popcll(bal & ((1ULL << lane) - 1ULL));
+                    wst[pos] = ns[j];
+                    wan[pos] = an[j];
+                }
+            }
+            out_base += stot;
+            __syncthreads();
+        }
+        if (tid == 0) dst.nruns[g % A.Gcap] = out_base;
+    }
+    const int wl = lb * NW + wave;
+    const int nwl = nlb * NW;
+    if constexpr (BATCH2) {
+        for (int g0 = G - PF_LEDGER_NEW - wl; g0 >= g_ret; g0 -= PF_LEDGER_BATCH * nwl) {
+            int nr[PF_LEDGER_BATCH], stv[PF_LEDGER_BATCH], nxt[PF_LEDGER_BATCH], anc[PF_LEDGER_BATCH];
+#pragma unroll
+            for (int b = 0; b < PF_LEDGER_BATCH; ++b) {
+                const int g = g0 - b * nwl;
+                nr[b] = g >= g_ret ? src.nruns[g % A.Gcap] : -1;
+            }
+#pragma unroll
+            for (int b = 0; b < PF_LEDGER_BATCH; ++b) {
+                const int g = g0 - b * nwl;
+                stv[b] = 0; nxt[b] = 0; anc[b] = 0;
+                if (nr[b] >= 0 && nr[b] <= 64 && lane < nr[b]) {
+                    const int* rst = src.st + (size_t)(g % A.Gcap) * Np;
+                    stv[b] = rst[lane];
+                    nxt[b] = lane + 1 < nr[b] ? rst[lane + 1] : (int)Np;
+                    anc[b] = src.anc[(size_t)(g % A.Gcap) * Np + lane];
+                }
+            }
+#pragma unroll
+            for (int b = 0; b < PF_LEDGER_BATCH; ++b) {
+                const bool valid = nr[b] >= 0 && nr[b] <= 64 && lane < nr[b];
+                stv[b] = valid ? lo[stv[b]] : 0;
+                nxt[b] = valid ? lo[nxt[b]] : 0;
+            }
+#pragma unroll
+            for (int b = 0; b < PF_LEDGER_BATCH; ++b) {
+                const int g = g0 - b * nwl;
+                if (nr[b] < 0) continue;
+                int* wst = dst.st + (size_t)(g % A.Gcap) * Np;
+                int* wan = dst.anc + (size_t)(g % A.Gcap) * Np;
+                if (nr[b] <= 64) {
+                    const bool keep = lane < nr[b] && nxt[b] > stv[b];
+                    const unsigned long long bal = __ballot(keep);
+                    if (keep) { const int pos = __popcll(bal & ((1ULL << lane) - 1ULL)); wst[pos] = stv[b]; wan[pos] = anc[b]; }
+                    if (lane == 0) dst.nruns[g % A.Gcap] = __popcll(bal);
+                    continue;
+                }
+                const int* rst = src.st + (size_t)(g % A.Gcap) * Np;
+                const int* ran = src.anc + (size_t)(g % A.Gcap) * Np;
+                int base = 0;
+                for (int off = 0; off < nr[b]; off += 64) {
+                    const int i = off + lane;
+                    const bool valid = i < nr[b];
+                    int s0 = 0, s1 = 0, an = 0;
+                    if (valid) { s0 = rst[i]; s1 = (i + 1 < nr[b]) ? rst[i + 1] : (int)Np; an = ran[i]; }
+                    const int ns = valid ? lo[s0] : 0;
+                    const int ne = valid ? lo[s1] : 0;
+                    const bool keep = valid && ne > ns;
+                    const unsigned long long bal = __ballot(keep);
+                    const int pos = __popcll(bal & ((1ULL << lane) - 1ULL));
+                    if (keep) { wst[base + pos] = ns; wan[base + pos] = an; }
+                    base += __popcll(bal);
+                }
+                if (lane == 0) dst.nruns[g % A.Gcap] = base;
+            }
+        }
+    } else
+    for (int g = G - PF_LEDGER_NEW - wl; g >= g_ret; g -= nwl) {
+        const int* rst = src.st + (size_t)(g % A.Gcap) * Np;
+        const int* ran = src.anc + (size_t)(g % A.Gcap) * Np;
+        int* wst = dst.st + (size_t)(g % A.Gcap) * Np;
+        int* wan = dst.anc + (size_t)(g % A.Gcap) * Np;
+        const int nr = src.nruns[g % A.Gcap];
+        int base = 0;
+        for (int off = 0; off < nr; off += 64) {
+            int i = off + lane;
+            bool valid = i < nr;
+            int stv = 0, nxt = 0, anc = 0;
+            if (valid) {
+                stv = rst[i];
+                nxt = (i + 1 < nr) ? rst[i + 1] : (int)Np;
+                anc = ran[i];
+            }
+            int ns = valid ? lo[stv] : 0;
+            int ne = valid ? lo[nxt] : 0;
+            bool keep = valid && ne > ns;
+            unsigned long long bal = __ballot(keep);
+            int pos = __popcll(bal & ((1ULL << lane) - 1ULL));
+            if (keep) { wst[base + pos] = ns; wan[base + pos] = anc; }
+            base += __popcll(bal);
+        }
+        if (lane == 0) dst.nruns[g % A.Gcap] = base;
+    }
+}
+
+template <class KA>
+__device__ __forceinline__ void ledger_new_list(const KA& A, RunLists dst, const int* blkcnt, int nblocks, int bx, int Gx, int gran = 1) {
+    const long long Np = A.Np;
+    const long long i = (long long)bx * PF_BS + threadIdx.x;
+    __shared__ int wsum[PF_BS / 64];
+    const int* lox = A.lo + (size_t)(Gx % A.Gcap) * (Np + 1);
+    const int lane = threadIdx.x & 63, wave = threadIdx.x >> 6;
+    int l0 = 0, l1 = 0;
+    if (i < Np) { l0 = lox[i]; l1 = lox[i + 1]; }
+    const bool surv = l1 > l0;
+    unsigned long long bal = __ballot(surv);
+    if (lane == 0) wsum[wave] = __popcll(bal);
+    __shared__ int sblk[1024];
+    for (int b = threadIdx.x; b < nblocks; b += PF_BS) {
+        int v = 0;
+        for (int j = 0; j < gran; ++j) v += blkcnt[b * gran + j];
+        sblk[b] = v;
+    }
+    __syncthreads();
+    int base = 0;
+    for (int b = 0; b < bx; ++b) base += sblk[b];
+    for (int w = 0; w < wave; ++w) base += wsum[w];
+    if (surv) {
+        int pos = base + __popcll(bal & ((1ULL << lane) - 1ULL));
+        dst.st[(size_t)(Gx % A.Gcap) * Np + pos] = l0;
+        dst.anc[(size_t)(Gx % A.Gcap) * Np + pos] = (int)i;
+    }
+    if (bx == nblocks - 1 && threadIdx.x == PF_BS - 1) {
+        int tot = base + __popcll(bal);
+        dst.nruns[Gx % A.Gcap] = tot;
+    }
+}
diff --git a/smcsmc_amd/csrc/pf_probe.hip b/smcsmc_amd/csrc/pf_probe.hip
--- a/smcsmc_amd/csrc/pf_probe.hip
+++ b/smcsmc_amd/csrc/pf_probe.hip
@@ -4,6 +4,7 @@
 #include <vector>
 
 #include "pf_tree_reg.h"
+#include "pf_ledger.h"
 
 namespace {
 
@@ -160,6 +161,29 @@
     oi[(1 * 4 + 3) * n + i] = pf::wave_prev_lane(k, k);
 }
 
+struct LedgerProbeArgs { long long Np; const int* lo; int Gcap; };
+template <bool BATCH2>
+__global__ __launch_bounds__(256) void k_ledger_probe(LedgerProbeArgs A, int G, RunLists src, RunLists dst) {
+    ledger_update<BATCH2>(A, (int)blockIdx.x, (int)gridDim.x, G, 0, src, dst);
+}
+
+__device__ __forceinline__ int wave_iscan_lds(int v, int lane) {
+#pragma unroll
+    for (int d = 1; d < 64; d <<= 1) {
+        int o = __shfl_up(v, d, 64);
+        if (lane >= d) v += o;
+    }
+    return v;
+}
+
+__global__ __launch_bounds__(256) void k_wave_iscan(int nwaves, const int32_t* xi, int32_t* oi) {
+    const size_t i = (size_t)blockIdx.x * 256 + threadIdx.x, n = (size_t)nwaves * 64;
+    if (i >= n) return;
+    const int k = xi[i];
+    oi[i] = wave_iscan_lds(k, threadIdx.x & 63);
+    oi[n + i] = pf::wave_iscan(k);
+}
+
 }
 
 extern "C" int pf_probe_handoff(int32_t mode, int32_t rows, int32_t nw, int64_t spin_ticks, double* us_per_row, double* checksum, int32_t device) {
@@ -260,3 +284,59 @@
     if (d_oi) hipFree(d_oi);
     return ok ? 0 : -2;
 }
+
+extern "C" int pf_probe_ledger(int32_t Np, int32_t ngen, int32_t nlb, const int32_t* st, const int32_t* anc, const int32_t* nruns, const int32_t* lo,
+                               int32_t* out_st, int32_t* out_anc, int32_t* out_nruns, int32_t device) {
+    if (Np < 1 || Np > (1 << 20) || ngen < 1 || ngen > 4096 || nlb < 1 || nlb > 1024) return -1;
+    for (int g = 0; g < ngen; ++g) if (nruns[g] < 0 || nruns[g] > Np) return -1;
+    for (int g = 0; g < ngen; ++g)
+        for (int i = 0; i < nruns[g]; ++i) {
+            const int v = st[(size_t)g * Np + i];
+            if (v < 0 || v >= Np || (i > 0 && v <= st[(size_t)g * Np + i - 1])) return -1;
+        }
+    for (int i = 0; i <= Np; ++i) if (lo[i] < 0 || lo[i] > Np || (i > 0 && lo[i] < lo[i - 1])) return -1;
+    if (lo[Np] != Np) return -1;
+    if (hipSetDevice(device) != hipSuccess) return -1;
+    const size_t nl = (size_t)ngen * Np, Gcap = (size_t)ngen + 1;
+    int32_t *d_st = nullptr, *d_anc = nullptr, *d_nr = nullptr, *d_lo = nullptr, *d_ost = nullptr, *d_oanc = nullptr, *d_onr = nullptr;
+    bool ok = hipMalloc(&d_st, Gcap * Np * 4) == hipSuccess && hipMalloc(&d_anc, Gcap * Np * 4) == hipSuccess && hipMalloc(&d_nr, Gcap * 4) == hipSuccess &&
+              hipMalloc(&d_lo, Gcap * ((size_t)Np + 1) * 4) == hipSuccess && hipMalloc(&d_ost, 2 * Gcap * Np * 4) == hipSuccess &&
+              hipMalloc(&d_oanc, 2 * Gcap * Np * 4) == hipSuccess && hipMalloc(&d_onr, 2 * Gcap * 4) == hipSuccess &&
+              hipMemset(d_st, 0, Gcap * Np * 4) == hipSuccess && hipMemset(d_anc, 0, Gcap * Np * 4) == hipSuccess && hipMemset(d_nr, 0, Gcap * 4) == hipSuccess &&
+              hipMemset(d_lo, 0, Gcap * ((size_t)Np + 1) * 4) == hipSuccess &&
+              hipMemset(d_ost, 0xff, 2 * Gcap * Np * 4) == hipSuccess && hipMemset(d_oanc, 0xff, 2 * Gcap * Np * 4) == hipSuccess && hipMemset(d_onr, 0xff, 2 * Gcap * 4) == hipSuccess &&
+              hipMemcpy(d_st, st, nl * 4, hipMemcpyHostToDevice) == hipSuccess && hipMemcpy(d_anc, anc, nl * 4, hipMemcpyHostToDevice) == hipSuccess &&
+              hipMemcpy(d_nr, nruns, (size_t)ngen * 4, hipMemcpyHostToDevice) == hipSuccess &&
+              hipMemcpy(d_lo + (size_t)ngen * ((size_t)Np + 1), lo, ((size_t)Np + 1) * 4, hipMemcpyHostToDevice) == hipSuccess;
+    if (ok) {
+        LedgerProbeArgs A; A.Np = Np; A.lo = d_lo; A.Gcap = (int)Gcap;
+        const RunLists src = {d_st, d_anc, d_nr};
+        const RunLists dst0 = {d_ost, d_oanc, d_onr}, dst1 = {d_ost + Gcap * Np, d_oanc + Gcap * Np, d_onr + Gcap};
+        hipLaunchKernelGGL(k_ledger_probe<false>, dim3((unsigned)nlb), dim3(256), 0, 0, A, (int)ngen, src, dst0);
+        hipLaunchKernelGGL(k_ledger_probe<true>, dim3((unsigned)nlb), dim3(256), 0, 0, A, (int)ngen, src, dst1);
+        ok = hipGetLastError() == hipSuccess && hipDeviceSynchronize() == hipSuccess;
+        for (int f = 0; ok && f < 2; ++f)
+            ok = hipMemcpy(out_st + f * nl, d_ost + f * Gcap * Np, nl * 4, hipMemcpyDeviceToHost) == hipSuccess &&
+                 hipMemcpy(out_anc + f * nl, d_oanc + f * Gcap * Np, nl * 4, hipMemcpyDeviceToHost) == hipSuccess &&
+                 hipMemcpy(out_nruns + (size_t)f * ngen, d_onr + f * Gcap, (size_t)ngen * 4, hipMemcpyDeviceToHost) == hipSuccess;
+    }
+    for (int32_t* q : {d_st, d_anc, d_nr, d_lo, d_ost, d_oanc, d_onr}) if (q) hipFree(q);
+    return ok ? 0 : -2;
+}
+
+extern "C" int pf_probe_wave_iscan(int32_t nwaves, const int32_t* xi, int32_t* out_i, int32_t device) {
+    if (nwaves < 1 || nwaves > (1 << 18)) return -1;
+    if (hipSetDevice(device) != hipSuccess) return -1;
+    const size_t n = (size_t)nwaves * 64;
+    int32_t *d_xi = nullptr, *d_oi = nullptr;
+    bool ok = hipMalloc(&d_xi, n * 4) == hipSuccess && hipMalloc(&d_oi, n * 2 * 4) == hipSuccess &&
+              hipMemcpy(d_xi, xi, n * 4, hipMemcpyHostToDevice) == hipSuccess;
+    if (ok) {
+        hipLaunchKernelGGL(k_wave_iscan, dim3((unsigned)((n + 255) / 256)), dim3(256), 0, 0, nwaves, (const int32_t*)d_xi, d_oi);
+        ok = hipGetLastError() == hipSuccess && hipDeviceSynchronize() == hipSuccess &&
+             hipMemcpy(out_i, d_oi, n * 2 * 4, hipMemcpyDeviceToHost) == hipSuccess;
+    }
+    if (d_xi) hipFree(d_xi);
+    if (d_oi) hipFree(d_oi);
+    return ok ? 0 : -2;
+}
diff --git a/smcsmc_amd/pf.py b/smcsmc_amd/pf.py
--- a/smcsmc_amd/pf.py
+++ b/smcsmc_amd/pf.py
@@ -89,7 +89,7 @@
     "pf_terminal_branch_quantiles",
     "pf_update_segment", "pf_count", "pf_resample", "pf_run", "pf_run_many", "pf_can_run_many", "pf_get_run_path", "pf_get_row_form", "pf_finish", "pf_sync",
     "pf_num_segments_done", "pf_logl", "pf_get_counts", "pf_get_trace", "pf_get_resample_events",
-    "pf_get_particles", "pf_get_migrations", "pf_get_local_recomb", "pf_sample_tree_events", "pf_sample_tree_events_pops", "pf_get_kernel_time", "pf_set_timing", "pf_get_stats", "pf_get_delay_stats", "pf_probe_handoff", "pf_probe_tree_edit", "pf_probe_wave_prims", "pf_set_wg_trace", "pf_get_wg_trace", "pf_debug_stamps", "pf_test_search_lut", "pf_simulate_sites",
+    "pf_get_particles", "pf_get_migrations", "pf_get_local_recomb", "pf_sample_tree_events", "pf_sample_tree_events_pops", "pf_get_kernel_time", "pf_set_timing", "pf_get_stats", "pf_get_delay_stats", "pf_probe_handoff", "pf_probe_tree_edit", "pf_probe_wave_prims", "pf_probe_wave_iscan", "pf_probe_ledger", "pf_set_wg_trace", "pf_get_wg_trace", "pf_debug_stamps", "pf_debug_stamps_blc", "pf_test_search_lut", "pf_simulate_sites",
     "pf_simulate_sites_wide", "pf_median_survival", "pf_median_survival_opts", "pf_test_math", "pf_test_div", "pf_test_uniform", "pf_test_reduce", "pf_test_systematic",
     "pf_test_live_bytes", "pf_test_plan",
 ]
@@ -146,6 +146,8 @@
     L.pf_probe_handoff.argtypes = [C.c_int32, C.c_int32, C.c_int32, C.c_int64, vp, vp, C.c_int32]
     L.pf_probe_tree_edit.argtypes = [C.c_int32] + [vp] * 10 + [C.c_int32]
     L.pf_probe_wave_prims.argtypes = [C.c_int32] + [vp] * 4 + [C.c_int32]
+    L.pf_probe_wave_iscan.argtypes = [C.c_int32] + [vp] * 2 + [C.c_int32]
+    L.pf_probe_ledger.argtypes = [C.c_int32] * 3 + [vp] * 7 + [C.c_int32]
     L.pf_set_wg_trace.argtypes = [vp, C.c_int64, C.c_int32]
     L.pf_get_wg_trace.argtypes = [vp, vp, C.c_int64, vp]
     L.pf_get_wg_trace.restype = C.c_int64
@@ -299,6 +301,32 @@
     return od, oi
 
 
+def probe_ledger(st, anc, nruns, lo, nlb, device=0):
+    L = load_library()
+    st = np.ascontiguousarray(st, dtype=np.int32); anc = np.ascontiguousarray(anc, dtype=np.int32)
+    nruns = np.ascontiguousarray(nruns, dtype=np.int32); lo = np.ascontiguousarray(lo, dtype=np.int32)
+    if st.ndim != 2 or anc.shape != st.shape or nruns.shape != (st.shape[0],) or lo.shape != (st.shape[1] + 1,):
+        raise PfError("probe_ledger: st[ngen][Np], anc[ngen][Np], nruns[ngen], lo[Np + 1]")
+    ost = np.zeros((2,) + st.shape, np.int32); oanc = np.zeros((2,) + st.shape, np.int32); onr = np.zeros((2, st.shape[0]), np.int32)
+    rc = L.pf_probe_ledger(st.shape[1], st.shape[0], int(nlb), st.ctypes.data, anc.ctypes.data, nruns.ctypes.data, lo.ctypes.data,
+                           ost.ctypes.data, oanc.ctypes.data, onr.ctypes.data, int(device))
+    if rc != 0:
+        raise PfError("pf_probe_ledger failed (%d)" % rc)
+    return ost, oanc, onr
+
+
+def probe_wave_iscan(xi, device=0):
+    L = load_library()
+    xi = np.ascontiguousarray(xi, dtype=np.int32)
+    if xi.ndim != 2 or xi.shape[1] != 64:
+        raise PfError("probe_wave_iscan: xi must be [K][64]")
+    out = np.zeros((2,) + xi.shape, np.int32)
+    rc = L.pf_probe_wave_iscan(xi.shape[0], xi.ctypes.data, out.ctypes.data, int(device))
+    if rc != 0:
+        raise PfError("pf_probe_wave_iscan failed (%d)" % rc)
+    return out
+
+
 RUN_PATHS = ("General", "TwoLaunch", "KPipe", "Sweep", "SweepSplit", "SweepXmp", "SweepXl", "SweepXlmp")
 ROW_FORMS = (None, "single", "paired")
 DEBUG_NO_PAIR = 4096
```

Result: faster. 49270, median of 6 (+2.0%).
